# zhang-xuan1314/ABC-Net

Measured on AMD Instinct MI355X. Metric: training images/sec (384x384, b16/GPU), higher is better.
Workload: dtype bf16; 1 GPU; unet.py train step (pack+fwd+fused loss+bwd+allreduce+Adam), 384x384, batch 16/GPU, dropout 0.2; global_batch=16, parallelism=dp1, graph=True, device_meters=False, device_rasteriser=False, device_extraction=False, logits_stored=True

## Files before the change

abc-net_amd/_lib.py:

```python
from __future__ import annotations

import ctypes as C
import os

_HERE = os.path.dirname(os.path.abspath(__file__))
LIB_PATH = os.path.join(_HERE, "libabcnet_hip.so")

F32, BF16, FP8 = 0, 1, 2
MAX_TAPS = 49
OMEGA_RAW, OMEGA_PEAKS = 0, 1

vp, i32, u32, i64, f32, f64 = C.c_void_p, C.c_int32, C.c_uint32, C.c_int64, C.c_float, C.c_double


class ActSrc(C.Structure):
    _fields_ = [("x", vp), ("scale", vp), ("shift", vp), ("slope", vp), ("Hx", i32), ("Wx", i32), ("ldx", i32),
                ("pool", i32), ("drop_p", f32), ("drop_seed", u32), ("planar", i32), ("ctot", i32), ("drop_salt", vp)]


class ConvDesc(C.Structure):
    _fields_ = [("src", ActSrc), ("w", vp), ("bias", vp), ("y", vp), ("stats", vp),
                ("dtype_in", i32), ("dtype_c", i32), ("dtype_out", i32),
                ("B", i32), ("Hin", i32), ("Win", i32), ("cin_off", i32), ("Cin", i32), ("Hg", i32), ("Wg", i32),
                ("Hout", i32), ("Wout", i32), ("ldy", i32), ("cout_off", i32), ("Cout", i32), ("Cout_pad", i32),
# ... 224 lines not shown
SCAN_CONSTANT, SCAN_BAD_PARAMS = 1, 2
SCAN_NBOX = 8
SCAN_GEOM_COLUMNS = ("thr", "inverted", "status", "y0", "x0", "bh", "bw", "rows", "cols", "ddx", "ddy", "ink")
SCAN_NO_COMPONENT, SCAN_CLEAN_FAILED = 4, 8
SCAN_CLEAN_CELLS = (8, 16, 32, 64)
SCAN_CLEAN_COLUMNS = ("components", "kept", "ink_kept", "ink_dropped", "heaviest", "occupied_cells")
STROKE_UNTIL_STABLE = -1
STROKE_MAX_SIZE = 1024
STROKE_STAT_COLUMNS = ("iterations", "converged", "ink_in", "ink_out", "skipped")
MOL_EMPTY, MOL_TRUNCATED = 1, 2
MAX_CAP_ATOMS, MAX_BOND_PEAKS, MAX_SCORE_RECORD, MAX_SIM_ATOMS = 2048, 4096, 1024, 512
TEXT_BAD_ROW, TEXT_OVERFLOW = 4, 8


_STRUCTS = [ActSrc, ConvDesc, PackDesc, BnFwdDesc, ActBwdDesc, BnBwdDesc, BnApplyDesc, WgradDesc, WgradReduceDesc,
            LossDesc, LossFinDesc, AdamDesc, NmsDesc, CbamChannelDesc, CbamPixDesc, CbamConv7Desc, MetricsDesc, ExtractDesc, RasterDesc,
            HeadsFusedDesc, HeadsEpi, ConvTDesc, LossScaleDesc, AdamSeg, AdamClass, AdamMultiDesc, ImageDesc, AssembleDesc]

SELF_SIZED = [(EvalDesc, "abc_eval_desc_size"), (GraphScoreDesc, "abc_graph_score_desc_size"),
              (GraphSimilarityDesc, "abc_graph_similarity_desc_size"), (MolBlockDesc, "abc_molblock_desc_size"),
              (ScanDesc, "abc_scan_desc_size")]
SELF_SIZED_SINCE = [(StrokeDesc, "abc_stroke_desc_size"), (GraphIdentityDesc, "abc_graph_identity_desc_size"),
                    (ScanCleanDesc, "abc_scan_clean_desc_size")]

P = C.POINTER
SYMBOLS = {
    "abc_conv_stat_blocks": (C.c_int, [P(ConvDesc)]),
    "abc_convt_fused_ok": (C.c_int, [P(ConvTDesc)]),
    "abc_convt_fused_fwd": (C.c_int, [P(ConvTDesc), vp]),
    "abc_conv_actbwd_ok": (C.c_int, [P(ConvDesc)]),
    "abc_conv_fwd_batch": (C.c_int, [P(ConvDesc), C.c_int32, C.c_void_p]),
    "abc_conv_batch_ok": (C.c_int, [P(ConvDesc), C.c_int32]),
    "abc_conv_variant": (C.c_int, [vp]),
    "abc_conv_weight_layout": (C.c_int, [vp]),
    "abc_conv_fwd": (C.c_int, [P(ConvDesc), vp]),
    "abc_conv_chunk": (C.c_int, [C.c_int, C.c_int]),
    "abc_heads_batch": (C.c_int, [vp, i32, i32, vp]),
    "abc_heads_fused_pack_bytes": (i64, []),
    "abc_heads_fused_chunks": (C.c_int, [P(HeadsFusedDesc)]),
    "abc_heads_fused_loss_blocks": (C.c_int, [P(HeadsFusedDesc)]),
    "abc_heads_fused_dl_elems": (i64, [P(HeadsFusedDesc)]),
    "abc_heads_fused_wgrad_floats": (i64, [P(HeadsFusedDesc)]),
    "abc_heads_fused_rows": (C.c_int, [i32]),
    "abc_heads_fused_chan_of_row": (C.c_int, [i32, i32]),
    "abc_heads_fused_pack": (C.c_int, [P(HeadsFusedDesc), vp]),
    "abc_heads_fused_fwd_bwd": (C.c_int, [P(HeadsFusedDesc), vp]),
    "abc_heads_fused_wgrad": (C.c_int, [P(HeadsFusedDesc), vp]),
    "abc_conv_tile": (C.c_int, [P(ConvDesc), P(i32), P(i32), P(i32)]),
    "abc_conv_route_info": (C.c_int, [P(ConvDesc), P(i32)]),
    "abc_pack_conv_weights": (C.c_int, [P(PackDesc), vp]),
    "abc_pack_item_bytes": (C.c_int, []),
    "abc_pack_item_fill": (i64, [vp, P(PackDesc), i64]),
    "abc_pack_batch": (C.c_int, [vp, i32, i64, vp]),
    "abc_bn_finalize_fwd": (C.c_int, [P(BnFwdDesc), vp]),
    "abc_bn_finalize_fwd_batch": (C.c_int, [vp, i32, i32, vp]),
    "abc_bn_finalize_bwd_batch": (C.c_int, [vp, i32, i32, vp]),
    "abc_bn_eval_coeffs": (C.c_int, [vp, vp, vp, vp, vp, vp, i32, f32, vp]),
    "abc_bn_eval_fold": (C.c_int, [vp, vp, vp, vp, vp, vp, vp, i32, f32, vp]),
    "abc_act_bwd_blocks": (C.c_int, [P(ActBwdDesc)]),
    "abc_act_bwd": (C.c_int, [P(ActBwdDesc), vp]),
    "abc_bn_finalize_bwd": (C.c_int, [P(BnBwdDesc), vp]),
    "abc_bn_apply_bwd": (C.c_int, [P(BnApplyDesc), vp]),
    "abc_wgrad_fuses_apply": (C.c_int, [vp]),
    "abc_wgrad_rowsum_ok": (C.c_int, [vp]),
    "abc_wgrad_pads": (C.c_int, [P(WgradDesc), P(i32), P(i32)]),
    "abc_wgrad_blocks": (C.c_int, [P(WgradDesc)]),
    "abc_wgrad_tile": (C.c_int, [P(WgradDesc), P(i32), P(i32)]),
    "abc_wgrad_route_info": (C.c_int, [P(WgradDesc), P(i32)]),
    "abc_wgrad": (C.c_int, [P(WgradDesc), vp]),
    "abc_wgrad_reduce": (C.c_int, [P(WgradReduceDesc), vp]),
    "abc_wgrad_reduce_bn_bwd": (C.c_int, [P(WgradReduceDesc), P(BnBwdDesc), vp]),
    "abc_wgrad_heads_batch": (C.c_int, [vp, i32, vp]),
    "abc_wgrad_reduce_batch": (C.c_int, [vp, i32, vp]),
    "abc_colsum_blocks": (C.c_int, [i64]),
    "abc_colsum": (C.c_int, [vp, i32, i64, i32, i32, i32, vp, vp, vp, vp]),
    "abc_colsum_w1": (C.c_int, [vp, i32, i64, i32, i32, i32, vp, vp, vp, vp, vp]),
    "abc_loss_blocks": (C.c_int, [P(LossDesc)]),
    "abc_loss_fwd_bwd": (C.c_int, [P(LossDesc), vp]),
    "abc_loss_finalize": (C.c_int, [P(LossFinDesc), vp]),
    "abc_adam_step": (C.c_int, [P(AdamDesc), vp]),
    "abc_loss_scale_grads": (C.c_int, [P(LossScaleDesc), vp]),
    "abc_adam_multi_chunk": (C.c_int, []),
    "abc_adam_multi": (C.c_int, [P(AdamMultiDesc), vp]),
    "abc_nms_peaks": (C.c_int, [P(NmsDesc), vp]),
    "abc_extract_work_ints": (i64, [P(ExtractDesc)]),
    "abc_extract_work_masks": (i64, [P(ExtractDesc)]),
    "abc_extract_peaks": (C.c_int, [P(ExtractDesc), vp]),
    "abc_assemble_work_ints": (i64, [P(AssembleDesc)]),
    "abc_assemble_graphs": (C.c_int, [P(AssembleDesc), vp]),
    "abc_rasterize_targets": (C.c_int, [P(RasterDesc), vp]),
    "abc_build_images": (C.c_int, [P(ImageDesc), vp]),
    "abc_build_scan_images": (C.c_int, [P(ScanDesc), vp]),
    "abc_scan_desc_size": (C.c_int, []),
    "abc_build_scan_images_clean": (C.c_int, [P(ScanDesc), P(ScanCleanDesc), vp]),
    "abc_scan_clean_desc_size": (C.c_int, []),
    "abc_scan_clean_scratch_bytes": (i64, [i32, i32, i32, i32]),
    "abc_normalize_strokes": (C.c_int, [P(StrokeDesc), vp]),
    "abc_stroke_desc_size": (C.c_int, []),
    "abc_metrics_blocks": (C.c_int, [P(MetricsDesc)]),
    "abc_metrics_update": (C.c_int, [P(MetricsDesc), vp]),
    "abc_eval_tables_blocks": (C.c_int, [P(EvalDesc)]),
    "abc_eval_tables_update": (C.c_int, [P(EvalDesc), vp]),
    "abc_eval_tables_update_sparse": (C.c_int, [P(EvalDesc), vp, vp]),
    "abc_eval_desc_size": (C.c_int, []),
    "abc_graph_score_update": (C.c_int, [P(GraphScoreDesc), vp]),
    "abc_graph_score_desc_size": (C.c_int, []),
    "abc_graph_similarity_update": (C.c_int, [P(GraphSimilarityDesc), vp]),
    "abc_graph_similarity_desc_size": (C.c_int, []),
    "abc_graph_identity_update": (C.c_int, [P(GraphIdentityDesc), vp]),
    "abc_graph_identity_desc_size": (C.c_int, []),
    "abc_molblock_text_bytes": (i64, [P(MolBlockDesc)]),
    "abc_write_molblocks": (C.c_int, [P(MolBlockDesc), vp]),
    "abc_molblock_desc_size": (C.c_int, []),
    "abc_plane_sum": (C.c_int, [vp, i32, i32, i32, vp, vp, vp, vp]),
    "abc_plane_sum_work": (C.c_int, [i32]),
    "abc_cbam_channel_fwd": (C.c_int, [P(CbamChannelDesc), vp]),
    "abc_cbam_channel_bwd": (C.c_int, [P(CbamChannelDesc), vp]),
    "abc_cbam_spatial_stats": (C.c_int, [P(CbamPixDesc), vp]),
    "abc_cbam_apply_fwd": (C.c_int, [P(CbamPixDesc), vp]),
    "abc_cbam_bwd1": (C.c_int, [P(CbamPixDesc), vp]),
    "abc_cbam_bwd2_blocks": (C.c_int, [P(CbamPixDesc)]),
    "abc_cbam_bwd2": (C.c_int, [P(CbamPixDesc), vp]),
    "abc_cbam_bwd3_blocks": (C.c_int, [P(CbamPixDesc)]),
    "abc_cbam_bwd3": (C.c_int, [P(CbamPixDesc), vp]),
    "abc_cbam_conv7_fwd": (C.c_int, [P(CbamConv7Desc), vp]),
    "abc_cbam_conv7_blocks": (C.c_int, [P(CbamConv7Desc)]),
    "abc_cbam_conv7_bwd": (C.c_int, [P(CbamConv7Desc), vp]),
    "abc_cbam_conv7_bwd_partial": (C.c_int, [P(CbamConv7Desc), vp]),
    "abc_cbam_channel_bwd_c7": (C.c_int, [P(CbamChannelDesc), P(CbamConv7Desc), vp]),
    "abc_add_into": (C.c_int, [vp, i32, i32, vp, i32, i32, i32, i64, i32, vp]),
    "abc_nhwc_to_nchw_f32": (C.c_int, [vp, i32, i32, i32, i32, i32, i32, vp, vp]),
    "abc_nchw_to_nhwc_f32": (C.c_int, [vp, i32, i32, i32, i32, vp, i32, i32, vp]),
    "abc_fill_f32": (C.c_int, [vp, f32, i64, vp]),
# ... 70 lines not shown
```

abc-net_amd/csrc/bn_act.hip:

```cpp
#include "common.hpp"
#include "../../include/abcnet_hip.h"
#include "capi_util.hpp"
#include "reduce_bn.hpp"
#include <stdlib.h>

namespace {

__device__ inline void bn_finalize_fwd_body(const abc_bn_fwd_desc& d, int pstride) {
    __shared__ double sm[4];
    const int c = blockIdx.x;
    if (c >= d.C) return;
    const int rows = d.rows == 4 ? 4 : 2;
    double s1 = 0.0, s2 = 0.0;
    for (int k = threadIdx.x; k < d.nblk; k += 256) {
        s1 += (double)d.partial[((size_t)k * rows + 0) * pstride + c];
        s2 += (double)d.partial[((size_t)k * rows + 1) * pstride + c];
    }
    s1 = block_sum_f64(s1, sm);
    s2 = block_sum_f64(s2, sm);
    if (threadIdx.x == 0) {
        const double mean = s1 / d.count;
        double var = s2 / d.count - mean * mean;
        if (var < 0.0) var = 0.0;
        const float invstd = (float)(1.0 / sqrt(var + (double)d.eps));
// ... 253 lines not shown
    const int64_t nitems = d.npix * ncv;
    const int64_t stride = (int64_t)gridDim.x * 256;
    T* g = (T*)d.g;
    T* o = d.out ? (T*)d.out : g;
    const int ld_o = d.out ? d.ld_out : d.ld_g;
    const T* yr = (const T*)d.y_raw;
    for (int64_t it = (int64_t)blockIdx.x * 256 + threadIdx.x; it < nitems; it += stride) {
        const int64_t p = it / ncv;
        const int c = (int)(it % ncv) * N;
        float gv[N], x[N], out[N];
        ldv<T, N>(g + p * d.ld_g + c, gv);
        ldv<T, N>(yr + p * d.ld_y + d.cy_off + c, x);
#pragma unroll
        for (int j = 0; j < N; ++j) {
            const float xh = (x[j] - d.mean[c + j]) * d.invstd[c + j];
            out[j] = d.gscale[c + j] * (gv[j] - d.k1[c + j] - xh * d.k2[c + j]);
        }
        stv<N>(o + p * ld_o + c, out);
    }
}

template <typename T>
__global__ __launch_bounds__(256) void colsum_kernel(const T* x, int64_t npix, int ld, int c_off, int C, const float* cs,
                                                      float* work, int CW) {
    __shared__ float red[256];
    const int PL = 256 / CW;
    const int cl = threadIdx.x % CW, pl = threadIdx.x / CW;
    float acc[8];
#pragma unroll
    for (int j = 0; j < 8; ++j) acc[j] = 0.f;
    for (int64_t p = (int64_t)blockIdx.x * PL + pl; p < npix; p += (int64_t)gridDim.x * PL) {
        const T* row = x + p * ld + c_off;
#pragma unroll
        for (int j = 0; j < 8; ++j) {
            const int c = cl + j * CW;
            if (c < C) acc[j] += (float)row[c];
        }
    }
#pragma unroll
    for (int j = 0; j < 8; ++j) {
        const int c = cl + j * CW;
        __syncthreads();
        red[threadIdx.x] = acc[j];
        __syncthreads();
        if (pl == 0 && c < C) {
            float s = 0.f;
            for (int q = 0; q < PL; ++q) s += red[q * CW + cl];
            work[(size_t)blockIdx.x * C + c] = s * (cs ? cs[c_off + c] : 1.f);
        }
    }
}
template <typename T>
__global__ __launch_bounds__(256) void colsum_vec_kernel(const T* x, int64_t npix, int ld, int c_off, int C, const float* cs, float* work) {
    constexpr int N = VecOf<T>::N;
    __shared__ float red[256][N + 1];
    const int ncv = C / N;
    const int cv = threadIdx.x % ncv, pl = threadIdx.x / ncv, PL = 256 / ncv;
    float acc[N];
#pragma unroll
    for (int j = 0; j < N; ++j) acc[j] = 0.f;
    const T* base = x + c_off + cv * N;
    int64_t p = (int64_t)blockIdx.x * PL + pl;
    const int64_t step = (int64_t)gridDim.x * PL;
    for (; p + step < npix; p += 2 * step) {
        float a[N], b[N];
        ldv<T, N>(base + p * ld, a);
        ldv<T, N>(base + (p + step) * ld, b);
#pragma unroll
        for (int j = 0; j < N; ++j) acc[j] += a[j] + b[j];
    }
    if (p < npix) {
        float a[N];
        ldv<T, N>(base + p * ld, a);
#pragma unroll
        for (int j = 0; j < N; ++j) acc[j] += a[j];
    }
#pragma unroll
    for (int j = 0; j < N; ++j) red[threadIdx.x][j] = acc[j];
    __syncthreads();
    for (int c = threadIdx.x; c < C; c += 256) {
        const int v = c / N, j = c % N;
        float s = 0.f;
        for (int q = 0; q < PL; ++q) s += red[q * ncv + v][j];
        work[(size_t)blockIdx.x * C + c] = s * (cs ? cs[c_off + c] : 1.f);
    }
}

__global__ __launch_bounds__(256) void colsum_reduce_kernel(const float* work, int nblk, int C, float* out) {
    __shared__ double sm[4];
    const int c = blockIdx.x;
    double s = 0.0;
    for (int k = threadIdx.x; k < nblk; k += 256) s += (double)work[(size_t)k * C + c];
    s = block_sum_f64(s, sm);
    if (threadIdx.x == 0) out[c] = (float)s;
}
template <typename T>
__global__ __launch_bounds__(256) void colsum_w1_kernel(const T* x, int64_t npix, int ld, int c_off, int C, const float* w, float* work) {
    constexpr int N = VecOf<T>::N;
    __shared__ float red[256][2 * N + 1];
    const int ncv = C / N;
    const int cv = threadIdx.x % ncv, pl = threadIdx.x / ncv, PL = 256 / ncv;
    float acc[N], accw[N];
#pragma unroll
    for (int j = 0; j < N; ++j) { acc[j] = 0.f; accw[j] = 0.f; }
    const T* base = x + c_off + cv * N;
    int64_t p = (int64_t)blockIdx.x * PL + pl;
    const int64_t step = (int64_t)gridDim.x * PL;
    for (; p + 3 * step < npix; p += 4 * step) {
        float a[4][N], wv[4];
#pragma unroll
        for (int u = 0; u < 4; ++u) { ldv<T, N>(base + (p + u * step) * ld, a[u]); wv[u] = w[p + u * step]; }
#pragma unroll
        for (int u = 0; u < 4; ++u)
#pragma unroll
            for (int j = 0; j < N; ++j) { acc[j] += a[u][j]; accw[j] = fmaf(a[u][j], wv[u], accw[j]); }
    }
    for (; p < npix; p += step) {
        float a[N];
        ldv<T, N>(base + p * ld, a);
        const float wv = w[p];
#pragma unroll
        for (int j = 0; j < N; ++j) { acc[j] += a[j]; accw[j] = fmaf(a[j], wv, accw[j]); }
    }
#pragma unroll
    for (int j = 0; j < N; ++j) { red[threadIdx.x][j] = acc[j]; red[threadIdx.x][N + j] = accw[j]; }
    __syncthreads();
    for (int c = threadIdx.x; c < 2 * C; c += 256) {
        const int row = c / C, cc = c - row * C;
        const int v = cc / N, j = cc % N;
        float s = 0.f;
        for (int q = 0; q < PL; ++q) s += red[q * ncv + v][row * N + j];
        work[((size_t)blockIdx.x * 2 + row) * C + cc] = s;
    }
}
__global__ __launch_bounds__(256) void colsum_w1_reduce_kernel(const float* work, int nblk, int C, float* out_sum, float* out_w) {
    __shared__ double sm[4];
    const int c = blockIdx.x, row = blockIdx.y;
    double s = 0.0;
    for (int k = threadIdx.x; k < nblk; k += 256) s += (double)work[((size_t)k * 2 + row) * C + c];
    s = block_sum_f64(s, sm);
    if (threadIdx.x == 0) {
        if (row == 0) { if (out_sum != nullptr) out_sum[c] = (float)s; }
        else out_w[c] = (float)s;
    }
}

__global__ void fill_kernel(float* p, float v, int64_t n) {
// ... 90 lines not shown

static int act_bwd_check(const abc_act_bwd_desc* d) {
    const int N = d->dtype == ABC_BF16 ? 8 : 4;
    if (d->C % N) return abc_fail(ABC_EINVAL, "act_bwd: C must be a multiple of the vector width");
    const int ncv = d->C / N;
    if (ncv > 256 || (256 % ncv)) return abc_fail(ABC_EUNSUPPORTED, "act_bwd: C/vec must divide 256");
    if (d->dA_pool && (((d->H | d->W) & 1) && d->drop_p > 0.f)) return abc_fail(ABC_EUNSUPPORTED, "act_bwd: odd pooled dims with dropout");
    if (!d->dA_pool && !d->dA_same) return abc_fail(ABC_EINVAL, "act_bwd: no gradient source");
    if ((d->ld_y | d->ld_g | d->cy_off) % N) return abc_fail(ABC_EINVAL, "act_bwd: alignment");
    if ((int64_t)d->B * d->H * d->W * ncv >= (int64_t(1) << 31)) return abc_fail(ABC_EUNSUPPORTED, "act_bwd: tensor too large for 32-bit indexing");
    return ABC_OK;
}

extern "C" int abc_act_bwd_blocks(const abc_act_bwd_desc* d) {
    const int N = d->dtype == ABC_BF16 ? 8 : 4;
    const bool pooled = d->dA_pool != nullptr;
    const int64_t n = (int64_t)d->B * (pooled ? d->H / 2 : d->H) * (pooled ? d->W / 2 : d->W) * (d->C / N);
    return ew_blocks(n);
}

extern "C" int abc_act_bwd(const abc_act_bwd_desc* d, abc_stream_t stream) {
    int rc = act_bwd_check(d);
    if (rc) return rc;
    const int nb = abc_act_bwd_blocks(d);
    if (d->dA_pool == nullptr && d->drop_p <= 0.f) {
        if (d->dtype == ABC_BF16) hipLaunchKernelGGL(act_bwd_plain_kernel<bf16>, dim3(nb), dim3(256), 0, (hipStream_t)stream, *d);
        else hipLaunchKernelGGL(act_bwd_plain_kernel<float>, dim3(nb), dim3(256), 0, (hipStream_t)stream, *d);
        return abc_check_launch("act_bwd");
    }
    if (d->dtype == ABC_BF16) hipLaunchKernelGGL(act_bwd_kernel<bf16>, dim3(nb), dim3(256), 0, (hipStream_t)stream, *d);
    else hipLaunchKernelGGL(act_bwd_kernel<float>, dim3(nb), dim3(256), 0, (hipStream_t)stream, *d);
    return abc_check_launch("act_bwd");
}

extern "C" int abc_bn_apply_bwd(const abc_bn_apply_desc* d, abc_stream_t stream) {
    const int N = d->dtype == ABC_BF16 ? 8 : 4;
    if (d->C % N || (d->ld_g | d->ld_y | d->cy_off) % N || (d->out && d->ld_out % N)) return abc_fail(ABC_EINVAL, "bn_apply: alignment");
    const int nb = ew_blocks(d->npix * (d->C / N));
    if (d->dtype == ABC_BF16) hipLaunchKernelGGL(bn_apply_kernel<bf16>, dim3(nb), dim3(256), 0, (hipStream_t)stream, *d);
    else hipLaunchKernelGGL(bn_apply_kernel<float>, dim3(nb), dim3(256), 0, (hipStream_t)stream, *d);
    return abc_check_launch("bn_apply_bwd");
}

extern "C" int abc_colsum_blocks(int64_t npix) {
    int64_t b = (npix + 63) / 64;
    return (int)(b < 1 ? 1 : (b > 1024 ? 1024 : b));
}

extern "C" int abc_colsum(const void* x, int32_t dtype, int64_t npix, int32_t ld, int32_t c_off, int32_t C,
                          const float* chan_scale, float* work, float* out, abc_stream_t stream) {
    const int nb = abc_colsum_blocks(npix);
    hipStream_t st = (hipStream_t)stream;
    if (C > 512) return abc_fail(ABC_EUNSUPPORTED, "colsum: C > 512");
    {
        const int N = dtype == ABC_BF16 ? 8 : 4;
        const int ncv = C / N;
        if (C % N == 0 && ncv >= 1 && ncv <= 256 && 256 % ncv == 0 && ld % N == 0 && c_off % N == 0) {
            if (dtype == ABC_BF16)
                hipLaunchKernelGGL(colsum_vec_kernel<bf16>, dim3(nb), dim3(256), 0, st, (const bf16*)x, npix, ld, c_off, C, chan_scale, work);
            else
                hipLaunchKernelGGL(colsum_vec_kernel<float>, dim3(nb), dim3(256), 0, st, (const float*)x, npix, ld, c_off, C, chan_scale, work);
            hipLaunchKernelGGL(colsum_reduce_kernel, dim3(C), dim3(256), 0, st, (const float*)work, nb, C, out);
            return abc_check_launch("colsum");
        }
    }
    int CW = 1;
    while (CW < C && CW < 64) CW <<= 1;
    if (dtype == ABC_BF16)
        hipLaunchKernelGGL(colsum_kernel<bf16>, dim3(nb), dim3(256), 0, st, (const bf16*)x, npix, ld, c_off, C, chan_scale, work, CW);
    else
        hipLaunchKernelGGL(colsum_kernel<float>, dim3(nb), dim3(256), 0, st, (const float*)x, npix, ld, c_off, C, chan_scale, work, CW);
    hipLaunchKernelGGL(colsum_reduce_kernel, dim3(C), dim3(256), 0, st, (const float*)work, nb, C, out);
    return abc_check_launch("colsum");
}

extern "C" int abc_colsum_w1(const void* x, int32_t dtype, int64_t npix, int32_t ld, int32_t c_off, int32_t C, const float* w,
                             float* work, float* out_sum, float* out_w, abc_stream_t stream) {
    const int nb = abc_colsum_blocks(npix);
    const int N = dtype == ABC_BF16 ? 8 : 4;
    const int ncv = C / N;
    if (x == nullptr || w == nullptr || work == nullptr || out_w == nullptr) return abc_fail(ABC_EINVAL, "colsum_w1: x, w, work and out_w are required");
    if (C % N || ncv < 1 || ncv > 256 || 256 % ncv || ld % N || c_off % N)
        return abc_fail(ABC_EUNSUPPORTED, "colsum_w1: C / vector width must divide 256, ld and c_off be multiples of the vector width");
    hipStream_t st = (hipStream_t)stream;
    if (dtype == ABC_BF16) hipLaunchKernelGGL(colsum_w1_kernel<bf16>, dim3(nb), dim3(256), 0, st, (const bf16*)x, npix, ld, c_off, C, w, work);
    else hipLaunchKernelGGL(colsum_w1_kernel<float>, dim3(nb), dim3(256), 0, st, (const float*)x, npix, ld, c_off, C, w, work);
    hipLaunchKernelGGL(colsum_w1_reduce_kernel, dim3(C, 2), dim3(256), 0, st, (const float*)work, nb, C, out_sum, out_w);
    return abc_check_launch("colsum_w1");
}

template <typename InT, typename OutT>
__global__ __launch_bounds__(256) void pool_act_kernel(const InT* x, const float* sc, const float* sh, const float* sl, int Hx, int Wx,
                                                        int ldx, int c_off, int C, int64_t nseg, OutT* out, int ld_out) {
    const int64_t i = (int64_t)blockIdx.x * 256 + threadIdx.x;
    if (i >= nseg) return;
    const int segs = C / 8;
    const int sg = (int)(i % segs);
    int64_t pix = i / segs;
    const int Wo = Wx / 2, Ho = Hx / 2;
    const int xo = (int)(pix % Wo); pix /= Wo;
    const int yo = (int)(pix % Ho);
    const int b = (int)(pix / Ho);
    const int c = c_off + sg * 8;
    float a[8], s_[8], t_[8];
    const bool tr = sc != nullptr;
#pragma unroll
    for (int j = 0; j < 8; ++j) { a[j] = tr ? sc[c + j] : 1.f; s_[j] = tr ? sh[c + j] : 0.f; t_[j] = tr ? sl[c + j] : 1.f; }
    float m[8];
#pragma unroll
    for (int q = 0; q < 4; ++q) {
        float v[8];
        LoadVec<InT, 8>::ld(x + ((size_t)(b * Hx + 2 * yo + (q >> 1)) * Wx + 2 * xo + (q & 1)) * ldx + c, v);
#pragma unroll
        for (int j = 0; j < 8; ++j) {
            const float y = tr ? abc_act(v[j], a[j], s_[j], t_[j]) : v[j];
            m[j] = (q == 0) ? y : fmaxf(m[j], y);
        }
// ... 54 lines not shown
```

abc-net_amd/csrc/misc.hip:

```cpp
#include "common.hpp"
#include "../../include/abcnet_hip.h"
#include "capi_util.hpp"
#include <string.h>

static thread_local char g_err[256] = "";
int abc_fail(int code, const char* msg) {
    strncpy(g_err, msg, sizeof(g_err) - 1);
    g_err[sizeof(g_err) - 1] = 0;
    return code;
}
int abc_allow_lds(const void* fn, int bytes, unsigned long long* done) {
    int dev = 0;
    if (hipGetDevice(&dev) != hipSuccess) dev = -1;
    if (dev >= 0 && dev < 64 && ((*done >> dev) & 1ull)) return ABC_OK;
    hipError_t e = hipFuncSetAttribute(fn, hipFuncAttributeMaxDynamicSharedMemorySize, bytes);
    if (e != hipSuccess) {
        snprintf(g_err, sizeof(g_err), "hipFuncSetAttribute(MaxDynamicSharedMemorySize=%d) on device %d: %s", bytes, dev, hipGetErrorString(e));
        return ABC_ELAUNCH;
    }
    if (dev >= 0 && dev < 64) *done |= 1ull << dev;
    return ABC_OK;
}
int abc_check_launch(const char* what) {
    hipError_t e = hipGetLastError();
// ... 44 lines not shown
            const int nx = d.px ? 2 : 1;
            const int iy = t / nx, ix = t % nx;
            const int ky = d.py ? (iy == 0 ? 0 : 2) : 1;
            const int kx = d.px ? (ix == 0 ? 0 : 2) : 1;
            if (n < d.Cout && rc < d.Cin) v = d.w[(((size_t)rc * d.Cout + n) * 3 + ky) * 3 + kx];
        } else {
            if (n < d.Cin && rc < d.Cout) v = d.w[((size_t)n * d.Cout + rc) * 9 + t];
        }
        if (d.row_scale != nullptr && (d.mode == 0 || d.mode == 2) && n < d.Cout) v *= d.row_scale[n];
        const int rtot = d.rows_total > 0 ? d.rows_total : d.rows_pad;
        dst[abc_pack_offset((size_t)t * nch_total + ch_off + c, rtot, d.rows_off + n, CK, k, d.layout)] = CT(v);
    }
}

struct PackItem { abc_pack_desc d; int32_t CK, ntaps, nchunks, dtype; int64_t first; int32_t ntiles, pad_; };
__device__ inline void pack_one(const PackItem& it, unsigned r) {
    const abc_pack_desc& d = it.d;
    const unsigned CK = it.CK, ntaps = it.ntaps, nchunks = it.nchunks, rows = d.rows_pad;
    const unsigned k = r % CK; r /= CK;
    const unsigned n = r % rows; r /= rows;
    const unsigned c = r % nchunks;
    const unsigned t = r / nchunks;
    const unsigned rc = c * CK + k;
    float v = 0.f;
    if (d.mode == 0) {
        if (n < (unsigned)d.Cout && rc < (unsigned)d.Cin) v = d.w[((size_t)n * d.Cin + rc) * ntaps + t];
    } else if (d.mode == 1) {
        if (n < (unsigned)d.Cin && rc < (unsigned)d.Cout) v = d.w[((size_t)rc * d.Cin + n) * ntaps + t];
    } else if (d.mode == 2) {
        const unsigned nx = d.px ? 2 : 1;
        const unsigned iy = t / nx, ix = t % nx;
        const unsigned ky = d.py ? (iy == 0 ? 0 : 2) : 1;
        const unsigned kx = d.px ? (ix == 0 ? 0 : 2) : 1;
        if (n < (unsigned)d.Cout && rc < (unsigned)d.Cin) v = d.w[(((size_t)rc * d.Cout + n) * 3 + ky) * 3 + kx];
    } else {
        if (n < (unsigned)d.Cin && rc < (unsigned)d.Cout) v = d.w[((size_t)n * d.Cout + rc) * 9 + t];
    }
    if (d.row_scale != nullptr && (d.mode == 0 || d.mode == 2) && n < (unsigned)d.Cout) v *= d.row_scale[n];
    const unsigned nch_total = (d.red_total + CK - 1) / CK, ch_off = d.red_off / CK;
    const unsigned rtot = d.rows_total > 0 ? (unsigned)d.rows_total : rows;
    const size_t o = abc_pack_offset((size_t)t * nch_total + ch_off + c, (int)rtot, (int)((unsigned)d.rows_off + n), (int)CK, (int)k, d.layout);
    if (it.dtype == ABC_BF16) ((bf16*)d.dst)[o] = (bf16)v; else if (it.dtype == ABC_FP8) ((f8*)d.dst)[o] = f8(v); else ((float*)d.dst)[o] = v;
}

constexpr int PACK_CHUNK = 2048;
__device__ inline int pack_find(const PackItem* items, int nitems, int64_t i) {
    int lo = 0, hi = nitems - 1;
    while (lo < hi) {
        const int mid = (lo + hi + 1) >> 1;
        if (items[mid].first <= i) lo = mid; else hi = mid - 1;
    }
    return lo;
}
__global__ __launch_bounds__(256) void pack_batch_kernel(const PackItem* items, int nitems, int64_t total) {
    __shared__ int s_lo, s_hi;
    const int64_t i0 = (int64_t)blockIdx.x * PACK_CHUNK;
    const int64_t i1 = (i0 + PACK_CHUNK < total) ? i0 + PACK_CHUNK : total;
    if (threadIdx.x == 0) { s_lo = pack_find(items, nitems, i0); s_hi = pack_find(items, nitems, i1 - 1); }
    __syncthreads();
    const int lo = __builtin_amdgcn_readfirstlane(s_lo), hi = __builtin_amdgcn_readfirstlane(s_hi);
    if (lo == hi) {
        const PackItem it = items[lo];
        if (it.ntiles > 0) return;
        const unsigned base = (unsigned)(i0 - it.first);
        for (unsigned e = threadIdx.x; e < (unsigned)(i1 - i0); e += 256) pack_one(it, base + e);
    } else {
        for (int64_t i = i0 + threadIdx.x; i < i1; i += 256) {
            const int j = pack_find(items, nitems, i);
            if (items[j].ntiles > 0) continue;
            pack_one(items[j], (unsigned)(i - items[j].first));
        }
    }
}

constexpr int PT_MAXT = 9;
constexpr int PT_MAXITEMS = 1023;
__global__ __launch_bounds__(256) void pack_tiles_kernel(const PackItem* items, int nitems) {
    __shared__ float tile[32 * (32 * PT_MAXT + 1)];
    __shared__ int s_nt[PT_MAXITEMS + 1];
    __shared__ int s_item, s_tile;
    const int tid = threadIdx.x;
    for (int j = tid; j < nitems; j += 256) s_nt[j + 1] = items[j].ntiles;
    __syncthreads();
    if (tid == 0) {
        s_nt[0] = 0;
        for (int j = 0; j < nitems; ++j) s_nt[j + 1] += s_nt[j];
    }
    __syncthreads();
    const int total = s_nt[nitems];
    for (int tg = blockIdx.x; tg < total; tg += gridDim.x) {
        __syncthreads();
        if (tid == 0) {
            int lo = 0, hi = nitems - 1;
            while (lo < hi) { const int mid = (lo + hi + 1) >> 1; if (s_nt[mid] <= tg) lo = mid; else hi = mid - 1; }
            s_item = lo; s_tile = tg - s_nt[lo];
        }
        __syncthreads();
        const PackItem it = items[__builtin_amdgcn_readfirstlane(s_item)];
        const abc_pack_desc& d = it.d;
        const int tl = __builtin_amdgcn_readfirstlane(s_tile);
        const int ntaps = it.ntaps, nchunks = it.nchunks;
        const int c = tl % nchunks, rb = tl / nchunks;
        const int n0 = rb * 32, k0 = c * 32;
        const int S = 32 * ntaps + 1;
        const int rows_real = d.mode == 0 ? d.Cout : d.Cin;
        const bool real = n0 < rows_real;
        if (real) {
            if ((((uintptr_t)d.w) & 15) == 0) {
                const int j = tid >> 3, q0 = tid & 7;
                const float* src = d.mode == 0 ? d.w + ((size_t)(n0 + j) * d.Cin + k0) * ntaps : d.w + ((size_t)(k0 + j) * d.Cin + n0) * ntaps;
                f32x4 v[PT_MAXT];
#pragma unroll
                for (int m = 0; m < PT_MAXT; ++m) {
                    if (m < ntaps) v[m] = *(const f32x4*)(src + 4 * (q0 + 8 * m));
                }
#pragma unroll
                for (int m = 0; m < PT_MAXT; ++m) {
                    if (m < ntaps) {
                        float* o = tile + j * S + 4 * (q0 + 8 * m);
                        o[0] = v[m][0]; o[1] = v[m][1]; o[2] = v[m][2]; o[3] = v[m][3];
                    }
                }
            } else {
                const int wv = tid >> 6, ln = tid & 63;
                constexpr int NQ = (32 * PT_MAXT + 63) / 64;
                float v[8][NQ];
#pragma unroll
                for (int jj = 0; jj < 8; ++jj) {
                    const int j = wv * 8 + jj;
                    const float* src = d.mode == 0 ? d.w + ((size_t)(n0 + j) * d.Cin + k0) * ntaps : d.w + ((size_t)(k0 + j) * d.Cin + n0) * ntaps;
#pragma unroll
                    for (int m = 0; m < NQ; ++m) {
                        const int q = ln + 64 * m;
                        v[jj][m] = q < 32 * ntaps ? src[q] : 0.f;
                    }
                }
#pragma unroll
                for (int jj = 0; jj < 8; ++jj) {
#pragma unroll
                    for (int m = 0; m < NQ; ++m) {
                        const int q = ln + 64 * m;
                        if (q < 32 * ntaps) tile[(wv * 8 + jj) * S + q] = v[jj][m];
                    }
                }
            }
        }
        __syncthreads();
        const int nch_total = (d.red_total + 31) / 32, ch_off = d.red_off / 32;
        const int rtot = d.rows_total > 0 ? d.rows_total : d.rows_pad;
        const int r = tid & 31, g = (tid >> 5) & 3, th = tid >> 7;
        const float rs = (real && d.row_scale != nullptr && d.mode == 0) ? d.row_scale[n0 + r] : 1.f;
        for (int t = th; t < ntaps; t += 2) {
            bf16x8 o;
#pragma unroll
            for (int i = 0; i < 8; ++i) {
                float v = 0.f;
                if (real) v = d.mode == 0 ? tile[r * S + (8 * g + i) * ntaps + t] : tile[(8 * g + i) * S + r * ntaps + t];
                if (d.row_scale != nullptr && d.mode == 0) v *= rs;
                o[i] = (bf16)v;
            }
            const size_t off = abc_pack_offset((size_t)t * nch_total + ch_off + c, rtot, d.rows_off + n0 + r, 32, 8 * g, d.layout);
            *(bf16x8*)((bf16*)d.dst + off) = o;
        }
    }
}

__global__ void step_inc_kernel(int64_t* step) { *step += 1; }

__global__ __launch_bounds__(256) void adam_kernel(const abc_adam_desc d) {
    const double t = (double)*d.step;
    const float bc1 = (float)(1.0 - pow((double)d.beta1, t));
    const float bc2s = (float)sqrt(1.0 - pow((double)d.beta2, t));
    const float step_size = d.lr / bc1;
    const int64_t n4 = d.n / 4;
    const int64_t stride = (int64_t)gridDim.x * 256;
    for (int64_t i = (int64_t)blockIdx.x * 256 + threadIdx.x; i < n4; i += stride) {
        f32x4 p = ((f32x4*)d.p)[i], g = ((const f32x4*)d.g)[i], m = ((f32x4*)d.m)[i], v = ((f32x4*)d.v)[i];
#pragma unroll
        for (int j = 0; j < 4; ++j) {
            const float gg = g[j] * d.grad_scale + d.weight_decay * p[j];
            m[j] = m[j] + (gg - m[j]) * (1.f - d.beta1);
            v[j] = v[j] * d.beta2 + (1.f - d.beta2) * gg * gg;
            p[j] -= step_size * m[j] / (sqrtf(v[j]) / bc2s + d.eps);
        }
        ((f32x4*)d.p)[i] = p; ((f32x4*)d.m)[i] = m; ((f32x4*)d.v)[i] = v;
    }
    if (blockIdx.x == 0) {
        for (int64_t i = n4 * 4 + threadIdx.x; i < d.n; i += 256) {
            const float gg = d.g[i] * d.grad_scale + d.weight_decay * d.p[i];
            const float m = d.m[i] + (gg - d.m[i]) * (1.f - d.beta1);
            const float v = d.v[i] * d.beta2 + (1.f - d.beta2) * gg * gg;
            d.m[i] = m; d.v[i] = v;
            d.p[i] -= step_size * m / (sqrtf(v) / bc2s + d.eps);
        }
    }
}

__global__ __launch_bounds__(256) void nms_kernel(const abc_nms_desc d) {
    const int hw = d.h * d.w;
    const int64_t npix = (int64_t)d.B * hw;
    const int64_t p = (int64_t)blockIdx.x * 256 + threadIdx.x;
    if (p >= npix) return;
    const int b = (int)(p / hw), yx = (int)(p % hw);
    const int y = yx / d.w, x = yx % d.w;
    for (int which = 0; which < 2; ++which) {
        const float* L = (which ? d.bond : d.atom) + (size_t)b * hw;
        const float v = L[yx];
        float m = v;
        for (int dy = -1; dy <= 1; ++dy)
            for (int dx = -1; dx <= 1; ++dx) {
                const int yy = y + dy, xx = x + dx;
                if (yy >= 0 && yy < d.h && xx >= 0 && xx < d.w) m = fmaxf(m, L[yy * d.w + xx]);
            }
        float* o = which ? d.bond_mask : d.atom_mask;
        o[(size_t)b * hw + yx] = (m == v && v > -1.f) ? 1.f : 0.f;
    }
    const int n = d.n_omega;
// ... 127 lines not shown
    }
    const int CK = d->ck;
    if (CK != abc_conv_chunk(d->dtype_c, d->red_total)) return abc_fail(ABC_EINVAL, "pack: ck does not match red_total");
    if (d->layout != 0 && (d->layout != 1 || CK * abc_dsize(d->dtype_c) != 64 || (d->rows_total > 0 ? d->rows_total : d->rows_pad) % 32 || d->rows_off % 32))
        return abc_fail(ABC_EINVAL, "pack: layout 1 needs 64-byte chunks (bf16 CK = 32 / fp8 CK = 64), whole 32-row blocks");
    if (d->red_pad % CK || d->red_pad < red || d->red_off % CK || d->red_off + d->red_pad > abc_roundup(d->red_total, CK))
        return abc_fail(ABC_EINVAL, "pack: red_pad/red_off");
    const int nchunks = d->red_pad / CK;
    const int64_t total = (int64_t)ntaps * nchunks * d->rows_pad * CK;
    int nb = (int)((total + 255) / 256);
    if (nb > 4096) nb = 4096;
    if (d->dtype_c == ABC_BF16) hipLaunchKernelGGL(pack_kernel<bf16>, dim3(nb), dim3(256), 0, (hipStream_t)stream, *d, CK, ntaps, nchunks);
    else if (d->dtype_c == ABC_FP8) hipLaunchKernelGGL(pack_kernel<f8>, dim3(nb), dim3(256), 0, (hipStream_t)stream, *d, CK, ntaps, nchunks);
    else hipLaunchKernelGGL(pack_kernel<float>, dim3(nb), dim3(256), 0, (hipStream_t)stream, *d, CK, ntaps, nchunks);
    return abc_check_launch("pack_conv_weights");
}

static int pack_shape(const abc_pack_desc* d, int* ntaps, int* red) {
    switch (d->mode) {
        case 0: *ntaps = d->kh * d->kw; *red = d->Cin; return 0;
        case 1: *ntaps = d->kh * d->kw; *red = d->Cout; return 0;
        case 2: *ntaps = (d->py ? 2 : 1) * (d->px ? 2 : 1); *red = d->Cin; return 0;
        case 3: *ntaps = 9; *red = d->Cout; return 0;
        default: return -1;
    }
}

extern "C" int abc_pack_item_bytes(void) { return (int)sizeof(PackItem); }

extern "C" int64_t abc_pack_item_fill(void* item, const abc_pack_desc* d, int64_t first) {
    int ntaps, red;
    if (pack_shape(d, &ntaps, &red)) { abc_fail(ABC_EINVAL, "pack: mode"); return -1; }
    const int CK = d->ck;
    if (CK != abc_conv_chunk(d->dtype_c, d->red_total) || d->red_pad % CK || d->red_pad < red || d->red_off % CK ||
        d->red_off + d->red_pad > abc_roundup(d->red_total, CK)) { abc_fail(ABC_EINVAL, "pack: red_pad/red_off/ck"); return -1; }
    if (d->layout != 0 && (d->layout != 1 || CK * abc_dsize(d->dtype_c) != 64 || (d->rows_total > 0 ? d->rows_total : d->rows_pad) % 32 || d->rows_off % 32)) {
        abc_fail(ABC_EINVAL, "pack: layout 1 needs 64-byte chunks (bf16 CK = 32 / fp8 CK = 64), whole 32-row blocks"); return -1;
    }
    PackItem* it = (PackItem*)item;
    it->d = *d; it->CK = CK; it->ntaps = ntaps; it->nchunks = d->red_pad / CK; it->dtype = d->dtype_c; it->first = first;
    const bool tiles = (d->mode == 0 || d->mode == 1) && d->dtype_c == ABC_BF16 && CK == 32 && ntaps <= PT_MAXT && d->Cout % 32 == 0 &&
                       d->Cin % 32 == 0 && d->rows_pad % 32 == 0 && d->red_pad == red && ((uintptr_t)d->dst & 15) == 0 &&
                       d->rows_off % 32 == 0;
    it->ntiles = tiles ? (d->rows_pad / 32) * it->nchunks : 0;
    it->pad_ = 0;
    return tiles ? 0 : (int64_t)ntaps * it->nchunks * d->rows_pad * CK;
}

extern "C" int abc_pack_batch(const void* items_dev, int32_t nitems, int64_t total, abc_stream_t stream) {
    if (nitems < 1 || total < 0) return abc_fail(ABC_EINVAL, "pack_batch: empty");
    if (nitems > PT_MAXITEMS) return abc_fail(ABC_EINVAL, "pack_batch: more than 1023 items");
    const int64_t nb = (total + PACK_CHUNK - 1) / PACK_CHUNK;
    if (nb > 0) hipLaunchKernelGGL(pack_batch_kernel, dim3((int)nb), dim3(256), 0, (hipStream_t)stream, (const PackItem*)items_dev, nitems, total);
    hipLaunchKernelGGL(pack_tiles_kernel, dim3(2048), dim3(256), 0, (hipStream_t)stream, (const PackItem*)items_dev, nitems);
    return abc_check_launch("pack_batch");
}

extern "C" int abc_adam_step(const abc_adam_desc* d, abc_stream_t stream) {
    if (d->n < 1) return abc_fail(ABC_EINVAL, "adam: empty");
    if (((uintptr_t)d->p | (uintptr_t)d->g | (uintptr_t)d->m | (uintptr_t)d->v) & 15) return abc_fail(ABC_EINVAL, "adam: 16-byte alignment");
    hipStream_t st = (hipStream_t)stream;
    hipLaunchKernelGGL(step_inc_kernel, dim3(1), dim3(1), 0, st, d->step);
    int64_t nb = (d->n / 4 + 255) / 256;
    if (nb > 2048) nb = 2048;
    if (nb < 1) nb = 1;
    hipLaunchKernelGGL(adam_kernel, dim3((int)nb), dim3(256), 0, st, *d);
    return abc_check_launch("adam_step");
}

extern "C" int abc_plane_sum_work(int32_t C) { return C * PS_CHUNKS; }

extern "C" int abc_plane_sum(const float* x, int32_t B, int32_t C, int32_t HW, const float* chan_scale, float* work, float* out,
                             abc_stream_t stream) {
    if (C < 1) return abc_fail(ABC_EINVAL, "plane_sum: empty");
    hipLaunchKernelGGL(plane_sum_kernel, dim3(C, PS_CHUNKS), dim3(256), 0, (hipStream_t)stream, x, B, C, HW, work);
    hipLaunchKernelGGL(plane_sum_reduce_kernel, dim3(abc_cdiv(C, 64)), dim3(64), 0, (hipStream_t)stream, (const float*)work, C,
                       chan_scale, out);
    return abc_check_launch("plane_sum");
}

extern "C" int abc_nms_peaks(const abc_nms_desc* d, abc_stream_t stream) {
    const int64_t npix = (int64_t)d->B * d->h * d->w;
    hipLaunchKernelGGL(nms_kernel, dim3((int)((npix + 255) / 256)), dim3(256), 0, (hipStream_t)stream, *d);
    return abc_check_launch("nms_peaks");
}

__global__ void counter_add_kernel(uint32_t* p, uint32_t inc) { *p += inc; }
struct ConcatArgs { const float* src[16]; int32_t first[17]; };
__global__ __launch_bounds__(256) void concat_kernel(const ConcatArgs a, int n, float* dst) {
    const int i = blockIdx.x * 256 + threadIdx.x;
    if (i >= a.first[n]) return;
    int j = 0;
    while (j + 1 < n && a.first[j + 1] <= i) ++j;
    dst[i] = a.src[j][i - a.first[j]];
}
extern "C" int abc_concat_f32(const float* const* srcs, const int32_t* counts, int32_t n, float* dst, abc_stream_t stream) {
    if (n < 1 || n > 16) return abc_fail(ABC_EINVAL, "concat_f32: 1..16 arrays");
    ConcatArgs a;
    a.first[0] = 0;
    for (int i = 0; i < n; ++i) {
        if (counts[i] < 0 || srcs[i] == nullptr) return abc_fail(ABC_EINVAL, "concat_f32: null / negative entry");
        a.src[i] = srcs[i]; a.first[i + 1] = a.first[i] + counts[i];
    }
    for (int i = n; i < 16; ++i) { a.src[i] = srcs[0]; a.first[i + 1] = a.first[n]; }
    if (a.first[n] == 0) return ABC_OK;
    hipLaunchKernelGGL(concat_kernel, dim3(abc_cdiv(a.first[n], 256)), dim3(256), 0, (hipStream_t)stream, a, n, dst);
    return abc_check_launch("concat_f32");
}

extern "C" int abc_counter_add_u32(uint32_t* p, uint32_t inc, abc_stream_t stream) {
    if (!p) return abc_fail(ABC_EINVAL, "counter_add: null");
    hipLaunchKernelGGL(counter_add_kernel, dim3(1), dim3(1), 0, (hipStream_t)stream, p, inc);
    return abc_check_launch("counter_add");
}

extern "C" int abc_sizeof(int which) {
    switch (which) {
        case 0: return (int)sizeof(abc_act_src);
        case 1: return (int)sizeof(abc_conv_desc);
        case 2: return (int)sizeof(abc_pack_desc);
// ... 29 lines not shown
```

abc-net_amd/csrc/reduce_bn.hpp:

```cpp
#pragma once
#include "common.hpp"
#include "../../include/abcnet_hip.h"

__device__ inline double block_sum_f64(double v, double* sm) {
#pragma unroll
    for (int o = 32; o > 0; o >>= 1) v += __shfl_xor(v, o);
    const int w = threadIdx.x >> 6;
    __syncthreads();
    if ((threadIdx.x & 63) == 0) sm[w] = v;
    __syncthreads();
    return sm[0] + sm[1] + sm[2] + sm[3];
}


__device__ inline void bn_finalize_bwd_body(const abc_bn_bwd_desc& d, int pstride, int c) {
    __shared__ double sm[4];
    if (c >= d.C) return;
    double s1 = 0.0, s2 = 0.0;
    for (int k = threadIdx.x; k < d.nblk; k += 256) {
        s1 += (double)d.partial[((size_t)k * 2 + 0) * pstride + c];
        s2 += (double)d.partial[((size_t)k * 2 + 1) * pstride + c];
    }
    s1 = block_sum_f64(s1, sm);
    s2 = block_sum_f64(s2, sm);
// ... 35 lines not shown
    const float s = (s0 + s1) + (s2 + s3);
    float* o = d.dw + ((size_t)ai * d.Cb + bi) * d.ntaps + t;
    *o = d.accumulate ? (*o + s) : s;
}



__device__ inline void wgrad_reduce_vec_body(const abc_wgrad_reduce_desc& d, int blk) {
    __shared__ float4 sm[3][64];
    const int cb4 = d.Cb >> 2;
    const int64_t n4 = (int64_t)d.ntaps * d.Ca * cb4;
    const int64_t idx = (int64_t)blk * 64 + (threadIdx.x & 63);
    const int g = threadIdx.x >> 6;
    const bool live = idx < n4;
    const int bi = live ? (int)(idx % cb4) * 4 : 0;
    const int ai = live ? (int)((idx / cb4) % d.Ca) : 0;
    const int t = live ? (int)(idx / ((int64_t)cb4 * d.Ca)) : 0;
    const size_t slab = (size_t)d.Ca_pad * d.Cb_pad;
    const size_t step = (size_t)d.ntaps * slab;
    const int k0 = (int)((int64_t)d.nsplit * g / 4), k1 = (int)((int64_t)d.nsplit * (g + 1) / 4);
    const float* p = d.partial + (size_t)t * slab + (size_t)ai * d.Cb_pad + bi + (size_t)k0 * step;
    float4 s0 = {0.f, 0.f, 0.f, 0.f}, s1 = s0;
    int k = k0;
    if (live) {
        for (; k + 8 <= k1; k += 8, p += 8 * step) {
            float4 v[8];
#pragma unroll
            for (int j = 0; j < 8; ++j) v[j] = *(const float4*)(p + (size_t)j * step);
#pragma unroll
            for (int j = 0; j < 8; j += 2) {
                s0.x += v[j].x; s0.y += v[j].y; s0.z += v[j].z; s0.w += v[j].w;
                s1.x += v[j + 1].x; s1.y += v[j + 1].y; s1.z += v[j + 1].z; s1.w += v[j + 1].w;
            }
        }
        for (; k < k1; ++k, p += step) {
            const float4 v = *(const float4*)p;
            s0.x += v.x; s0.y += v.y; s0.z += v.z; s0.w += v.w;
        }
    }
    s0.x += s1.x; s0.y += s1.y; s0.z += s1.z; s0.w += s1.w;
    if (g > 0) sm[g - 1][threadIdx.x & 63] = s0;
    __syncthreads();
    if (g > 0 || !live) return;
#pragma unroll
    for (int w = 0; w < 3; ++w) {
        const float4 v = sm[w][threadIdx.x];
        s0.x += v.x; s0.y += v.y; s0.z += v.z; s0.w += v.w;
    }
    float* o = d.dw + ((size_t)ai * d.Cb + bi) * d.ntaps + t;
    const float r[4] = {s0.x, s0.y, s0.z, s0.w};
#pragma unroll
    for (int j = 0; j < 4; ++j) o[(size_t)j * d.ntaps] = d.accumulate ? (o[(size_t)j * d.ntaps] + r[j]) : r[j];
}
```

abc-net_amd/csrc/wgrad.hip:

```cpp
#include "wgrad_parts.hpp"
#include "capi_util.hpp"
#include "reduce_bn.hpp"
#include "conv_fast.hpp"
#include <stddef.h>
#include <stdlib.h>
#include <algorithm>

namespace {

constexpr int MAXT_FAST = 9;
constexpr int MAXT_SLOW = 5;
constexpr int WTHR_HOST = 512;

struct WgK {
    ActSrc p, q;
    float* partial;
    int B, Hg, Wg, Hq, Wq;
    int cp_off, Ca, cq_off, Cb, Ca_pad, Cb_pad;
    int ntaps, tgw, nsplit, npatch, tiles_x, tiles_y;
    int dy_min, dx_min, HH, HW, PSWP, PSWQ, sP_bytes, sQ_bytes, coef_off, cstrP, cstrQ, nta, ntb, fast_p, fast_q, nbuf;
    unsigned bytesP2;
    int magicQ, k3;
    unsigned mg_tx, mg_ty;
    int regP;
    int qtab_off;
    unsigned bytesP, bytesQ;
    const void* p2; void* p_out; int ld_p2, cp2_off, ld_pout;
    int8_t ty[ABC_MAX_TAPS], tx[ABC_MAX_TAPS];
};
static_assert(sizeof(WgK) == 448 && offsetof(WgK, bytesP2) == 284 && offsetof(WgK, k3) == 292 && offsetof(WgK, qtab_off) == 308 &&
              offsetof(WgK, p2) == 320 && offsetof(WgK, ty) == 348, "WgK: the argument offsets the kernels were tuned with");

template <typename T, typename CT, int CW>
__device__ inline void stage_slow(char* dst, int RS, int PS, int HH, int HW, int b, int iy0, int ix0, int Hin, int Win,
                                                     const ActSrc* s, int c0, int tid, int cvalid, int nthr) {
    stage_halo<T, CT, CW>(dst, RS, PS, HH, HW, b, iy0, ix0, Hin, Win, *s, c0, tid, nthr, cvalid);
}

template <typename PT, typename QT, typename CT, int AT, int BT, int STRIDE, bool FAST, int PM, bool K3, bool DUAL = false, bool TS = false>
__global__ __launch_bounds__(WTHR_HOST, 2) void wgrad_kernel(const WgK a) {
    constexpr int WTHR = WTHR_HOST;
    static_assert(!TS || (AT == 1 && BT == 1 && FAST && !K3 && sizeof(CT) == 2), "tap split: one bf16 tile pair on the prefetch path");
    constexpr int MAXT = TS ? 4 : (FAST ? MAXT_FAST : MAXT_SLOW);
    constexpr int RSPLIT = TS ? 1 : (WTHR / 64) / (AT * BT);
    constexpr int PROWS = 8 * PM;
    constexpr int ROWS = PROWS / RSPLIT;
    constexpr int CWP = AT * 32, CWQ = BT * 32;
    constexpr int NPF_P = (PROWS * 16 * (CWP / Frag<CT>::NV) + WTHR - 1) / WTHR;
    constexpr int NPF_Q = (PM > 1 || STRIDE == 2) ? 5 : ((sizeof(CT) == 2) ? 4 : 6);
    extern __shared__ __attribute__((aligned(16))) char smem[];
    const int buf_bytes = a.sP_bytes + a.sQ_bytes;
    float* sCoefP = (float*)(smem + a.coef_off);
    float* sCoefQ = sCoefP + 3 * a.cstrP;
    const int tid = threadIdx.x, lane = tid & 63, wave = tid >> 6;
    const int r = lane & 31, h = lane >> 5;

    int id = abc_xcd_remap(blockIdx.x, gridDim.x);
    const int bt = id % a.ntb; id /= a.ntb;
// ... 268 lines not shown
            if (a.nbuf == 1) __syncthreads();
        }
        if (has_next) commit(next, smem + ((a.nbuf == 2) ? ((it + 1) & 1) * buf_bytes : 0));
        __syncthreads();
    }

    if constexpr (RSPLIT > 1) {
        float* red = (float*)smem;
#pragma unroll
        for (int t = 0; t < MAXT; ++t) {
            if (t < tcnt) {
                __syncthreads();
                if (rs > 0) {
#pragma unroll
                    for (int k = 0; k < 16; ++k) red[(wave * 16 + k) * 64 + lane] = acc[t][k];
                }
                __syncthreads();
                if (rs == 0) {
                    for (int w = 1; w < RSPLIT; ++w)
#pragma unroll
                        for (int k = 0; k < 16; ++k) acc[t][k] += red[((wave + w) * 16 + k) * 64 + lane];
                }
            }
        }
        if (rs != 0) return;
    }

#pragma unroll
    for (int t = 0; t < MAXT; ++t) {
        if (tap_ok(t)) {
            float* out = a.partial + ((size_t)(split * a.ntaps + tap_of(t)) * a.Ca_pad + ca0 + ai * 32) * a.Cb_pad + cb0 + bi * 32 + r;
#pragma unroll
            for (int k = 0; k < 16; ++k) {
                const int arow = (k & 3) + 8 * (k >> 2) + 4 * h;
                out[(size_t)arow * a.Cb_pad] = acc[t][k];
            }
        }
    }
}

__global__ __launch_bounds__(256) void wgrad_reduce_kernel(const abc_wgrad_reduce_desc d) { wgrad_reduce_body(d, blockIdx.x); }

__global__ __launch_bounds__(256) void wgrad_reduce_vec_kernel(const abc_wgrad_reduce_desc d) { wgrad_reduce_vec_body(d, blockIdx.x); }

struct ReduceBn { abc_wgrad_reduce_desc r; abc_bn_bwd_desc f; int nr, vec; };
__global__ __launch_bounds__(256) void wgrad_reduce_bn_kernel(const ReduceBn a) {
    if ((int)blockIdx.x < a.nr) {
        if (a.vec) wgrad_reduce_vec_body(a.r, blockIdx.x); else wgrad_reduce_body(a.r, blockIdx.x);
    } else {
        bn_finalize_bwd_body(a.f, a.f.C, (int)blockIdx.x - a.nr);
    }
}

__global__ __launch_bounds__(64) void wgrad_reduce_wave_kernel(const abc_wgrad_reduce_desc d) {
    const int idx = blockIdx.x;
    const int bi = idx % d.Cb, ai = (idx / d.Cb) % d.Ca, t = idx / (d.Cb * d.Ca);
    const size_t slab = (size_t)d.Ca_pad * d.Cb_pad;
    const float* p = d.partial + (size_t)t * slab + (size_t)ai * d.Cb_pad + bi;
    const size_t step = (size_t)d.ntaps * slab;
    float s = 0.f;
    for (int k = threadIdx.x; k < d.nsplit; k += 64) s += p[(size_t)k * step];
    for (int m = 32; m >= 1; m >>= 1) s += __shfl_xor(s, m);
    if (threadIdx.x == 0) {
        float* o = d.dw + ((size_t)ai * d.Cb + bi) * d.ntaps + t;
        *o = d.accumulate ? (*o + s) : s;
    }
}

constexpr int MAX_RB = 16;
struct ReduceBatch { abc_wgrad_reduce_desc d[MAX_RB]; };
__global__ __launch_bounds__(256) void wgrad_reduce_batch_kernel(const ReduceBatch bt) {
    const abc_wgrad_reduce_desc& d = bt.d[blockIdx.y];
    const int64_t n = (int64_t)d.ntaps * d.Ca * d.Cb;
    const size_t slab = (size_t)d.Ca_pad * d.Cb_pad;
    const size_t step = (size_t)d.ntaps * slab;
    if (n <= 4096 && d.nsplit >= 128) {
        const int64_t idx = (int64_t)blockIdx.x * 4 + (threadIdx.x >> 6);
        const int lane = threadIdx.x & 63;
        if (idx >= n) return;
        const int bi = (int)(idx % d.Cb), ai = (int)((idx / d.Cb) % d.Ca), t = (int)(idx / ((int64_t)d.Cb * d.Ca));
        const float* p = d.partial + (size_t)t * slab + (size_t)ai * d.Cb_pad + bi;
        float s = 0.f;
        for (int k = lane; k < d.nsplit; k += 64) s += p[(size_t)k * step];
        for (int m = 32; m >= 1; m >>= 1) s += __shfl_xor(s, m);
        if (lane == 0) {
            float* o = d.dw + ((size_t)ai * d.Cb + bi) * d.ntaps + t;
            *o = d.accumulate ? (*o + s) : s;
        }
        return;
    }
    const int64_t idx = (int64_t)blockIdx.x * 256 + threadIdx.x;
    if (idx >= n) return;
    const int bi = (int)(idx % d.Cb);
    const int ai = (int)((idx / d.Cb) % d.Ca);
    const int t = (int)(idx / ((int64_t)d.Cb * d.Ca));
    const float* p = d.partial + (size_t)t * slab + (size_t)ai * d.Cb_pad + bi;
    float s0 = 0.f, s1 = 0.f, s2 = 0.f, s3 = 0.f;
    int k = 0;
    for (; k + 4 <= d.nsplit; k += 4) {
        s0 += p[(size_t)k * step]; s1 += p[(size_t)(k + 1) * step]; s2 += p[(size_t)(k + 2) * step]; s3 += p[(size_t)(k + 3) * step];
    }
    for (; k < d.nsplit; ++k) s0 += p[(size_t)k * step];
    const float s = (s0 + s1) + (s2 + s3);
    float* o = d.dw + ((size_t)ai * d.Cb + bi) * d.ntaps + t;
    *o = d.accumulate ? (*o + s) : s;
}

struct WGeom {
    int AT, BT, dy_min, dx_min, HH, HW, PSWP, PSWQ, sP_bytes, sQ_bytes, coef_off, cstrP, cstrQ, lds, tgw, ngroups, nta, ntb, npatch,
        tiles_x, tiles_y, fast_p, fast_q, nbuf, PM, ts;
    int64_t bytesP, bytesQ;
};

static int psw_for(int cw, int csz) {
    if (csz == 2) return cw == 32 ? 64 : (cw == 64 ? 192 : 320);
    return cw * 4;
}

static bool fast_ok(const abc_act_src& s, int csz_c, int cvalid_min, int64_t bytes) {
    const int nv = 16 / csz_c;
    return !s.pool && !s.planar && s.drop_p <= 0.f && (cvalid_min % nv) == 0 && bytes < (int64_t(1) << 31);
}

static int wgeom_pm(const abc_wgrad_desc* d, WGeom* g, int pm) {
    const int csz = d->dtype_c == ABC_BF16 ? 2 : 4;
    const int cwp = g->AT * 32, cwq = g->BT * 32;
    g->PM = pm;
    int dymin = 127, dymax = -127, dxmin = 127, dxmax = -127;
    for (int t = 0; t < d->ntaps; ++t) {
        dymin = d->tap_dy[t] < dymin ? d->tap_dy[t] : dymin; dymax = d->tap_dy[t] > dymax ? d->tap_dy[t] : dymax;
        dxmin = d->tap_dx[t] < dxmin ? d->tap_dx[t] : dxmin; dxmax = d->tap_dx[t] > dxmax ? d->tap_dx[t] : dxmax;
    }
    g->dy_min = dymin; g->dx_min = dxmin;
    g->HH = (8 * pm - 1) * d->stride + (dymax - dymin) + 1;
    g->HW = 15 * d->stride + (dxmax - dxmin) + 1;
    g->PSWP = psw_for(cwp, csz); g->PSWQ = psw_for(cwq, csz);
    g->sP_bytes = abc_roundup(128 * pm * g->PSWP, 256);
    g->sQ_bytes = abc_roundup(g->HH * g->HW * g->PSWQ, 256);
    g->cstrP = cwp; g->cstrQ = cwq;
    const int coef_bytes = 3 * (cwp + cwq) * 4 + 256;
    g->nbuf = (2 * (g->sP_bytes + g->sQ_bytes) + coef_bytes <= 160 * 1024) ? 2 : 1;
    g->coef_off = g->nbuf * (g->sP_bytes + g->sQ_bytes);
    g->lds = g->coef_off + coef_bytes;
    if (g->lds < 8 * 16 * 64 * 4) g->lds = 8 * 16 * 64 * 4;
    if (g->lds > 160 * 1024) return abc_fail(ABC_EUNSUPPORTED, "wgrad: LDS tile too large");
    g->nta = abc_cdiv(d->Ca, cwp); g->ntb = abc_cdiv(d->Cb, cwq);
    g->tiles_x = abc_cdiv(d->Wg, 16); g->tiles_y = abc_cdiv(d->Hg, 8 * pm);
    g->npatch = g->tiles_x * g->tiles_y * d->B;
    const int lastP = d->Ca - (g->nta - 1) * cwp, lastQ = d->Cb - (g->ntb - 1) * cwq;
    const int segq = cwq / (16 / csz);
    g->bytesP = (int64_t)d->B * d->p.Hx * d->p.Wx * d->p.ldx * (d->dtype_p == ABC_BF16 ? 2 : 4);
    g->bytesQ = (int64_t)d->B * d->q.Hx * d->q.Wx * d->q.ldx * (d->dtype_q == ABC_BF16 ? 2 : 4);
    g->fast_p = (fast_ok(d->p, csz, lastP, g->bytesP) && g->HH * g->HW * g->HW < 65536) ? 1 : 0;
    g->fast_q = (fast_ok(d->q, csz, lastQ, g->bytesQ) && abc_cdiv(g->HH * g->HW * segq, WTHR_HOST) <= ((pm > 1 || (d->stride == 2 && csz == 2)) ? 5 : (csz == 2 ? 4 : 6))) ? 1 : 0;
    g->ngroups = abc_cdiv(d->ntaps, (g->fast_p && g->fast_q) ? MAXT_FAST : MAXT_SLOW);
    g->tgw = abc_cdiv(d->ntaps, g->ngroups);
    return ABC_OK;
}
// ... 182 lines not shown
    return wgrad_route(d, &r) ? -1 : r.blocks;
}

extern "C" int abc_wgrad(const abc_wgrad_desc* d, abc_stream_t stream) {
    if (d->nsplit < 1) return abc_fail(ABC_EINVAL, "wgrad: nsplit");
    if (d->ntaps < 1 || d->ntaps > ABC_MAX_TAPS) return abc_fail(ABC_EINVAL, "wgrad: ntaps");
    WgRoute r;
    if (int rc = wgrad_route(d, &r)) return rc;
    if (r.family == WG_HEAD) return abc_wgrad_head_launch(d, stream);
    const int php = d->p.pool ? d->p.Hx / 2 : d->p.Hx, pwp = d->p.pool ? d->p.Wx / 2 : d->p.Wx;
    const int qhp = d->q.pool ? d->q.Hx / 2 : d->q.Hx, qwp = d->q.pool ? d->q.Wx / 2 : d->q.Wx;
    if (php != d->Hg || pwp != d->Wg || qhp != d->Hq || qwp != d->Wq) return abc_fail(ABC_EINVAL, "wgrad: dims mismatch");
    if (r.family == WG_C1) return abc_wgrad_c1_launch(d, stream);
    if (r.family == WG_NARROW16) return abc_wgrad_narrow_launch(d, stream);
    if (r.family == WG_N32R2) return abc_wgrad_n32r2_launch(d, stream);
    const WGeom& g = r.g;
    WgK k{};
    auto cp = [](ActSrc& o, const abc_act_src& i) {
        o.x = i.x; o.scale = i.scale; o.shift = i.shift; o.slope = i.slope; o.Hx = i.Hx; o.Wx = i.Wx; o.ldx = i.ldx;
        o.pool = i.pool; o.drop_p = i.drop_p; o.drop_seed = i.drop_seed; o.planar = i.planar; o.ctot = i.ctot; o.drop_salt = i.drop_salt;
    };
    cp(k.p, d->p); cp(k.q, d->q);
    k.partial = d->partial; k.B = d->B; k.Hg = d->Hg; k.Wg = d->Wg; k.Hq = d->Hq; k.Wq = d->Wq;
    k.cp_off = d->cp_off; k.Ca = d->Ca; k.cq_off = d->cq_off; k.Cb = d->Cb;
    k.Ca_pad = r.ca_pad; k.Cb_pad = r.cb_pad;
    k.ntaps = d->ntaps; k.tgw = g.tgw; k.nsplit = d->nsplit; k.npatch = g.npatch; k.tiles_x = g.tiles_x; k.tiles_y = g.tiles_y;
    k.dy_min = g.dy_min; k.dx_min = g.dx_min; k.HH = g.HH; k.HW = g.HW; k.PSWP = g.PSWP; k.PSWQ = g.PSWQ;
    k.sP_bytes = g.sP_bytes; k.sQ_bytes = g.sQ_bytes; k.coef_off = g.coef_off; k.cstrP = g.cstrP; k.cstrQ = g.cstrQ;
    k.nta = g.nta; k.ntb = g.ntb; k.fast_p = g.fast_p; k.fast_q = g.fast_q; k.nbuf = g.nbuf;
    k.magicQ = 65536 / g.HW + 1;
    if (g.npatch >= 65536 || g.tiles_x > 4096 || g.tiles_y > 4096) return abc_fail(ABC_EUNSUPPORTED, "wgrad: more than 65535 patches");
    k.mg_tx = (unsigned)((0x100000000ull + (unsigned)g.tiles_x - 1) / (unsigned)g.tiles_x);
    k.mg_ty = (unsigned)((0x100000000ull + (unsigned)g.tiles_y - 1) / (unsigned)g.tiles_y);
    k.regP = (d->Hg % (8 * g.PM) == 0 && d->Wg % 16 == 0 && d->p.Hx == d->Hg && d->p.Wx == d->Wg) ? 1 : 0;
    k.k3 = r.k3; k.qtab_off = r.qtab_off;
    if (d->p_dual) {
        if (!r.fuses_apply) return abc_fail(ABC_EUNSUPPORTED, "wgrad: p_dual is not served for this descriptor (abc_wgrad_fuses_apply)");
        k.p2 = d->p2; k.p_out = d->p_out; k.ld_p2 = d->ld_p2; k.cp2_off = d->cp2_off; k.ld_pout = d->ld_pout;
        k.bytesP2 = (unsigned)((int64_t)d->B * d->Hg * d->Wg * d->ld_p2 * 2);
    }
    k.bytesP = (unsigned)g.bytesP; k.bytesQ = (unsigned)g.bytesQ;
    for (int t = 0; t < d->ntaps; ++t) { k.ty[t] = (int8_t)(d->tap_dy[t] - g.dy_min); k.tx[t] = (int8_t)(d->tap_dx[t] - g.dx_min); }
    hipStream_t st = (hipStream_t)stream;
    if (d->dtype_c == ABC_F32) {
        if (d->dtype_p != ABC_F32 || d->dtype_q != ABC_F32) return abc_fail(ABC_EUNSUPPORTED, "wgrad: f32 compute needs f32 operands");
        return wdispatch<float, float, float>(k, g, d->stride, d->nsplit, st);
    }
    if (d->dtype_p == ABC_BF16 && d->dtype_q == ABC_BF16) return wdispatch<bf16, bf16, bf16>(k, g, d->stride, d->nsplit, st);
    if (d->dtype_p == ABC_F32 && d->dtype_q == ABC_BF16) return wdispatch<float, bf16, bf16>(k, g, d->stride, d->nsplit, st);
    if (d->dtype_p == ABC_BF16 && d->dtype_q == ABC_F32) return wdispatch<bf16, float, bf16>(k, g, d->stride, d->nsplit, st);
    return abc_fail(ABC_EUNSUPPORTED, "wgrad: dtype combination");
}

extern "C" int abc_wgrad_reduce(const abc_wgrad_reduce_desc* d, abc_stream_t stream) {
    const ReduceForm f = reduce_form(*d);
    if (f.kind == RED_WAVE) hipLaunchKernelGGL(wgrad_reduce_wave_kernel, dim3(f.grid), dim3(64), 0, (hipStream_t)stream, *d);
    else if (f.kind == RED_VEC) hipLaunchKernelGGL(wgrad_reduce_vec_kernel, dim3(f.grid), dim3(256), 0, (hipStream_t)stream, *d);
    else hipLaunchKernelGGL(wgrad_reduce_kernel, dim3(f.grid), dim3(256), 0, (hipStream_t)stream, *d);
    return abc_check_launch("wgrad_reduce");
}

extern "C" int abc_wgrad_reduce_bn_bwd(const abc_wgrad_reduce_desc* d, const abc_bn_bwd_desc* f, abc_stream_t stream) {
    if (f->C < 1 || f->nblk < 1) return abc_fail(ABC_EINVAL, "wgrad_reduce_bn_bwd: empty finaliser");
    const ReduceForm rf = reduce_form(*d);
    if (rf.kind == RED_WAVE) {
        if (int rc = abc_wgrad_reduce(d, stream)) return rc;
        return abc_bn_finalize_bwd(f, stream);
    }
    ReduceBn a;
    a.r = *d; a.f = *f;
    a.vec = rf.kind == RED_VEC ? 1 : 0;
    a.nr = rf.grid;
    hipLaunchKernelGGL(wgrad_reduce_bn_kernel, dim3(a.nr + f->C), dim3(256), 0, (hipStream_t)stream, a);
    return abc_check_launch("wgrad_reduce_bn_bwd");
}

extern "C" int abc_wgrad_reduce_batch(const abc_wgrad_reduce_desc* descs, int32_t n, abc_stream_t stream) {
    if (n < 1 || n > MAX_RB) return abc_fail(ABC_EINVAL, "wgrad_reduce_batch: 1..16 items");
    ReduceBatch bt;
    int64_t gx = 1;
    for (int i = 0; i < n; ++i) {
        bt.d[i] = descs[i];
        const int64_t cnt = (int64_t)descs[i].ntaps * descs[i].Ca * descs[i].Cb;
        const int64_t blocks = reduce_form(descs[i]).kind == RED_WAVE ? (cnt + 3) / 4 : (cnt + 255) / 256;
        gx = blocks > gx ? blocks : gx;
    }
    for (int i = n; i < MAX_RB; ++i) bt.d[i] = descs[0];
    hipLaunchKernelGGL(wgrad_reduce_batch_kernel, dim3((int)gx, n), dim3(256), 0, (hipStream_t)stream, bt);
    return abc_check_launch("wgrad_reduce_batch");
}
```

abc-net_amd/engine.py:

```python
from __future__ import annotations

import ctypes as C
import weakref
from typing import NamedTuple

import torch

from . import _lib as L
from . import arch

BN_EPS = 1e-5
BN_MOM = 0.1
DROP_STEP = 0x9E3779B9
def head_offsets(heads):
    offs, o = [], 0
    for h in heads:
        offs.append(o)
        o += h
    return offs


def taps_square(k):
    p = (k - 1) // 2
    return [(ky - p, kx - p) for ky in range(k) for kx in range(k)]
# ... 33 lines not shown

class Src:

    def __init__(self, t, dt, H, W, ld, coff, C, coef=None, pool=False, drop_p=0.0, drop_seed=0, producer=None, planar=False):
        self.t, self.dt, self.H, self.W, self.ld, self.coff, self.C = t, dt, H, W, ld, coff, C
        self.coef, self.pool, self.drop_p, self.drop_seed, self.producer = coef, pool, drop_p, drop_seed, producer
        self.drop_salt = None
        self.planar = planar
        self.q = None

    def lh(self):
        return (self.H // 2, self.W // 2) if self.pool else (self.H, self.W)

    def fill(self, a: L.ActSrc):
        a.x = self.t.data_ptr()
        a.planar, a.ctot = (1, self.C) if self.planar else (0, 0)
        if self.coef is not None:
            a.scale, a.shift, a.slope = (c.data_ptr() for c in self.coef)
        else:
            a.scale = a.shift = a.slope = None
        a.Hx, a.Wx, a.ldx, a.pool = self.H, self.W, self.ld, 1 if self.pool else 0
        a.drop_p, a.drop_seed = self.drop_p, self.drop_seed
        a.drop_salt = self.drop_salt.data_ptr() if (self.drop_salt is not None and self.drop_p > 0) else None


class Rec:

    def __init__(self, **kw):
        self.grad_same = None
        self.grad_pool = None
        self.__dict__.update(kw)


def set_reserved_cus(n):
    lib = L.load()
    n = (int(n) + 3) & ~3
    if n == lib.abc_get_reserved_cus():
        return n
    alive = [e for e in Engine._live]
    if alive:
        raise L.AbcNetHipError("cannot change the reserved-CU count from %d to %d: %d plan(s) built under the current value are alive "
                               "(it is a process-wide setting baked into their grids; build every Trainer / InferenceRunner of this "
                               "process with the same reserve_cus, or drop the old ones first)" % (lib.abc_get_reserved_cus(), n, len(alive)))
    L.check(lib.abc_set_reserved_cus(n), "set_reserved_cus")
    return n


class Engine:
    _live = weakref.WeakSet()

    def __init__(self, variant, in_channels, heads, params, grads, buffers, counters, layout, B, H, W, dtype, train,
                 dropout_p=0.2, device="cuda", drop_seed=0x1234ABCD, fold_bn=False, fused_heads=False, batched_heads=True, fp8=False,
                 guards=False, heads_epilogue=False, actbwd_epilogue=True, merge_reduce=True, nms_heads=False, decode=False,
                 dual_wgrad=True, fused_convt=True, zero_skip=True):
        if variant not in ("unet", "unet2"):
            raise NotImplementedError("variant %r" % variant)
        if H < 32 or W < 32:
            raise ValueError("H and W must be at least 32 (five 2x2 poolings; got %dx%d)" % (H, W))
        if in_channels < 1:
            raise ValueError("in_channels must be positive")
        self.in_channels = in_channels
        self.lib = L.load()
        self.reserved_cus = self.lib.abc_get_reserved_cus()
        self.dual_wgrad = bool(dual_wgrad)
        self.fused_convt = bool(fused_convt)
        self.variant, self.heads, self.B, self.H, self.W = variant, list(heads), B, H, W
        self.train = train
        self.fold = bool(fold_bn)
        if self.fold and (train or variant != "unet"):
            raise ValueError("fold_bn is the eval-mode graph of unet.py")
        self.fp8 = bool(fp8)
        if self.fp8 and not (self.fold and dtype == "bf16"):
            raise ValueError("fp8 is a form of the BatchNorm-folded bf16 inference graph (fold_bn=True, dtype='bf16')")
        self.fp8_recs = []
        self.hfeat_q = None
        self.fp8_calibrated = False
        self.guards = bool(guards)
        self._guarded = []
        self.heads_epilogue = bool(heads_epilogue)
        self.nms_heads = bool(nms_heads) and not train
        self.nms_rho = self.nms_omega = None
        self.decode = bool(decode) and self.nms_heads
        self.btype_idx = None
        self.actbwd_epilogue = bool(actbwd_epilogue)
        self.merge_reduce = bool(merge_reduce)
        self.zero_skip = bool(zero_skip)
        self._pending_reduce = None
        self.dt = L.BF16 if dtype == "bf16" else L.F32
        self.tdt = torch.bfloat16 if dtype == "bf16" else torch.float32
        self.batched_heads = bool(batched_heads)
        self.want_fused_heads = bool(fused_heads) and train and dtype == "bf16" and self.batched_heads and self.heads == arch.TRAIN_HEADS
        self.hf = None
        self.dev = device
        self.params, self.grads, self.buffers, self.counters = params, grads, buffers, counters
        self.lay_p, self.lay_b, self.lay_c = layout
        self.drop_p = dropout_p if (train and variant == "unet") else 0.0
        self.drop_seed = drop_seed & 0xFFFFFFFF
        self.drop_salt = torch.zeros(1, dtype=torch.int32, device=device)
        self.head_off = head_offsets(self.heads)
        self.keep = []
        self.pack_ops, self.fwd_ops, self.bwd_ops = [], [], []
        self._pack_descs = []
        self._w_layout = {}
        self.recs = []
        self._ws_need = 0
        self._ws_users = []
        self._colsum_need = 0
        self._colsum_users = []
        self._build()
        Engine._live.add(self)

    def dropout_seed(self, nth_forward):
        return (self.drop_seed + nth_forward * DROP_STEP) & 0xFFFFFFFF

    def P(self, name):
        off, n = self.lay_p[name]
        return self.params.data_ptr() + 4 * off

    def G(self, name):
        off, n = self.lay_p[name]
        return self.grads.data_ptr() + 4 * off

    def Bf(self, name):
        off, n = self.lay_b[name]
        return self.buffers.data_ptr() + 4 * off

    def Cn(self, name):
        return self.counters.data_ptr() + 8 * self.lay_c[name]

    GUARD_BYTES = 4096

    def new(self, shape, dtype=None, fill=0.0):
        dtype = dtype or self.tdt
        if not self.guards:
            t = torch.full(shape, fill, dtype=dtype, device=self.dev)
            self.keep.append(t)
            return t
        n = 1
        for s_ in shape:
            n *= s_
        esz = torch.empty((), dtype=dtype).element_size()
        body = -(-n * esz // 256) * 256
        raw = torch.full((body + 2 * self.GUARD_BYTES,), 0xA5, dtype=torch.uint8, device=self.dev)
        t = raw[self.GUARD_BYTES:self.GUARD_BYTES + n * esz].view(dtype).view(shape)
        t.fill_(fill)
        self.keep.append(t)
        self._guarded.append((raw, n * esz, tuple(shape), str(dtype)))
        return t

    def check_guards(self):
        if not self.guards:
            raise RuntimeError("this plan was built without guards (Engine(guards=True) / Trainer(guards=True))")
        bad = []
        for i, (raw, nbytes, shape, dt) in enumerate(self._guarded):
            G = self.GUARD_BYTES
            lo_ok = bool((raw[:G] == 0xA5).all())
            hi_ok = bool((raw[G + nbytes:] == 0xA5).all())
            if not (lo_ok and hi_ok):
                bad.append((i, shape, dt, "below" if not lo_ok else "above"))
        if bad:
            raise RuntimeError("out-of-bounds stores next to %d of %d plan buffers: %s" % (len(bad), len(self._guarded), bad[:8]))
        return len(self._guarded)

    def act_buf(self, H, W, C, dt=None):
        t = self.new((self.B, H, W, C), self._tdt(dt)) if dt is not None else self.new((self.B, H, W, C))
        coef = (self.new((C,), torch.float32, 1.0), self.new((C,), torch.float32, 0.0), self.new((C,), torch.float32, 1.0))
        return t, coef

    def _emit(self, ops, fn, args, what, writes=(), meta=None):
        args = [C.byref(a) if isinstance(a, C.Structure) else a for a in args]
        ops.append(Op(fn, args, what, tuple(writes), meta or {"kernel": what.split(" ")[0], "flops": 0, "bytes": 0}))
        return args

    def _ew_meta(self, kernel, npix, Cn, passes, dt=None):
        return {"kernel": kernel, "flops": 0, "bytes": float(npix * Cn * self._esz(self.dt if dt is None else dt) * passes)}

    def _batch(self, descs, metas, kernel):
        arr = (type(descs[0]) * len(descs))(*descs)
        return arr, {"kernel": kernel, "flops": sum(m["flops"] for m in metas), "bytes": sum(m["bytes"] for m in metas)}

    def _flush_reduce(self, ops):
        pr = getattr(self, "_pending_reduce", None)
        if pr is not None:
            self._pending_reduce = None
            pops, rd, what, writes, meta = pr
            self._emit(pops, self.lib.abc_wgrad_reduce, (rd,), what, writes=writes, meta=meta)

    def _emit_bn_bwd(self, ops, f, what, writes):
        pr = getattr(self, "_pending_reduce", None)
        if pr is None or pr[0] is not ops or not self.merge_reduce:
            self._flush_reduce(ops)
            self._emit(ops, self.lib.abc_bn_finalize_bwd, (f,), what, writes=writes)
            return
        self._pending_reduce = None
        _pops, rd, rwhat, rwrites, rmeta = pr
        meta = {"ws": rmeta.get("ws", 0), "kernel": "wgrad_reduce+bn_bwd", "flops": 0, "bytes": rmeta["bytes"]}
        self._emit(ops, self.lib.abc_wgrad_reduce_bn_bwd, (rd, f), rwhat + " + " + what, tuple(rwrites) + tuple(writes), meta)

    def _dn(self, dt):
        return {L.BF16: "bf16", L.F32: "f32", L.FP8: "fp8"}[dt]

    def _esz(self, dt):
        return {L.BF16: 2, L.F32: 4, L.FP8: 1}[dt]

    def _tdt(self, dt):
        return {L.BF16: torch.bfloat16, L.F32: torch.float32, L.FP8: torch.float8_e4m3fn}[dt]

    FP8_OUT = ("up3.conv.double_conv.0", "up3.conv.double_conv.3", "dconv1.double_conv.0", "dconv1.double_conv.3",
               "dconv2.double_conv.0", "dconv2.double_conv.3")

    def _out_dt(self, cname):
        return L.FP8 if (self.fp8 and cname in self.FP8_OUT) else self.dt

    def emit_pack(self, wname, dst, mode, Cout, Cin, k, rows_pad, red_real, red_total=None, red_off=0, py=0, px=0, rows_total=0,
                  rows_off=0, row_scale=None, cdt=None):
        cdt = self.dt if cdt is None else cdt
        d = L.PackDesc()
        d.rows_total, d.rows_off = rows_total, rows_off
        d.row_scale = row_scale
        d.w, d.dst, d.mode, d.dtype_c = self.P(wname), dst.data_ptr(), mode, cdt
        d.Cout, d.Cin, d.kh, d.kw, d.py, d.px = Cout, Cin, k, k, py, px
        total = red_real if red_total is None else red_total
        ck = self.lib.abc_conv_chunk(cdt, total)
        d.rows_pad, d.red_pad, d.red_total, d.red_off, d.ck = rows_pad, -(-red_real // ck) * ck, total, red_off, ck
        self._pack_descs.append(d)

    def packed(self, ntaps, red, rows_pad, cdt=None):
        cdt = self.dt if cdt is None else cdt
        ck = self.lib.abc_conv_chunk(cdt, red)
        if ck <= 0:
            raise ValueError("no K-chunk for %d reduction channels in %s" % (red, self._dn(cdt)))
        return self.new((ntaps * (-(-red // ck)) * rows_pad * ck,), self._tdt(cdt))

    def _pack_weights(self, wname, mode, cout, cin, k):
        rows, red = (cout, cin) if mode == 0 else (cin, cout)
        rows_pad = -(-rows // 32) * 32
        w = self.packed(k * k, red, rows_pad)
        self.emit_pack(wname, w, mode, cout, cin, k, rows_pad, red)
        return w

    def emit_conv(self, ops, src: Src, w, bias, y, y_dt, Hout, Wout, ldy, cout_off, Cout, taps, stats=None, stride=1,
                  grid=None, om=1, oy0=0, ox0=0, cin_off=None, Cin=None, what="conv", planar_out=False, stats_rows=2,
                  accumulate=False, collect=None, out_slope=None, cdt=None, out_scale=None, out_quant=None, out_quant_stride=0, heads_epi=None,
                  actbwd=None, only_variant=None):
        cdt = self.dt if cdt is None else cdt
        d = L.ConvDesc()
        if out_slope is not None:
            d.out_act, d.out_slope = 1, out_slope
        src.fill(d.src)
        d.w, d.bias, d.y = w.data_ptr(), bias, y.data_ptr()
# ... 51 lines not shown

    def emit_conv_batch(self, ops, items, what):
        n = len(items)
        arr, meta = self._batch([d for d, _w, _m in items], [m for _d, _w, m in items], items[0][2]["kernel"].replace("<", "_x%d<" % n, 1))
        if not self.lib.abc_conv_batch_ok(arr, n):
            for d, w, m in items:
                self._emit(ops, self.lib.abc_conv_fwd, (d,), w, meta=m)
            return
        self._emit(ops, self.lib.abc_conv_fwd_batch, (arr, n), what, meta=meta)

    def emit_heads_batch(self, ops, items, which, what):
        want = 3 if which == 0 else 4
        ok = 1 <= len(items) <= 8 and all(self.lib.abc_conv_variant(C.byref(d)) == want for d, _w, _m in items) and self.batched_heads
        if not ok:
            for d, w, m in items:
                self._emit(ops, self.lib.abc_conv_fwd, (d,), w, meta=m)
            return
        arr, meta = self._batch([d for d, _w, _m in items], [m for _d, _w, m in items], "heads_%s_batch" % ("fwd" if which == 0 else "dgrad"))
        self._emit(ops, self.lib.abc_heads_batch, (arr, len(items), which), what, meta=meta)

    def _wgrad_desc(self, p: Src, q: Src, Ca, Cb, taps, stride, cp_off=None, cq_off=None, dual=None):
        d = L.WgradDesc()
        p.fill(d.p)
        q.fill(d.q)
        d.dtype_p, d.dtype_q, d.dtype_c = p.dt, q.dt, self.dt
        gh, gw = p.lh()
        qh, qw = q.lh()
        d.B, d.Hg, d.Wg, d.Hq, d.Wq = self.B, gh, gw, qh, qw
        d.cp_off = p.coff if cp_off is None else cp_off
        d.cq_off = q.coff if cq_off is None else cq_off
        d.Ca, d.Cb, d.stride = Ca, Cb, stride
        L.set_taps(d, taps)
        if dual is not None:
            y2, ld2, c2, out_ptr, ld_out = dual
            d.p2, d.ld_p2, d.cp2_off, d.p_dual, d.p_out, d.ld_pout = y2.data_ptr(), ld2, c2, 1, out_ptr, ld_out
            if not self.lib.abc_wgrad_fuses_apply(C.byref(d)):
                return None
        ca_pad, cb_pad, at_, bt_ = L.i32(), L.i32(), L.i32(), L.i32()
        L.check(self.lib.abc_wgrad_pads(C.byref(d), C.byref(ca_pad), C.byref(cb_pad)), "wgrad_pads")
        L.check(self.lib.abc_wgrad_tile(C.byref(d), C.byref(at_), C.byref(bt_)), "wgrad_tile")
        per_split = self.lib.abc_wgrad_blocks(C.byref(d))
        npatch = self.B * (-(-gh // 8)) * (-(-gw // 16))
        nsplit = max(1, min(max(1, npatch // 2), 256 // per_split))
        meta = {"kernel": "wgrad<%s,%s,%s,%dx%d,S%d>" % (self._dn(p.dt), self._dn(q.dt), self._dn(self.dt), at_.value, bt_.value, stride),
                "flops": 2.0 * self.B * gh * gw * Ca * Cb * len(taps)}
        return d, (ca_pad.value, cb_pad.value), (at_.value, bt_.value), nsplit, meta

    def _reduce_desc(self, partial, nsplit, ntaps, Ca, Cb, ca_pad, cb_pad, dw):
        r = L.WgradReduceDesc()
        r.partial, r.nsplit, r.ntaps, r.Ca, r.Cb, r.Ca_pad, r.Cb_pad, r.dw, r.accumulate = partial, nsplit, ntaps, Ca, Cb, ca_pad, cb_pad, dw, 0
        return r

    def emit_wgrad(self, ops, p: Src, q: Src, Ca, Cb, taps, stride, wname, what, cp_off=None, cq_off=None, dual=None, rowsum_to=None,
                   collect=None, nsplit=None):
        got = self._wgrad_desc(p, q, Ca, Cb, taps, stride, cp_off, cq_off, dual)
        if got is None:
            return False
        d, (ca_pad, cb_pad), tile, nsplit_default, meta = got
        gh, gw = p.lh()
        qh, qw = q.lh()
        nsplit_arg, nsplit = nsplit, nsplit_default
        if tile == (0, 1):
            nsplit = min(-(-self.B * gh // 12), 512)
        elif tile == (0, 2):
            nsplit = max(1, min(512, self.B * (gh // 8) * (gw // 16) // 8))
        elif tile == (0, 3):
            nsplit = max(1, min(512, self.B * (gh // 8) * (gw // 16) // 4))
        elif nsplit_arg is not None and tile == (0, 0):
            nsplit = max(1, min(nsplit_arg, self.B * gh * gw // 128))
        d.nsplit = nsplit
        need = nsplit * len(taps) * ca_pad * cb_pad
        self._ws_need = max(self._ws_need, need)
        wsk = 0
        r = self._reduce_desc(None, nsplit, len(taps), Ca, Cb, ca_pad, cb_pad, self.G(wname))
        if collect is not None:
            own = self.new((need,), torch.float32)
            d.partial = r.partial = own.data_ptr()
        else:
            self._ws_users += [(d, wsk), (r, wsk)]
        operands = self.B * gh * gw * Ca * self._esz(p.dt) + self.B * qh * qw * (4 if q.pool else 1) * Cb * self._esz(q.dt)
        meta["ws"] = wsk
        meta["bytes"] = float(operands + need * 4 + (2 * self.B * gh * gw * Ca * self._esz(self.dt) if dual is not None else 0))
        meta["operand_bytes"] = float(operands + Ca * Cb * len(taps) * 4)
        if collect is None:
            self._flush_reduce(ops)
            self._emit(ops, self.lib.abc_wgrad, (d,), what, meta=meta)
        post = [(r, what + " reduce", (wname,) if wname else (),
                 {"ws": wsk, "kernel": "wgrad_reduce", "flops": 0, "bytes": float(need * 4 + Ca * Cb * len(taps) * 4)})]
        fused_rowsum = rowsum_to is not None and bool(self.lib.abc_wgrad_rowsum_ok(C.byref(d)))
        if fused_rowsum:
            rs = self.new((nsplit, ca_pad), torch.float32)
            d.rowsum_partial = rs.data_ptr()
            post.append((self._reduce_desc(rs.data_ptr(), nsplit, 1, Ca, 1, ca_pad, 1, self.G(rowsum_to)), "dbias " + what[6:] + " reduce",
                         (rowsum_to,), {"kernel": "wgrad_reduce", "flops": 0, "bytes": float(nsplit * ca_pad * 4)}))
        if collect is not None:
            collect.append((d, what, meta, post))
        else:
            for k, (rd, w, wr, m) in enumerate(post):
                if k == 0 and self.merge_reduce and self.train:
                    self._pending_reduce = (ops, rd, w, wr, m)
                else:
                    self._emit(ops, self.lib.abc_wgrad_reduce, (rd,), w, writes=wr, meta=m)
        return "rowsum" if fused_rowsum else True

    def emit_wgrad_heads_batch(self, ops, items, what):
        def tile(d):
            at_, bt_ = L.i32(), L.i32()
            L.check(self.lib.abc_wgrad_tile(C.byref(d), C.byref(at_), C.byref(bt_)), "wgrad_tile")
            return at_.value, bt_.value
        ok = 1 <= len(items) <= 8 and all(tile(d) == (0, 0) for d, _w, _m, _p in items) and self.batched_heads
        if ok:
            arr, meta = self._batch([d for d, _w, _m, _p in items], [m for _d, _w, m, _p in items], "heads_wgrad_batch")
            self._emit(ops, self.lib.abc_wgrad_heads_batch, (arr, len(items)), what, meta=meta)
        else:
            for d, w, m, _p in items:
                self._emit(ops, self.lib.abc_wgrad, (d,), w, meta=m)
        posts = [p for _d, _w, _m, post in items for p in post]
        if ok and len(posts) <= 16:
            rarr, meta = self._batch([rd for rd, _w, _wr, _m in posts], [m for _rd, _w, _wr, m in posts], "wgrad_reduce_batch")
            self._emit(ops, self.lib.abc_wgrad_reduce_batch, (rarr, len(posts)), what + " reduce",
                       tuple(w for _rd, _w, wr, _m in posts for w in wr), meta)
        else:
            for rd, w, wr, m in posts:
                self._emit(ops, self.lib.abc_wgrad_reduce, (rd,), w, writes=wr, meta=m)

    def emit_colsum(self, ops, t, dt, npix, ld, c_off, Cn, chan_scale, bname, what):
        nb = self.lib.abc_colsum_blocks(npix)
        self._colsum_need = max(self._colsum_need, nb * Cn)
        self._colsum_users.append(self._emit(
            ops, self.lib.abc_colsum, (t.data_ptr(), dt, npix, ld, c_off, Cn, None if chan_scale is None else chan_scale.data_ptr(), None, self.G(bname)),
            what, (bname,), self._ew_meta("colsum", npix, Cn, 1, dt)))

    def emit_colsum_w1(self, ops, t, dt, npix, ld, c_off, Cn, img, bname, wname, what):
        nb = self.lib.abc_colsum_blocks(npix)
        self._colsum_need = max(self._colsum_need, 2 * nb * Cn)
        self._colsum_users.append(self._emit(
            ops, self.lib.abc_colsum_w1, (t.data_ptr(), dt, npix, ld, c_off, Cn, img.data_ptr(), None, self.G(bname), self.G(wname)),
            what, (bname, wname), {"kernel": "colsum_w1", "flops": 0, "bytes": float(npix * (Cn * self._esz(dt) + 4))}))

    def conv_bn(self, cname, bname, src: Src, cout, k, dst, slope, recname=None, stats_rows=2, force_stats=False, stat_out=None,
                collect_fin=None, shared=None):
        yt, coef, H, W, ld, coff = dst
        cin = src.C
        taps = taps_square(k)
        if self.fold:
            return self._conv_bn_folded(cname, bname, src, cout, k, dst, slope, shared)
        if shared is not None:
            stats, nblk = shared
        else:
            wf = self._pack_weights(cname + ".weight", 0, cout, cin, k)
            stats, nblk = self.emit_conv(self.fwd_ops, src, wf, self.P(cname + ".bias"), yt, self.dt, H, W, ld, coff, cout, taps,
                                         stats=self.train or force_stats, what="fwd " + cname, stats_rows=stats_rows)
        rec = Rec(kind="conv", cname=cname, bname=bname, src=src, cin=cin, cout=cout, k=k, taps=taps, y=yt, H=H, W=W, ld=ld,
                  coff=coff, coef=coef, slope=slope)
        sc, sh, sl = coef
        sl[coff:coff + cout] = slope
        rec.scale, rec.shift, rec.slopes = sc[coff:coff + cout], sh[coff:coff + cout], sl[coff:coff + cout]
        if stat_out is not None:
            rec.mean, rec.invstd = stat_out
        else:
            rec.mean, rec.invstd = self.new((cout,), torch.float32), self.new((cout,), torch.float32, 1.0)
        if self.train:
            d = L.BnFwdDesc()
            d.partial, d.nblk, d.C, d.count, d.rows = stats.data_ptr() + (4 * coff if shared is not None else 0), nblk, cout, float(self.B * H * W), stats_rows
            d.gamma, d.beta = self.P(bname + ".weight"), self.P(bname + ".bias")
            d.scale, d.shift, d.mean, d.invstd = rec.scale.data_ptr(), rec.shift.data_ptr(), rec.mean.data_ptr(), rec.invstd.data_ptr()
            d.running_mean, d.running_var = self.Bf(bname + ".running_mean"), self.Bf(bname + ".running_var")
            d.num_batches_tracked = self.Cn(bname + ".num_batches_tracked")
            d.eps, d.momentum = BN_EPS, BN_MOM
            if collect_fin is not None:
                collect_fin.append(d)
            else:
                self._emit(self.fwd_ops, self.lib.abc_bn_finalize_fwd, (d,), "bn " + bname)
        else:
            a = (self.P(bname + ".weight"), self.P(bname + ".bias"), self.Bf(bname + ".running_mean"),
                 self.Bf(bname + ".running_var"), rec.scale.data_ptr(), rec.shift.data_ptr(), cout, BN_EPS)
            self._emit(self.pack_ops, self.lib.abc_bn_eval_coeffs, a, "bn-eval " + bname, meta={"kernel": "bn_eval", "flops": 0, "bytes": 0})
        rec.stats, rec.nblk = stats, nblk
        self.recs.append(rec)
        out = Src(yt, self.dt, H, W, ld, coff, cout, coef=coef, producer=rec)
        return rec, out

    def _fold_coeffs(self, cname, bname, cout, scale_t, bias_t):
        a = (self.P(bname + ".weight"), self.P(bname + ".bias"), self.Bf(bname + ".running_mean"), self.Bf(bname + ".running_var"),
             self.P(cname + ".bias"), scale_t.data_ptr(), bias_t.data_ptr(), cout, BN_EPS)
        self._emit(self.pack_ops, self.lib.abc_bn_eval_fold, a, "bn-fold " + bname, meta={"kernel": "bn_fold", "flops": 0, "bytes": 0})

    def _conv_bn_folded(self, cname, bname, src, cout, k, dst, slope, shared):
        yt, coef, H, W, ld, coff = dst
        cin = src.C
        taps = taps_square(k)
# ... 125 lines not shown
                fused = dT
                wall = self.packed(9, cin, rows_pad)
                dT.w = wall.data_ptr()
                slice_elems = wall.numel() // 9
                first_slice = {(0, 0): 0, (0, 1): 1, (1, 0): 3, (1, 1): 5}
        for py in (0, 1):
            for px in (0, 1):
                taps = convT_phase_taps(py, px, crop_y, crop_x)
                if fused is not None:
                    wp = wall[first_slice[(py, px)] * slice_elems:(first_slice[(py, px)] + len(taps)) * slice_elems]
                    self._w_layout[wp.data_ptr()] = 1
                    self.emit_pack(name + ".up.weight", wp, 2, half, cin, 3, rows_pad, cin, py=convT_pack_parity(py, crop_y),
                                   px=convT_pack_parity(px, crop_x))
                    phases.append(wp)
                    continue
                wp = self.packed(len(taps), cin, rows_pad)
                self.emit_pack(name + ".up.weight", wp, 2, half, cin, 3, rows_pad, cin, py=convT_pack_parity(py, crop_y),
                               px=convT_pack_parity(px, crop_x))
                gh, gw = (Hs - py + 1) // 2, (Ws - px + 1) // 2
                self.emit_conv(self.fwd_ops, low, wp, self.P(name + ".up.bias"), cat, self.dt, Hs, Ws, Ctot, half, half, taps,
                               grid=(gh, gw), om=2, oy0=py, ox0=px, what="fwd %s.up phase %d%d" % (name, py, px), collect=items)
                phases.append(wp)
        if fused is not None:
            meta = {"kernel": "convt_fused<bf16>", "flops": 2.0 * self.B * lh * lw * cin * half * 9,
                    "bytes": float(self.B * lh * lw * cin * 2 + self.B * Hs * Ws * half * 2)}
            self._emit(self.fwd_ops, self.lib.abc_convt_fused_fwd, (fused,), "fwd %s.up (4 phases, one pass)" % name, meta=meta)
        else:
            self.emit_conv_batch(self.fwd_ops, items, "fwd %s.up (4 phases)" % name)
        rec = Rec(kind="convT", cname=name + ".up", src=low, cin=cin, cout=half, H=Hs, W=Ws, ld=Ctot, coff=half, y=cat,
                  taps_bwd=convT_dgrad_taps(crop_y, crop_x))
        self.recs.append(rec)
        cat_src = Src(cat, self.dt, Hs, Ws, Ctot, 0, Ctot, coef=None if self.fold else cat_coef, producer=("cat", None))
        if skip_producer is None:
            skip_producer = [r for r in self.recs if r.kind == "conv" and r.y is cat and r.coff == 0][0]
        cat_src.cat = (skip_producer, rec)
        if self.variant == "unet2":
            self.units2.append(("convT", rec))
            return self.block2(name + ".conv", cat_src, cout, 3), rec
        return self.double_conv(name + ".conv", cat_src, cout, 3), rec

    def _image_src(self):
        cin = self.in_channels
        self.img = self.new((self.B, cin, self.H, self.W), torch.float32)
        if cin == 1:
            return Src(self.img, L.F32, self.H, self.W, 1, 0, 1)
        return Src(self.img, L.F32, self.H, self.W, 0, 0, cin, planar=True)

    def _build(self):
        if self.variant == "unet2":
            return self._build2()
        B, H, W = self.B, self.H, self.W
        S = [(H >> i, W >> i) for i in range(6)]
        img_src = self._image_src()
        if self.drop_p > 0:
            self._emit(self.fwd_ops, self.lib.abc_counter_add_u32, (self.drop_salt.data_ptr(), DROP_STEP), "dropout step",
                       meta={"kernel": "counter_add", "flops": 0, "bytes": 0})
        x = None
        if self.fold and self.dt == L.BF16 and self.in_channels == 1:
            x = self._stem_fused_double_conv("inc1", img_src, 16)
        if x is None:
            x = self.double_conv("inc1", img_src, 16, 3)
        x1 = self.double_conv("inc2", x, 16, 3)
        x2 = self.double_conv("down1.maxpool_conv.1", self.pooled(x1), 32, 3)
        x = self.double_conv("down2.maxpool_conv.1", self.pooled(x2), 64, 3)
        cat3, cc3 = self.act_buf(S[2][0], S[2][1], 128)
        cat2, cc2 = self.act_buf(S[3][0], S[3][1], 256)
        cat1, cc1 = self.act_buf(S[4][0], S[4][1], 512)
        x3 = self.double_conv("inc3", x, 64, 3, dst_b=(cat3, cc3, S[2][0], S[2][1], 128, 0))
        x4 = self.double_conv("down3.maxpool_conv.1", self.pooled(x3), 128, 3, dst_b=(cat2, cc2, S[3][0], S[3][1], 256, 0))
        x5 = self.double_conv("down4.maxpool_conv.1", self.pooled(x4), 256, 3, dst_b=(cat1, cc1, S[4][0], S[4][1], 512, 0))
        x6 = self.double_conv("down5.maxpool_conv.1", self.pooled(x5), 512, 3)
        u, _ = self.up("up1", x6, cat1, cc1, S[4][0], S[4][1], 512, 256)
        u, _ = self.up("up2", u, cat2, cc2, S[3][0], S[3][1], 256, 128)
        u, _ = self.up("up3", u, cat3, cc3, S[2][0], S[2][1], 128, 128)
        u = self.double_conv("dconv1", u, 128, 3)
        trunk = self.double_conv("dconv2", u, 128, 3)
        self.trunk = trunk
        self._build_heads(trunk)
        if self.train:
            self._build_backward()
            self._flush_reduce(self.bwd_ops)
        self._finish_build()

    def _finish_build(self):
        lib = self.lib
        isz = lib.abc_pack_item_bytes()
        host = (C.c_char * (isz * len(self._pack_descs)))()
        first, elems = 0, 0
        for i, pd in enumerate(self._pack_descs):
            pd.layout = self._w_layout.get(pd.dst, 0)
            n = lib.abc_pack_item_fill(C.addressof(host) + i * isz, C.byref(pd), first)
            if n < 0:
                L.check(-1, "pack_item_fill")
            first += n
            ntaps = {0: pd.kh * pd.kw, 1: pd.kh * pd.kw, 2: (2 if pd.py else 1) * (2 if pd.px else 1), 3: 9}[pd.mode]
            elems += ntaps * pd.red_pad * pd.rows_pad
        table = torch.frombuffer(bytearray(bytes(host)), dtype=torch.uint8).to(self.dev)
        self.keep.append(table)
        self._emit(self.pack_ops, lib.abc_pack_batch, (table.data_ptr(), len(self._pack_descs), first), "pack weights",
                   meta={"kernel": "pack_batch", "flops": 0, "bytes": float(elems * (2 if self.dt == L.BF16 else 4) + elems * 4)})
        self.ws = [self.new((max(self._ws_need, 4),), torch.float32)]
        for d, k in self._ws_users:
            d.partial = self.ws[k].data_ptr()
        self.cs_ws = self.new((max(self._colsum_need, 4),), torch.float32)
        for a in self._colsum_users:
            a[7] = self.cs_ws.data_ptr()

    def _build_heads(self, trunk: Src):
        h, w = trunk.H, trunk.W
        nh = len(self.heads)
        self.h, self.w = h, w
        f8_feat = self.fp8 and trunk.dt == L.FP8 and trunk.C == 128 and nh <= 8 and self.batched_heads and (h * w) % 64 == 0
        self.hepi = None
        if self.fold and self.heads_epilogue and self.batched_heads and self.dt == L.BF16 and trunk.C == 128 and nh <= 8 and \
                (trunk.dt == L.BF16 or f8_feat):
            self.hepi = torch.zeros(nh * C.sizeof(L.HeadsEpi), dtype=torch.uint8, device=self.dev)
            self.keep.append(self.hepi)
        if self.hepi is not None:
            self.hfeat = self.new((1, 1, 1, 128 * nh), self._tdt(L.FP8) if f8_feat else None)
            self.hcoef = None
        else:
            self.hfeat, self.hcoef = self.act_buf(h, w, 128 * nh, L.FP8 if f8_feat else None)
        if f8_feat:
            self.hfeat_q = (self.new((nh,), torch.float32, 0.0), self.new((nh,), torch.float32, 1.0), self.new((nh,), torch.float32, 1.0))
        epi_items = []
        self.logits = [self.new((self.B, hc, h, w), torch.float32) for hc in self.heads]
        self.head_recs, self.head2 = [], []
        head_convs, head_fins = [], []
        self.hmean, self.hinvstd = self.new((128 * nh,), torch.float32), self.new((128 * nh,), torch.float32, 1.0)
        batch_fin = nh <= 8 and self.batched_heads
        shared = None
        if batch_fin and self.dt == L.BF16 and trunk.C == 128:
            shared = self._heads_conv1_merged(trunk, h, w)
        fused = self.want_fused_heads and shared is not None and (h * w) % 128 == 0 \
            and self.B * h * w * 128 * nh < (1 << 30)
        for i, hc in enumerate(self.heads):
            p = "out_modules.%d" % i
            rec, f = self.conv_bn(p + ".conv1", p + ".bn", trunk, 128, 3, (self.hfeat, self.hcoef, h, w, 128 * nh, 128 * i), 0.01,
                                  stat_out=(self.hmean[128 * i:128 * (i + 1)], self.hinvstd[128 * i:128 * (i + 1)]),
                                  collect_fin=head_fins if batch_fin else None, shared=shared)
            rec.is_head = True
            self.head_recs.append(rec)
            f.drop_p, f.drop_seed, f.drop_salt = self.drop_p, self.drop_seed, self.drop_salt
            if not fused:
                rows_pad = -(-hc // 32) * 32
                if self.hfeat_q is not None:
                    f.dt, f.q = L.FP8, tuple(t[i:i + 1] for t in self.hfeat_q)
                    qmul, deq = self._fp8_weight_scales(p + ".conv2.weight", hc, 128, None, f.q[1], self.new((hc,), torch.float32, 1.0),
                                                        self.new((hc,), torch.float32, 1.0))
                    w2 = self.packed(1, 128, rows_pad, cdt=L.FP8)
                    self.emit_pack(p + ".conv2.weight", w2, 0, hc, 128, 1, rows_pad, 128, row_scale=qmul.data_ptr(), cdt=L.FP8)
                    if self.hepi is not None:
                        epi_items.append((w2, self.P(p + ".conv2.bias"), deq, self.logits[i], hc, rows_pad))
                    else:
                        self.emit_conv(self.fwd_ops, f, w2, self.P(p + ".conv2.bias"), self.logits[i], L.F32, h, w, hc, 0, hc,
                                       [(0, 0)], what="fwd %s.conv2" % p, planar_out=True, collect=head_convs, cdt=L.FP8, out_scale=deq)
                    self.head2.append(Rec(kind="head2", cname=p + ".conv2", src=f, cout=hc, idx=i))
                    continue
                w2 = self._pack_weights(p + ".conv2.weight", 0, hc, 128, 1)
# ... 357 lines not shown
        self.emit_conv(ops, dy_all, wd_all, None, dtrunk, self.dt, h, w, 128, 0, 128, taps_mirror(taps), what=what)

    def _heads_bn_bwd_batch(self, ops, g, part, nblk, in_scale=None):
        nh = len(self.heads)
        Ct = 128 * nh
        ca_all, cb_all, cc_all = (self.new((Ct,), torch.float32) for _ in range(3))
        descs, writes, out = [], (), []
        for i, rec in enumerate(self.head_recs):
            sl = slice(128 * i, 128 * (i + 1))
            f, _k, wr = self._bn_bwd_desc(rec, part.data_ptr() + 4 * 128 * i, nblk, (ca_all[sl], cb_all[sl], cc_all[sl]),
                                          None if in_scale is None else in_scale.data_ptr() + 4 * self.head_off[i])
            descs.append(f)
            writes += wr
            out.append(Src(g, self.dt, rec.H, rec.W, Ct, 128 * i, 128, coef=(ca_all, cc_all, cb_all)))
        self._emit(ops, self.lib.abc_bn_finalize_bwd_batch, ((L.BnBwdDesc * nh)(*descs), nh, Ct), "bn_bwd out_modules.*.bn", writes,
                   {"kernel": "bn_bwd", "flops": 0, "bytes": 0})
        return out

    def _heads_backward_fused(self, ops):
        B, h, w = self.B, self.h, self.w
        nh = len(self.heads)
        Ct = 128 * nh
        npx = B * h * w
        writes = tuple(n for i in range(nh) for n in ("out_modules.%d.conv2.weight" % i, "out_modules.%d.conv2.bias" % i))
        self._emit(ops, self.lib.abc_heads_fused_wgrad, (self.hf,), "wgrad out_modules.*.conv2", writes,
                   {"kernel": "heads_fused_wgrad", "flops": 2.0 * npx * sum(self.heads) * 128,
                    "bytes": float(npx * Ct * 2 + self.hf_dl.numel() * 2 + self.hf_work.numel() * 4)})
        merged = self._heads_bn_bwd_batch(ops, self.hf_g, self.hf_bnpart, self.hf_chunks, in_scale=self.chan_scale)
        taps = taps_square(3)
        dyh = self.new((B, h, w, Ct))
        if not self._heads_conv1_wgrad_merged(ops, merged, dyh, taps):
            raise RuntimeError("fused heads: the merged conv1 weight gradient was refused")
        self._heads_conv1_dgrad(ops, dyh, taps)

    def _heads_conv1_wgrad_merged(self, ops, merged, dyh, taps):
        nh = len(self.heads)
        Ct = 128 * nh
        q = self.head_recs[0].src
        g0 = merged[0]
        p = Src(g0.t, self.dt, g0.H, g0.W, Ct, 0, Ct, coef=g0.coef)
        got = self._wgrad_desc(p, q, Ct, 128, taps, 1, dual=(self.hfeat, Ct, 0, dyh.data_ptr(), Ct))
        if got is None:
            return False
        d, (ca_pad, cb_pad), _tile, nsplit, meta = got
        d.nsplit = nsplit
        need = nsplit * len(taps) * ca_pad * cb_pad
        slabs = self.new((need,), torch.float32)
        d.partial = slabs.data_ptr()
        npx = self.B * g0.H * g0.W
        meta["bytes"] = float(3 * npx * Ct * self._esz(self.dt) + npx * 128 * self._esz(q.dt) + need * 4)
        self._emit(ops, self.lib.abc_wgrad, (d,), "wgrad out_modules.*.conv1", meta=meta)
        reduces = [self._reduce_desc(slabs.data_ptr() + 4 * 128 * i * cb_pad, nsplit, len(taps), 128, 128, ca_pad, cb_pad, self.G(rec.cname + ".weight"))
                   for i, rec in enumerate(self.head_recs)]
        self._emit(ops, self.lib.abc_wgrad_reduce_batch, ((L.WgradReduceDesc * nh)(*reduces), nh), "wgrad out_modules.*.conv1 reduce",
                   tuple(rec.cname + ".weight" for rec in self.head_recs),
                   {"kernel": "wgrad_reduce_batch", "flops": 0, "bytes": float(need * 4 + Ct * 128 * len(taps) * 4)})
        return True

    def _convT_backward(self, ops, rec):
        B = self.B
        dcat, ld, coff = rec.grad_out
        hs, ws = rec.H, rec.W
        dOut = Src(dcat, self.dt, hs, ws, ld, coff, rec.cout)
        self.emit_colsum(ops, dcat, self.dt, B * hs * ws, ld, coff, rec.cout, None, rec.cname + ".bias", "dbias " + rec.cname)
        self.emit_wgrad(ops, rec.src, dOut, rec.cin, rec.cout, rec.taps_bwd, 2, rec.cname + ".weight", "wgrad " + rec.cname)
        lh, lw = rec.src.lh()
        wd = self._pack_weights(rec.cname + ".weight", 3, rec.cout, rec.cin, 3)
        dsrc = self.new((B, lh, lw, rec.cin))
        rec.dsrc = dsrc
        self.emit_conv(ops, dOut, wd, None, dsrc, self.dt, lh, lw, rec.cin, 0, rec.cin, rec.taps_bwd, stride=2,
                       what="dgrad " + rec.cname)
        rec.src.producer.grad_same = (dsrc, rec.cin, 0)

    def f32buf(self, *shape, fill=0.0):
        return self.new(tuple(shape), torch.float32, fill)

    def block2(self, prefix, xin: Src, cout, k, dst=None):
        lib = self.lib
        H, W = xin.lh()
        B, cin = self.B, xin.C
        p = prefix + ".double_conv"
        t1, c1 = self.act_buf(H, W, cout)
        rec1, a1 = self.conv_bn(p + ".0", p + ".1", xin, cout, k, (t1, c1, H, W, cout, 0), 0.0)
        t2, c2 = self.act_buf(H, W, cout)
        rec2, _ = self.conv_bn(p + ".3", p + ".4", a1, cout, k, (t2, c2, H, W, cout, 0), 1.0, stats_rows=4, force_stats=True)
        mid = cout // 16
        m = p + ".5.channel_attention.shared_MLP"
        blk = Rec(kind="blk2", prefix=prefix, rec1=rec1, rec2=rec2, xin=xin, cin=cin, cout=cout, k=k, H=H, W=W, mid=mid)
        blk.ca, blk.avgz, blk.maxz = self.f32buf(B, cout), self.f32buf(B, cout), self.f32buf(B, cout)
        blk.ext, blk.first = self.f32buf(B, cout), self.new((B, cout), torch.int32, 0x7FFFFFFF)
        blk.hid_a, blk.hid_m = self.f32buf(B, mid), self.f32buf(B, mid)
        ch = L.CbamChannelDesc()
        ch.partial, ch.tiles_per_img, ch.B, ch.C, ch.mid, ch.HW = rec2.stats.data_ptr(), rec2.nblk // B, B, cout, mid, float(H * W)
        ch.scale, ch.shift = rec2.scale.data_ptr(), rec2.shift.data_ptr()
        ch.w1, ch.b1, ch.w2, ch.b2 = self.P(m + ".0.weight"), self.P(m + ".0.bias"), self.P(m + ".2.weight"), self.P(m + ".2.bias")
        ch.ca, ch.avgz, ch.maxz = blk.ca.data_ptr(), blk.avgz.data_ptr(), blk.maxz.data_ptr()
        ch.hid_avg, ch.hid_max = blk.hid_a.data_ptr(), blk.hid_m.data_ptr()
        ch.ext, ch.first = blk.ext.data_ptr(), blk.first.data_ptr()
        self._emit(self.fwd_ops, lib.abc_cbam_channel_fwd, (ch,), "cbam_channel " + prefix)
        blk.st, blk.amax, blk.sa = self.f32buf(B, H, W, 2), self.new((B, H, W), torch.int32), self.f32buf(B, H, W)
        if cin != cout:
            tr = self.new((B, H, W, cout))
            wr = self._pack_weights(prefix + ".res_conv.weight", 0, cout, cin, 1)
            self.emit_conv(self.fwd_ops, xin, wr, self.P(prefix + ".res_conv.bias"), tr, self.dt, H, W, cout, 0, cout, [(0, 0)],
                           what="fwd %s.res_conv" % prefix)
            res = (tr, cout, 0, 0)
        else:
            res = (xin.t, xin.ld, xin.coff, 1 if xin.pool else 0)
        if dst is None:
            to = self.new((B, H, W, cout))
            dst = (to, H, W, cout, 0)
        to, _, _, ld_o, coff_o = dst
        blk.out, blk.ld_out, blk.coff_out, blk.res = to, ld_o, coff_o, res

        def pix():
            d = L.CbamPixDesc()
            d.y, d.ld_y, d.cy_off = t2.data_ptr(), cout, 0
            d.scale, d.shift, d.mean, d.invstd = rec2.scale.data_ptr(), rec2.shift.data_ptr(), rec2.mean.data_ptr(), rec2.invstd.data_ptr()
            d.ca, d.maxz, d.sa, d.st, d.amax = blk.ca.data_ptr(), blk.maxz.data_ptr(), blk.sa.data_ptr(), blk.st.data_ptr(), blk.amax.data_ptr()
            d.ext, d.first = blk.ext.data_ptr(), blk.first.data_ptr()
            d.res, d.ld_res, d.cres_off, d.res_pool = res[0].data_ptr(), res[1], res[2], res[3]
            d.out, d.ld_out, d.cout_off = to.data_ptr(), ld_o, coff_o
            d.dtype, d.B, d.H, d.W, d.C = self.dt, B, H, W, cout
            return d

        blk.pix = pix
        npx = B * H * W
        self._emit(self.fwd_ops, lib.abc_cbam_spatial_stats, (pix(),), "cbam_spatial_stats " + prefix, meta=self._ew_meta("cbam_spatial_stats", npx, cout, 1))
        c7 = L.CbamConv7Desc()
        sp = p + ".5.spatial_attention.conv2d"
        c7.st, c7.w7, c7.b7, c7.sa = blk.st.data_ptr(), self.P(sp + ".weight"), self.P(sp + ".bias"), blk.sa.data_ptr()
        c7.B, c7.H, c7.W = B, H, W
        self._emit(self.fwd_ops, lib.abc_cbam_conv7_fwd, (c7,), "cbam_conv7 " + prefix)
        self._emit(self.fwd_ops, lib.abc_cbam_apply_fwd, (pix(),), "cbam_apply " + prefix, meta=self._ew_meta("cbam_apply", npx, cout, 3))
        self.units2.append(("blk", blk))
        return Src(to, self.dt, H, W, ld_o, coff_o, cout, coef=None, producer=blk)

    def _build2(self):
        B, H, W = self.B, self.H, self.W
        S = [(H >> i, W >> i) for i in range(6)]
        self.units2 = []
        img_src = self._image_src()
        x = self.block2("inc1", img_src, 32, 5)
        x1 = self.block2("inc2", x, 32, 5)
        x2 = self.block2("down1.maxpool_conv.1", self.pooled(x1), 32, 3)
        x = self.block2("down2.maxpool_conv.1", self.pooled(x2), 64, 3)
        cat3, cc3 = self.act_buf(S[2][0], S[2][1], 128)
        cat2, cc2 = self.act_buf(S[3][0], S[3][1], 256)
        cat1, cc1 = self.act_buf(S[4][0], S[4][1], 512)
        x3 = self.block2("inc3", x, 64, 3, dst=(cat3, S[2][0], S[2][1], 128, 0))
        x4 = self.block2("down3.maxpool_conv.1", self.pooled(x3), 128, 3, dst=(cat2, S[3][0], S[3][1], 256, 0))
        x5 = self.block2("down4.maxpool_conv.1", self.pooled(x4), 256, 3, dst=(cat1, S[4][0], S[4][1], 512, 0))
        x6 = self.block2("down5.maxpool_conv.1", self.pooled(x5), 512, 3)
        u, _ = self.up("up1", x6, cat1, None, S[4][0], S[4][1], 512, 256, skip_producer=x5.producer)
        u, _ = self.up("up2", u, cat2, None, S[3][0], S[3][1], 256, 128, skip_producer=x4.producer)
        u, _ = self.up("up3", u, cat3, None, S[2][0], S[2][1], 128, 128, skip_producer=x3.producer)
        u = self.block2("dconv1", u, 128, 3)
        trunk = self.block2("dconv2", u, 128, 3)
        self.trunk = trunk
        self._build_heads(trunk)
        if self.train:
            self._build_backward2()
            self._flush_reduce(self.bwd_ops)
        self._finish_build()

    def _build_backward2(self):
        ops = self.bwd_ops
        lib = self.lib
        B = self.B
        self._heads_backward(ops)
        for kind, u in reversed(self.units2):
            if kind == "convT":
                self._convT_backward(ops, u)
                continue
            blk = u
            H, W, Cc = blk.H, blk.W, blk.cout
            npx = B * H * W
            g = self.new((B, H, W, Cc))
            dz = self.new((B, H, W, Cc))
            du, dst = self.f32buf(B, H, W), self.f32buf(B, H, W, 2)
            d_avgz, d_maxz = self.f32buf(B, Cc), self.f32buf(B, Cc)
            blk.bw = {"g": g, "dz": dz, "du": du, "dst": dst, "d_avgz": d_avgz, "d_maxz": d_maxz}

            def pix(blk=blk, g=g, dz=dz, du=du, dst=dst, d_avgz=d_avgz, d_maxz=d_maxz):
                d = blk.pix()
                d.g, d.ld_g, d.dz, d.ld_dz = g.data_ptr(), Cc, dz.data_ptr(), Cc
                d.du, d.dst, d.d_avgz, d.d_maxz = du.data_ptr(), dst.data_ptr(), d_avgz.data_ptr(), d_maxz.data_ptr()
                return d

            d1 = pix()
            if blk.grad_same is not None:
                d1.d_same, d1.ld_same, d1.csame_off = blk.grad_same[0].data_ptr(), blk.grad_same[1], blk.grad_same[2]
            if blk.grad_pool is not None:
                d1.d_pool, d1.ld_pool, d1.cpool_off = blk.grad_pool[0].data_ptr(), blk.grad_pool[1], blk.grad_pool[2]
            self._emit(ops, lib.abc_cbam_bwd1, (d1,), "cbam_bwd1 " + blk.prefix, meta=self._ew_meta("cbam_bwd1", npx, Cc, 4))
            p = blk.prefix + ".double_conv"
            sp = p + ".5.spatial_attention.conv2d"
            c7 = L.CbamConv7Desc()
            c7.st, c7.w7, c7.b7, c7.du, c7.dst = blk.st.data_ptr(), self.P(sp + ".weight"), self.P(sp + ".bias"), du.data_ptr(), dst.data_ptr()
            c7.B, c7.H, c7.W = B, H, W
            nb7 = lib.abc_cbam_conv7_blocks(C.byref(c7))
            part7 = self.f32buf(nb7, 99)
            c7.dw_partial, c7.dw7, c7.db7 = part7.data_ptr(), self.G(sp + ".weight"), self.G(sp + ".bias")
            self._emit(ops, lib.abc_cbam_conv7_bwd_partial, (c7,), "cbam_conv7_bwd " + blk.prefix)
            d2 = pix()
            nb2 = lib.abc_cbam_bwd2_blocks(C.byref(d2))
            part2 = self.f32buf(B, nb2, Cc)
            d2.partial = part2.data_ptr()
            self._emit(ops, lib.abc_cbam_bwd2, (d2,), "cbam_bwd2 " + blk.prefix, meta=self._ew_meta("cbam_bwd2", npx, Cc, 3))
            m = p + ".5.channel_attention.shared_MLP"
            ch = L.CbamChannelDesc()
            ch.partial, ch.tiles_per_img, ch.B, ch.C, ch.mid, ch.HW = part2.data_ptr(), nb2, B, Cc, blk.mid, float(H * W)
            ch.w1, ch.b1, ch.w2, ch.b2 = self.P(m + ".0.weight"), self.P(m + ".0.bias"), self.P(m + ".2.weight"), self.P(m + ".2.bias")
            ch.ca, ch.avgz, ch.maxz = blk.ca.data_ptr(), blk.avgz.data_ptr(), blk.maxz.data_ptr()
            ch.hid_avg, ch.hid_max = blk.hid_a.data_ptr(), blk.hid_m.data_ptr()
            ch.dw1, ch.db1, ch.dw2, ch.db2 = self.G(m + ".0.weight"), self.G(m + ".0.bias"), self.G(m + ".2.weight"), self.G(m + ".2.bias")
# ... 58 lines not shown
```

abc-net_amd/model.py:

```python
from __future__ import annotations

import ctypes as C
import threading
import weakref
from collections import OrderedDict

import torch
import torch.nn as nn

from . import _lib as L
from . import arch
from .engine import Engine


GRAD_STORE_ALIGN = 840 * 128


def _kaiming_uniform_(t, fan_in, gen=None):
    b = 1.0 / (fan_in ** 0.5)
    with torch.no_grad():
        t.uniform_(-b, b, generator=gen)


class _UNetFn(torch.autograd.Function):
# ... 150 lines not shown

    def reset_parameters(self, seed=None):
        gen = None
        if seed is not None:
            gen = torch.Generator().manual_seed(seed)
        fan = {}
        for name, shape, role in self._table:
            if role == "param" and name.endswith(".weight") and len(shape) >= 2:
                f = shape[1]
                for d in shape[2:]:
                    f *= d
                fan[name[:-7]] = f
        with torch.no_grad():
            for name, shape, role in self._table:
                v = self._view(name)
                if v.device.type != "cpu":
                    raise L.AbcNetHipError("reset_parameters(): initialise on the host, then .to(device)")
                if role == "param":
                    if name == "s":
                        v.copy_(torch.randn(10, generator=gen) / 100)
                    elif len(shape) >= 2:
                        _kaiming_uniform_(v, fan[name[:-7]], gen)
                    elif name.endswith(".bias") and name[:-5] in fan:
                        _kaiming_uniform_(v, fan[name[:-5]], gen)
                    elif name.endswith(".weight"):
                        v.fill_(1.0)
                    else:
                        v.zero_()
                elif role == "buffer":
                    v.fill_(1.0 if name.endswith("running_var") else 0.0)
                else:
                    v.zero_()

    def named_reference_parameters(self):
        for name, shape, role in self._table:
            if role == "param":
                yield name, self._view(name)

    def grad_of(self, name):
        off, cnt = self._lay_p[name]
        return self._flat_grad[off:off + cnt].view(self._shape_role(name)[0])

    def flat_param_grads(self):
        return torch.cat([(p.grad if p.grad is not None else torch.zeros_like(p)).reshape(-1) for p in self.parameters()])

    def load_state_dict(self, state_dict, strict=True, assign=False):
        if assign:
            raise L.AbcNetHipError("load_state_dict(assign=True) would detach the parameters from the arena")
        if state_dict and all(k.startswith("module.") for k in state_dict.keys()):
            state_dict = OrderedDict((k[7:], v) for k, v in state_dict.items())
        return super().load_state_dict(state_dict, strict=strict)

    def _engine_for(self, x, train, fold_bn=False, fused_heads=False, batched_heads=True, fp8=False, guards=False, heads_epilogue=False,
                    actbwd_epilogue=True, merge_reduce=True, nms_heads=False, decode=False, dual_wgrad=True, fused_convt=True, zero_skip=True):
        if not x.is_cuda:
            raise L.AbcNetHipError("abcnet_amd runs on an MI355X only (got a %s tensor); there is no CPU fallback" % x.device)
        if x.device != self._flat.device:
            raise L.AbcNetHipError("input on %s but the model lives on %s (move one of them; several GPUs: nn.DataParallel(model, "
                                   "device_ids=...) or, better, one process per GPU -- abcnet_amd.distributed.launch_ranks / torchrun)"
                                   % (x.device, self._flat.device))
        B, Cc, H, W = x.shape
        if Cc != self.n_channels:
            raise ValueError("expected %d input channels, got %d" % (self.n_channels, Cc))
        key = (B, H, W, bool(train), self.compute_dtype, self.dropout_seed, bool(fold_bn), bool(fused_heads), bool(batched_heads), bool(fp8), bool(guards), bool(heads_epilogue), bool(actbwd_epilogue), bool(merge_reduce),
               bool(nms_heads), bool(decode), bool(dual_wgrad), bool(fused_convt), bool(zero_skip), L.load().abc_get_reserved_cus())
        eng = self._engines.get(key)
        if eng is None or eng.params.data_ptr() != self._flat.data_ptr():
            if self._flat_grad is None or self._flat_grad.device != x.device:
                pad = -(-self._np // GRAD_STORE_ALIGN) * GRAD_STORE_ALIGN
                self._grad_store = torch.zeros(pad, dtype=torch.float32, device=x.device)
                self._flat_grad = self._grad_store[:self._np]
            with torch.cuda.device(x.device):
                eng = Engine(self.VARIANT, self.n_channels, self.heads, self._flat, self._flat_grad, self._flat_buf,
                             self._counters, (self._lay_p, self._lay_b, self._lay_c), B, H, W, self.compute_dtype, train,
                             dropout_p=self.dropout_p, device=x.device, drop_seed=self.dropout_seed, fold_bn=fold_bn,
                             fused_heads=fused_heads, batched_heads=batched_heads, fp8=fp8, guards=guards, heads_epilogue=heads_epilogue, nms_heads=nms_heads,
                             actbwd_epilogue=actbwd_epilogue, merge_reduce=merge_reduce, decode=decode, dual_wgrad=dual_wgrad, fused_convt=fused_convt, zero_skip=zero_skip)
            self._engines[key] = eng
        return eng

    def _load_image(self, eng, x):
        eng.img.copy_(x.reshape(eng.img.shape))

    def _export_logits(self, eng, st):
        return [t.clone() for t in eng.logits]

    def _replica_tensors(self):
        params, bufs, cnts = [], [], []
        for name, shape, role in self._table:
            *path, attr = name.split(".")
            mod = self
            for seg in path:
                mod = mod._modules[seg]
            if role == "param":
                params.append(mod._former_parameters[attr])
            elif role == "buffer":
                bufs.append(mod._buffers[attr])
            else:
                cnts.append(mod._buffers[attr])
        return params, bufs, cnts

    def _dp_release(self, token=None):
        lock = getattr(self, "_dp_lock", None)
        if lock is None:
            self._dp_busy = False
            return
        with lock:
            if token is None or getattr(self, "_dp_token", None) is token:
                self._dp_busy = False
                self._dp_token = None

    def _dp_checkout(self, master, dev):
        with master._dp_lock:
            if dev == master._flat.device and not master._dp_busy:
                master._dp_busy = True
                return master
            pool = master._dp_shadows.setdefault(dev, [])
            for sh in pool:
                if not sh._dp_busy:
                    sh._dp_busy = True
                    return sh
            if len(pool) >= 4:
                raise L.AbcNetHipError("nn.DataParallel: more than 4 unfinished forward passes on %s (a training forward holds its "
                                       "engine until its backward has run)" % dev)
            fn, args = master.__reduce__()
            args = list(args)
            args[8] = str(dev)
            sh = fn(*args)
            sh._dp_busy = True
            pool.append(sh)
# ... 70 lines not shown
```

abc-net_amd/ops.py:

```python
from __future__ import annotations

import ctypes as C

import numpy as np
import torch

from . import _lib as L
from .contract import (HEAD_NAMES, HEADS, CandidateLists, GraphRecords, MoleculeRows, check_head_maps, check_targets, current_stream,
                       require_device_tensor, set_target_ptrs, stream_or_current)

EXTRACT_HEADS = HEADS


def _fin_desc(partial, s_ptr, ds_ptr, out, chan_scale, chan_off, head_c, grad_scale):
    f = L.LossFinDesc()
    f.partial, f.nblk, f.s, f.ds, f.out = partial.data_ptr(), partial.shape[0], s_ptr, ds_ptr, out.data_ptr()
    f.chan_scale, f.nchan = chan_scale.data_ptr(), chan_scale.numel()
    for i in range(8):
        f.chan_off[i], f.head_c[i] = chan_off[i], head_c[i]
    f.grad_scale = grad_scale
    return f


def terms_dict(out):
# ... 572 lines not shown
    UPDATE, COLUMNS = "graph_identity_update", L.GRAPH_IDENT_COLUMNS
    MAX_CAP_ATOMS, MAX_RECORD = L.MAX_SIM_ATOMS, (L.MAX_SIM_ATOMS, None)

    def __init__(self, mol_counts, mol_atoms=None, mol_bonds=None, max_atoms=256, max_bonds=256, n_valid=None, records=None,
                 max_tries=None, max_rounds=None, witness=False):
        budgets = []
        for name, v, default in (("max_tries", max_tries, L.IDENT_DEFAULT_TRIES), ("max_rounds", max_rounds, L.IDENT_DEFAULT_ROUNDS)):
            v = default if v is None else int(v)
            if not (1 <= v < 1 << 31):
                raise ValueError("GraphIdentity: %s must be 1..2^31-1, got %d" % (name, v))
            budgets.append(v)
        self.max_tries, self.max_rounds = budgets
        d = L.GraphIdentityDesc()
        d.max_tries, d.max_rounds = budgets
        records = records.records if isinstance(records, _RecordScorer) else records
        self._bind(d, (mol_counts, mol_atoms, mol_bonds), n_valid, records, max_atoms, max_bonds)
        self.map = torch.full((self.B, self.cap_atoms), -1, dtype=torch.int32, device=self.rows.device) if witness else None
        d.map_out = L.ptr(self.map)

    def result(self):
        out = self._totals()
        for share, num in (("share_same", "same"), ("share_undecided", "undecided")):
            out[share] = out[num] / out["counted"] if out["counted"] else float("nan")
        return out


def timed(stream, marks, label, flops, nbytes, fn, operand_bytes=None):
    e0, e1 = torch.cuda.Event(enable_timing=True), torch.cuda.Event(enable_timing=True)
    e0.record(stream)
    rc = fn()
    e1.record(stream)
    marks.append((label, e0, e1, {"flops": flops, "bytes": nbytes, "operand_bytes": nbytes if operand_bytes is None else operand_bytes}))
    return rc


def fold_marks(acc, marks, fields):
    for label, e0, e1, cost in marks:
        r = acc.setdefault(label, dict({"calls": 0, "ms": 0.0}, **{f: 0.0 for f in fields}))
        r["calls"] += 1
        r["ms"] += e0.elapsed_time(e1)
        for f in fields:
            r[f] += cost[f]


def per_iteration(acc, iters):
    for r in acc.values():
        for f in r:
            r[f] /= iters
    return acc


class FusedAdam:

    def __init__(self, params, grads, lr=2.5e-4, betas=(0.9, 0.999), eps=1e-8, weight_decay=1e-8, grad_scale=1.0):
        self.lib = L.load()
        self.p, self.g = params, grads
        self.m = torch.zeros_like(params)
        self.v = torch.zeros_like(params)
        self.step_t = torch.zeros(1, dtype=torch.int64, device=params.device)
        d = L.AdamDesc()
        d.p, d.g, d.m, d.v, d.n = params.data_ptr(), grads.data_ptr(), self.m.data_ptr(), self.v.data_ptr(), params.numel()
        d.step = self.step_t.data_ptr()
        d.lr, d.beta1, d.beta2, d.eps, d.weight_decay, d.grad_scale = lr, betas[0], betas[1], eps, weight_decay, grad_scale
        self.d = d

    def step(self, stream=None):
        L.check(self.lib.abc_adam_step(C.byref(self.d), stream_or_current(stream)), "adam_step")
```

abc-net_amd/train.py:

```python
from __future__ import annotations

import os

import torch

from . import _lib as L
from . import distributed as D
from .contract import HEADS, alloc_targets, check_sparse_rasterizer, current_stream, refuse_dense_targets, resolve_device
from .ops import FusedAdam, FusedHeadsLoss, FusedLoss, FusedMetrics, fold_marks, meters_dict, per_iteration, timed


class Trainer:
    def __init__(self, model, batch, height, width, lr=2.5e-4, weight_decay=1e-8, use_graph=True, bucket_mb=8.0,
                 process_group=None, device=None, metrics=False, broadcast_buffers="lazy", fused_heads=True, keep_logits=True,
                 batched_heads=True, exchange="all_reduce", force_exchange=False, guards=False, actbwd_epilogue=True, merge_reduce=True,
                 reserve_cus=None, dual_wgrad=True, fused_convt=True, exchange_dtype="f32", zero_skip=True):
        if exchange_dtype not in D.GradReducer.WIRE_DTYPES:
            raise ValueError("Trainer: exchange_dtype must be one of %s, got %r" % (D.GradReducer.WIRE_DTYPES, exchange_dtype))
        if exchange_dtype == "bf16" and exchange != "direct":
            raise ValueError("Trainer: exchange_dtype='bf16' needs exchange='direct' (the local f32 sum between all-to-all and "
                             "all-gather), got exchange=%r" % (exchange,))
        if tuple(model.heads) != HEADS:
            raise ValueError("Trainer: the fused training step is defined for heads %s (train.py:47), got heads %s"
                             % (list(HEADS), list(model.heads)))
        self.dev = dev = resolve_device(model, device, "Trainer")
        self.model = model
        dist_on = torch.distributed.is_initialized()
        self.world = torch.distributed.get_world_size(process_group) if dist_on else 1
        self.rank = torch.distributed.get_rank(process_group) if dist_on else 0
        self.group = process_group
        if broadcast_buffers not in ("step", "lazy", False):
            raise ValueError("broadcast_buffers must be 'step', 'lazy' or False")
        self.broadcast_buffers = broadcast_buffers if self.world > 1 else False
        model.dropout_seed = D.rank_dropout_seed(model.dropout_seed_base, self.rank)
        model.train()
        from .engine import set_reserved_cus
        self.reserve_cus = L.load().abc_get_reserved_cus() if reserve_cus is None else set_reserved_cus(reserve_cus)
        with torch.cuda.device(dev):
            x0 = torch.zeros((batch, model.n_channels, height, width), device=dev)
            self.eng = model._engine_for(x0, True, fused_heads=fused_heads, batched_heads=batched_heads, guards=guards,
                                         actbwd_epilogue=actbwd_epilogue, merge_reduce=merge_reduce, dual_wgrad=dual_wgrad, fused_convt=fused_convt, zero_skip=zero_skip)
        eng = self.eng
        self.targets = alloc_targets(batch, eng.h, eng.w, dev)
        off_s, _ = model._lay_p["s"]
        extra = {"keep_logits": bool(keep_logits or metrics)} if eng.hf is not None else {}
        self.loss = (FusedHeadsLoss if eng.hf is not None else FusedLoss)(
            eng, self.targets, model._flat.data.data_ptr() + 4 * off_s, model._flat_grad.data_ptr() + 4 * off_s, grad_scale=1.0 / self.world, **extra)
        self.metrics = FusedMetrics(eng.logits, self.targets) if metrics else None
        self.lr, self.wd = lr, weight_decay
        self.opt = FusedAdam(model._flat.data, model._flat_grad, lr=lr, weight_decay=weight_decay)
        names = list(model._lay_p.keys())
        sizes = [model._lay_p[n][1] for n in names]
        ready = {n: -1 for n in names}
        for j, (_fn, _args, _what, writes, _meta) in enumerate(eng.bwd_ops):
            for n in writes:
                ready[n] = max(ready[n], j)
        rd = [ready[n] for n in names]
        self.buckets = D.plan_buckets(rd, sizes, int(bucket_mb * (1 << 20) / 4))
        store = getattr(model, "_grad_store", None)
        align = 128 * self.world
        self.exchange_on = self.world > 1 or (bool(force_exchange) and dist_on)
        if self.exchange_on and exchange != "all_reduce" and store is not None and store.numel() % align == 0 \
                and store.data_ptr() == model._flat_grad.data_ptr():
            self.buckets = D.align_buckets(self.buckets, sizes, rd, align, store.numel())
            self.reducer = D.GradReducer(store, self.buckets, process_group, mode=exchange, force=force_exchange, wire_dtype=exchange_dtype)
        else:
            self.reducer = D.GradReducer(model._flat_grad, self.buckets, process_group, mode="all_reduce", force=force_exchange)
            if self.exchange_on and exchange_dtype == "bf16":
                self.reducer.fallback_reason = "the gradient store does not split into buckets of 128 x world elements: f32 all_reduce instead of the bf16 exchange"
        self.use_graph = use_graph
        self._graphs = None
        self._segments = self._plan_segments()
        self.steps = 0
        self._buffers_synced_at = 0
        self._loss_acc = torch.zeros(2, dtype=torch.float64, device=dev)

    def load_batch(self, imgs, targets=None):
        self.eng.img.copy_(imgs.reshape(self.eng.img.shape), non_blocking=True)
        if targets is None:
            return
        refuse_dense_targets(getattr(self, "_rasterizer", None))
        for dst, src in zip(self.targets, targets):
            dst.copy_(src, non_blocking=True)

    @property
    def input_images(self):
        return self.eng.img

    def use_sparse_targets(self, rasterizer):
        if not hasattr(self.loss, "use_target_flags"):
            raise L.AbcNetHipError("sparse targets need the fused heads pass (bf16, fused_heads=True)")
        if rasterizer is None:
            self.loss.use_target_flags(None)
            self._rasterizer = None
        else:
            check_sparse_rasterizer(rasterizer, self.targets, "Trainer")
            self.loss.use_target_flags(rasterizer.group_flags)
            self._rasterizer = rasterizer
        self._graphs = None

    def reset_optimizer(self, lr):
        self.lr = lr
        self.opt = FusedAdam(self.model._flat.data, self.model._flat_grad, lr=lr, weight_decay=self.wd)
        self._graphs = None

    def _plan_segments(self):
        eng = self.eng
        pre = [eng.run_pack, eng.run_forward, self.loss.run]
        if self.metrics is not None:
            pre.append(self.metrics.run)
        cut = sorted(set(b[2] for b in self.buckets)) if self.exchange_on else []
        segs, seg_b = [], []
        cur = list(pre)
        start = 0
        ops = eng.bwd_ops
        early = [b for b in self.buckets if b[2] < 0]
        for c in [c for c in cut if c >= 0]:
            chunk = ops[start:c + 1]
            cur.append(lambda st, chunk=chunk: eng._run(chunk, st))
            segs.append(cur)
            seg_b.append([b for b in self.buckets if b[2] == c])
            cur = []
            start = c + 1
        tail = ops[start:]
        if tail:
            cur.append(lambda st, chunk=tail: eng._run(chunk, st))
        segs.append(cur)
        seg_b.append([])
        self._early = early
        self._seg_buckets = seg_b
        return segs

    def _run_segment(self, k):
        st = current_stream(self.dev)
        for fn in self._segments[k]:
            fn(st)

    def _capture(self):
        graphs = []
        for k in range(len(self._segments)):
            if not self._segments[k]:
                graphs.append(None)
                continue
            g = torch.cuda.CUDAGraph()
            with torch.cuda.graph(g, capture_error_mode="thread_local"):
                self._run_segment(k)
            graphs.append(g)
        gopt = torch.cuda.CUDAGraph()
        with torch.cuda.graph(gopt, capture_error_mode="thread_local"):
            self.opt.step()
        self._graphs = (graphs, gopt)

    def sync_buffers(self):
        if self.world > 1:
            with torch.cuda.device(self.dev):
                D.broadcast_buffers(self.model._flat_buf, self.model._counters, group=self.group)
# ... 130 lines not shown
```

include/abcnet_hip.h:

```cpp
#ifndef ABCNET_HIP_H
#define ABCNET_HIP_H
#include <stdint.h>

#ifdef __cplusplus
extern "C" {
#endif

typedef void* abc_stream_t;

enum abc_status { ABC_OK = 0, ABC_EINVAL = -1, ABC_EUNSUPPORTED = -2, ABC_ELAUNCH = -3 };
enum abc_dtype { ABC_F32 = 0, ABC_BF16 = 1, ABC_FP8 = 2  };
#define ABC_MAX_TAPS_C 49

typedef struct abc_act_src {
    const void* x;
    const float* scale;
    const float* shift;
    const float* slope;
    int32_t Hx, Wx, ldx;
    int32_t pool;
    float drop_p;
    uint32_t drop_seed;
    int32_t planar;
    int32_t ctot;
// ... 29 lines not shown
    void* pool_y;
    int32_t ld_pool;
    const float* stem_x; const float* stem_w; const float* stem_scale; const float* stem_bias; float stem_slope;
    const float* out_scale;
    const float* out_quant;
    int32_t out_quant_stride;
    const abc_heads_epi* heads_epi;
    const void* actbwd_y;
    int32_t actbwd_ld, actbwd_coff;
    const float *actbwd_scale, *actbwd_shift, *actbwd_slope, *actbwd_mean, *actbwd_invstd;
    float* head_aux;
    int32_t head_aux_mode;
} abc_conv_desc;

int abc_conv_stat_blocks(const abc_conv_desc* d);
int abc_conv_fwd_batch(const abc_conv_desc* d, int32_t n, abc_stream_t stream);

typedef struct abc_convt_desc {
    abc_act_src src;
    const void* w; const float* bias; void* y;
    int32_t dtype;
    int32_t B, Hin, Win, cin_off, Cin;
    int32_t Hout, Wout, ldy, cout_off, Cout, Cout_pad;
} abc_convt_desc;
int abc_convt_fused_ok(const abc_convt_desc* d);
int abc_convt_fused_fwd(const abc_convt_desc* d, abc_stream_t stream);
int abc_conv_batch_ok(const abc_conv_desc* d, int32_t n);
int abc_conv_actbwd_ok(const abc_conv_desc* d);
int abc_conv_variant(const abc_conv_desc* d);
int abc_conv_fwd(const abc_conv_desc* d, abc_stream_t stream);
int abc_conv_tile(const abc_conv_desc* d, int32_t* bn, int32_t* mt, int32_t* ck);
int abc_conv_route_info(const abc_conv_desc* d, int32_t* info);

int abc_conv_chunk(int dtype_c, int Cin);

typedef struct abc_pack_desc {
    const float* w; void* dst;
    int32_t mode, dtype_c, Cout, Cin, kh, kw, py, px;
    int32_t rows_pad;
    int32_t red_pad;
    int32_t red_total;
    int32_t red_off;
    int32_t ck;
    int32_t rows_total;
    int32_t rows_off;
    int32_t layout;
    const float* row_scale;
} abc_pack_desc;
int abc_pack_conv_weights(const abc_pack_desc* d, abc_stream_t stream);
int abc_conv_weight_layout(const abc_conv_desc* d);
int abc_pack_item_bytes(void);
int64_t abc_pack_item_fill(void* item, const abc_pack_desc* d, int64_t first);
int abc_pack_batch(const void* items_dev, int32_t nitems, int64_t total, abc_stream_t stream);

int abc_absmax(const void* x, int32_t dtype, int64_t n, float* out, abc_stream_t stream);
int abc_absmax_cols(const void* x, int32_t dtype, int64_t npix, int32_t ld, int32_t c_off, int32_t C, float* out, abc_stream_t stream);
int abc_fp8_act_scale(const float* amax, float margin, float* s_out, float* inv_s_out, abc_stream_t stream);
int abc_fp8_weight_scales(const float* w, int32_t rows, int32_t K, const float* fold, const float* s_in, float* qmul, float* deq,
                          abc_stream_t stream);

typedef struct abc_bn_fwd_desc {
    const float* partial; int32_t nblk; int32_t C; double count;
    int32_t rows;
    const float* gamma; const float* beta;
    float* scale; float* shift; float* mean; float* invstd;
    float* running_mean; float* running_var; int64_t* num_batches_tracked;
    float eps, momentum;
} abc_bn_fwd_desc;
int abc_bn_finalize_fwd(const abc_bn_fwd_desc* d, abc_stream_t stream);
int abc_bn_finalize_fwd_batch(const abc_bn_fwd_desc* descs, int32_t n, int32_t pstride, abc_stream_t stream);
int abc_bn_eval_coeffs(const float* gamma, const float* beta, const float* running_mean, const float* running_var,
                       float* scale, float* shift, int32_t C, float eps, abc_stream_t stream);

int abc_bn_eval_fold(const float* gamma, const float* beta, const float* running_mean, const float* running_var,
                     const float* conv_bias, float* scale, float* bias_out, int32_t C, float eps, abc_stream_t stream);

typedef struct abc_act_bwd_desc {
    const void* y_raw; int32_t ld_y;
    const void* dA_same; int32_t ld_same;
    const void* dA_pool; int32_t ld_pool;
    void* g; int32_t ld_g;
    float* partial;
    const float* scale; const float* shift; const float* slope; const float* mean; const float* invstd;
    int32_t dtype, B, H, W, C, cy_off, csame_off, cpool_off;
    float drop_p; uint32_t drop_seed; int32_t drop_ld;
    const uint32_t* drop_salt;
} abc_act_bwd_desc;
int abc_act_bwd_blocks(const abc_act_bwd_desc* d);
int abc_act_bwd(const abc_act_bwd_desc* d, abc_stream_t stream);
typedef struct abc_bn_bwd_desc {
    const float* partial; int32_t nblk; int32_t C; double count;
    const float* gamma; const float* invstd;
    float* dgamma; float* dbeta; float* k1; float* k2; float* gscale;
    const float* mean; float* ca; float* cb; float* cc;
    const float* in_scale;
} abc_bn_bwd_desc;
int abc_bn_finalize_bwd(const abc_bn_bwd_desc* d, abc_stream_t stream);
int abc_bn_finalize_bwd_batch(const abc_bn_bwd_desc* descs, int32_t n, int32_t pstride, abc_stream_t stream);
typedef struct abc_bn_apply_desc {
    void* g; int32_t ld_g; const void* y_raw; int32_t ld_y; int32_t cy_off;
    const float* mean; const float* invstd; const float* k1; const float* k2; const float* gscale;
    int32_t dtype, C; int64_t npix;
    void* out; int32_t ld_out;
} abc_bn_apply_desc;
int abc_bn_apply_bwd(const abc_bn_apply_desc* d, abc_stream_t stream);

typedef struct abc_wgrad_desc {
    abc_act_src p;
    abc_act_src q;
    float* partial;
    int32_t dtype_p, dtype_q, dtype_c;
    int32_t B, Hg, Wg;
    int32_t Hq, Wq;
    int32_t cp_off, Ca, cq_off, Cb;
    int32_t stride, ntaps, nsplit;
    int8_t tap_dy[ABC_MAX_TAPS_C];
    int8_t tap_dx[ABC_MAX_TAPS_C];
    const void* p2; int32_t ld_p2, cp2_off, p_dual; void* p_out; int32_t ld_pout;
    float* rowsum_partial;
} abc_wgrad_desc;
int abc_wgrad_rowsum_ok(const abc_wgrad_desc* d);
int abc_wgrad_fuses_apply(const abc_wgrad_desc* d);
int abc_wgrad_pads(const abc_wgrad_desc* d, int32_t* ca_pad, int32_t* cb_pad);
int abc_wgrad_tile(const abc_wgrad_desc* d, int32_t* at, int32_t* bt);
int abc_wgrad_route_info(const abc_wgrad_desc* d, int32_t* info);
int abc_wgrad_blocks(const abc_wgrad_desc* d);
int abc_wgrad(const abc_wgrad_desc* d, abc_stream_t stream);
typedef struct abc_wgrad_reduce_desc {
    const float* partial; int32_t nsplit, ntaps, Ca, Cb, Ca_pad, Cb_pad;
    float* dw;
    int32_t accumulate;
} abc_wgrad_reduce_desc;
int abc_wgrad_heads_batch(const abc_wgrad_desc* descs, int32_t n, abc_stream_t stream);
int abc_wgrad_reduce(const abc_wgrad_reduce_desc* d, abc_stream_t stream);
int abc_wgrad_reduce_bn_bwd(const abc_wgrad_reduce_desc* r, const abc_bn_bwd_desc* f, abc_stream_t stream);
int abc_wgrad_reduce_batch(const abc_wgrad_reduce_desc* descs, int32_t n, abc_stream_t stream);

int abc_colsum_blocks(int64_t npix);
int abc_colsum(const void* x, int32_t dtype, int64_t npix, int32_t ld, int32_t c_off, int32_t C,
               const float* chan_scale, float* work , float* out, abc_stream_t stream);
int abc_colsum_w1(const void* x, int32_t dtype, int64_t npix, int32_t ld, int32_t c_off, int32_t C, const float* w,
                  float* work, float* out_sum, float* out_w, abc_stream_t stream);

typedef struct abc_loss_desc {
    const float* logits[8]; float* dlogits[8];
    const float* t_atom; const float* t_types; const float* t_charges; const float* t_hs; const float* t_bond;
    const float* t_btypes; const double* t_rho; const double* t_omega;
    int32_t B, h, w;
    double* partial;
} abc_loss_desc;
int abc_loss_blocks(const abc_loss_desc* d);
int abc_loss_fwd_bwd(const abc_loss_desc* d, abc_stream_t stream);
typedef struct abc_loss_fin_desc {
    const double* partial; int32_t nblk;
    const float* s; float* ds;
    double* out;
    float* chan_scale; int32_t nchan;
    int32_t chan_off[8]; int32_t head_c[8];
    float grad_scale;
} abc_loss_fin_desc;
int abc_loss_finalize(const abc_loss_fin_desc* d, abc_stream_t stream);
typedef struct abc_loss_scale_desc {
    float* dlogits[8]; int64_t n[8];
    const float* head_scale;
    float* ds;
    const double* grad_out;
} abc_loss_scale_desc;
int abc_loss_scale_grads(const abc_loss_scale_desc* d, abc_stream_t stream);

int abc_plane_sum_work(int32_t C);
int abc_plane_sum(const float* x, int32_t B, int32_t C, int32_t HW, const float* chan_scale, float* work, float* out,
                  abc_stream_t stream);

typedef struct abc_adam_desc {
    float* p; const float* g; float* m; float* v; int64_t n;
    int64_t* step;
    float lr, beta1, beta2, eps, weight_decay, grad_scale;
} abc_adam_desc;
int abc_adam_step(const abc_adam_desc* d, abc_stream_t stream);

#define ABC_ADAM_MAX_CLASSES 32
typedef struct abc_adam_seg {
    float* p; const float* g; float* m; float* v;
    int64_t n;
    int64_t first_chunk;
    int32_t cls;
    int32_t pad_;
} abc_adam_seg;
typedef struct abc_adam_class {
    float step_size;
    float bc2_sqrt;
    float beta1, beta2, eps, weight_decay;
    float pad_[2];
} abc_adam_class;
typedef struct abc_adam_multi_desc {
    const abc_adam_seg* segs;
    int32_t nseg;
    int32_t nclass;
    int64_t chunk_total;
    abc_adam_class cls[ABC_ADAM_MAX_CLASSES];
} abc_adam_multi_desc;
int abc_adam_multi_chunk(void);
int abc_adam_multi(const abc_adam_multi_desc* d, abc_stream_t stream);

int abc_heads_batch(const abc_conv_desc* descs, int32_t n, int32_t which, abc_stream_t stream);

typedef struct abc_heads_fused_desc {
    const void* feat; int32_t ld;
    const float* scale; const float* shift; const float* slope;
    const float* mean; const float* invstd;
    float drop_p; uint32_t drop_seed; const uint32_t* drop_salt;
    const float* w2[8]; const float* b2[8];
    void* w2_pack;
    float* logits[8];
    const float* t_atom; const float* t_types; const float* t_charges; const float* t_hs; const float* t_bond;
    const float* t_btypes; const double* t_rho; const double* t_omega;
    void* dl;
    void* g;
    float* bn_partial;
    double* loss_partial;
    int32_t B, h, w;
    const float* chan_scale; int32_t chan_off[8];
    float* dw2[8]; float* db2[8];
    float* wgrad_work;
    void* keep_mask;
    const uint32_t* target_flags; const void* zero_bytes;
    uint64_t* dl_tiles; int32_t no_zero_skip; int32_t pad_;
} abc_heads_fused_desc;
int64_t abc_heads_fused_pack_bytes(void);
int abc_heads_fused_chunks(const abc_heads_fused_desc* d);
int abc_heads_fused_loss_blocks(const abc_heads_fused_desc* d);
int64_t abc_heads_fused_dl_elems(const abc_heads_fused_desc* d);
// ... 322 lines not shown
```

Measured before the change: 2815 images/sec.

## Merge small independent kernels into shared launches to cut launch count

Adds combined kernels that dispatch by block index: the pack-tiles and pack-batch kernels share one grid (with an optional counter bump), the wgrad reduce batch is fused with the BN backward finalize, and a 'shared small' kernel runs a wgrad reduce, BN bwd finalize, colsum and colsum-reduce together. The Adam step counter increment is folded into an existing launch, so Adam uses an update-only entry point. The intent is to remove per-launch overhead and serialization gaps for many tiny kernels in the graph. The risk is heterogeneous blocks sharing one launch, with larger shared memory or register use per block and possible ordering issues between the merged pieces.

```diff
diff --git a/abc-net_amd/_lib.py b/abc-net_amd/_lib.py
--- a/abc-net_amd/_lib.py
+++ b/abc-net_amd/_lib.py
@@ -300,6 +300,7 @@
     "abc_pack_item_bytes": (C.c_int, []),
     "abc_pack_item_fill": (i64, [vp, P(PackDesc), i64]),
     "abc_pack_batch": (C.c_int, [vp, i32, i64, vp]),
+    "abc_pack_batch_shared": (C.c_int, [vp, i32, i64, vp, u32, vp]),
     "abc_bn_finalize_fwd": (C.c_int, [P(BnFwdDesc), vp]),
     "abc_bn_finalize_fwd_batch": (C.c_int, [vp, i32, i32, vp]),
     "abc_bn_finalize_bwd_batch": (C.c_int, [vp, i32, i32, vp]),
@@ -317,9 +318,13 @@
     "abc_wgrad_route_info": (C.c_int, [P(WgradDesc), P(i32)]),
     "abc_wgrad": (C.c_int, [P(WgradDesc), vp]),
     "abc_wgrad_reduce": (C.c_int, [P(WgradReduceDesc), vp]),
+    "abc_wgrad_reduce_is_wave": (C.c_int, [P(WgradReduceDesc)]),
     "abc_wgrad_reduce_bn_bwd": (C.c_int, [P(WgradReduceDesc), P(BnBwdDesc), vp]),
     "abc_wgrad_heads_batch": (C.c_int, [vp, i32, vp]),
     "abc_wgrad_reduce_batch": (C.c_int, [vp, i32, vp]),
+    "abc_wgrad_reduce_batch_bn_bwd": (C.c_int, [vp, i32, P(BnBwdDesc), vp]),
+    "abc_shared_small_colsum_ok": (C.c_int, [i32, i32, i32, i32]),
+    "abc_shared_small": (C.c_int, [P(WgradReduceDesc), P(BnBwdDesc), vp, i32, i64, i32, i32, i32, vp, vp, vp, i32, i32, vp, vp, vp]),
     "abc_colsum_blocks": (C.c_int, [i64]),
     "abc_colsum": (C.c_int, [vp, i32, i64, i32, i32, i32, vp, vp, vp, vp]),
     "abc_colsum_w1": (C.c_int, [vp, i32, i64, i32, i32, i32, vp, vp, vp, vp, vp]),
@@ -327,6 +332,7 @@
     "abc_loss_fwd_bwd": (C.c_int, [P(LossDesc), vp]),
     "abc_loss_finalize": (C.c_int, [P(LossFinDesc), vp]),
     "abc_adam_step": (C.c_int, [P(AdamDesc), vp]),
+    "abc_adam_update": (C.c_int, [P(AdamDesc), vp]),
     "abc_loss_scale_grads": (C.c_int, [P(LossScaleDesc), vp]),
     "abc_adam_multi_chunk": (C.c_int, []),
     "abc_adam_multi": (C.c_int, [P(AdamMultiDesc), vp]),
diff --git a/abc-net_amd/csrc/bn_act.hip b/abc-net_amd/csrc/bn_act.hip
--- a/abc-net_amd/csrc/bn_act.hip
+++ b/abc-net_amd/csrc/bn_act.hip
@@ -329,47 +329,11 @@
 }
 template <typename T>
 __global__ __launch_bounds__(256) void colsum_vec_kernel(const T* x, int64_t npix, int ld, int c_off, int C, const float* cs, float* work) {
-    constexpr int N = VecOf<T>::N;
-    __shared__ float red[256][N + 1];
-    const int ncv = C / N;
-    const int cv = threadIdx.x % ncv, pl = threadIdx.x / ncv, PL = 256 / ncv;
-    float acc[N];
-#pragma unroll
-    for (int j = 0; j < N; ++j) acc[j] = 0.f;
-    const T* base = x + c_off + cv * N;
-    int64_t p = (int64_t)blockIdx.x * PL + pl;
-    const int64_t step = (int64_t)gridDim.x * PL;
-    for (; p + step < npix; p += 2 * step) {
-        float a[N], b[N];
-        ldv<T, N>(base + p * ld, a);
-        ldv<T, N>(base + (p + step) * ld, b);
-#pragma unroll
-        for (int j = 0; j < N; ++j) acc[j] += a[j] + b[j];
-    }
-    if (p < npix) {
-        float a[N];
-        ldv<T, N>(base + p * ld, a);
-#pragma unroll
-        for (int j = 0; j < N; ++j) acc[j] += a[j];
-    }
-#pragma unroll
-    for (int j = 0; j < N; ++j) red[threadIdx.x][j] = acc[j];
-    __syncthreads();
-    for (int c = threadIdx.x; c < C; c += 256) {
-        const int v = c / N, j = c % N;
-        float s = 0.f;
-        for (int q = 0; q < PL; ++q) s += red[q * ncv + v][j];
-        work[(size_t)blockIdx.x * C + c] = s * (cs ? cs[c_off + c] : 1.f);
-    }
+    colsum_vec_body<T, VecOf<T>::N>(x, npix, ld, c_off, C, cs, work, blockIdx.x, gridDim.x);
 }
 
 __global__ __launch_bounds__(256) void colsum_reduce_kernel(const float* work, int nblk, int C, float* out) {
-    __shared__ double sm[4];
-    const int c = blockIdx.x;
-    double s = 0.0;
-    for (int k = threadIdx.x; k < nblk; k += 256) s += (double)work[(size_t)k * C + c];
-    s = block_sum_f64(s, sm);
-    if (threadIdx.x == 0) out[c] = (float)s;
+    colsum_reduce_body(work, nblk, C, out, blockIdx.x);
 }
 template <typename T>
 __global__ __launch_bounds__(256) void colsum_w1_kernel(const T* x, int64_t npix, int ld, int c_off, int C, const float* w, float* work) {
@@ -566,17 +530,13 @@
     const int nb = abc_colsum_blocks(npix);
     hipStream_t st = (hipStream_t)stream;
     if (C > 512) return abc_fail(ABC_EUNSUPPORTED, "colsum: C > 512");
-    {
-        const int N = dtype == ABC_BF16 ? 8 : 4;
-        const int ncv = C / N;
-        if (C % N == 0 && ncv >= 1 && ncv <= 256 && 256 % ncv == 0 && ld % N == 0 && c_off % N == 0) {
-            if (dtype == ABC_BF16)
-                hipLaunchKernelGGL(colsum_vec_kernel<bf16>, dim3(nb), dim3(256), 0, st, (const bf16*)x, npix, ld, c_off, C, chan_scale, work);
-            else
-                hipLaunchKernelGGL(colsum_vec_kernel<float>, dim3(nb), dim3(256), 0, st, (const float*)x, npix, ld, c_off, C, chan_scale, work);
-            hipLaunchKernelGGL(colsum_reduce_kernel, dim3(C), dim3(256), 0, st, (const float*)work, nb, C, out);
-            return abc_check_launch("colsum");
-        }
+    if (colsum_vec_ok(dtype, ld, c_off, C)) {
+        if (dtype == ABC_BF16)
+            hipLaunchKernelGGL(colsum_vec_kernel<bf16>, dim3(nb), dim3(256), 0, st, (const bf16*)x, npix, ld, c_off, C, chan_scale, work);
+        else
+            hipLaunchKernelGGL(colsum_vec_kernel<float>, dim3(nb), dim3(256), 0, st, (const float*)x, npix, ld, c_off, C, chan_scale, work);
+        hipLaunchKernelGGL(colsum_reduce_kernel, dim3(C), dim3(256), 0, st, (const float*)work, nb, C, out);
+        return abc_check_launch("colsum");
     }
     int CW = 1;
     while (CW < C && CW < 64) CW <<= 1;
diff --git a/abc-net_amd/csrc/misc.hip b/abc-net_amd/csrc/misc.hip
--- a/abc-net_amd/csrc/misc.hip
+++ b/abc-net_amd/csrc/misc.hip
@@ -120,9 +120,9 @@
     }
     return lo;
 }
-__global__ __launch_bounds__(256) void pack_batch_kernel(const PackItem* items, int nitems, int64_t total) {
+__device__ inline void pack_batch_body(const PackItem* items, int nitems, int64_t total, int blk) {
     __shared__ int s_lo, s_hi;
-    const int64_t i0 = (int64_t)blockIdx.x * PACK_CHUNK;
+    const int64_t i0 = (int64_t)blk * PACK_CHUNK;
     const int64_t i1 = (i0 + PACK_CHUNK < total) ? i0 + PACK_CHUNK : total;
     if (threadIdx.x == 0) { s_lo = pack_find(items, nitems, i0); s_hi = pack_find(items, nitems, i1 - 1); }
     __syncthreads();
@@ -140,10 +140,13 @@
         }
     }
 }
+__global__ __launch_bounds__(256) void pack_batch_kernel(const PackItem* items, int nitems, int64_t total) {
+    pack_batch_body(items, nitems, total, blockIdx.x);
+}
 
 constexpr int PT_MAXT = 9;
 constexpr int PT_MAXITEMS = 1023;
-__global__ __launch_bounds__(256) void pack_tiles_kernel(const PackItem* items, int nitems) {
+__device__ inline void pack_tiles_body(const PackItem* items, int nitems, int blk, int nblk) {
     __shared__ float tile[32 * (32 * PT_MAXT + 1)];
     __shared__ int s_nt[PT_MAXITEMS + 1];
     __shared__ int s_item, s_tile;
@@ -156,7 +159,7 @@
     }
     __syncthreads();
     const int total = s_nt[nitems];
-    for (int tg = blockIdx.x; tg < total; tg += gridDim.x) {
+    for (int tg = blk; tg < total; tg += nblk) {
         __syncthreads();
         if (tid == 0) {
             int lo = 0, hi = nitems - 1;
@@ -231,6 +234,15 @@
             *(bf16x8*)((bf16*)d.dst + off) = o;
         }
     }
+}
+constexpr int PT_BLOCKS = 2048;
+__global__ __launch_bounds__(256) void pack_tiles_kernel(const PackItem* items, int nitems) { pack_tiles_body(items, nitems, blockIdx.x, gridDim.x); }
+
+__global__ __launch_bounds__(256) void pack_shared_kernel(const PackItem* items, int nitems, int64_t total, int nbatch, uint32_t* counter, uint32_t inc) {
+    const int blk = blockIdx.x;
+    if (blk < PT_BLOCKS) pack_tiles_body(items, nitems, blk, PT_BLOCKS);
+    else if (blk < PT_BLOCKS + nbatch) pack_batch_body(items, nitems, total, blk - PT_BLOCKS);
+    else if (counter != nullptr && threadIdx.x == 0) *counter += inc;
 }
 
 __global__ void step_inc_kernel(int64_t* step) { *step += 1; }
@@ -464,8 +476,18 @@
     if (nitems > PT_MAXITEMS) return abc_fail(ABC_EINVAL, "pack_batch: more than 1023 items");
     const int64_t nb = (total + PACK_CHUNK - 1) / PACK_CHUNK;
     if (nb > 0) hipLaunchKernelGGL(pack_batch_kernel, dim3((int)nb), dim3(256), 0, (hipStream_t)stream, (const PackItem*)items_dev, nitems, total);
-    hipLaunchKernelGGL(pack_tiles_kernel, dim3(2048), dim3(256), 0, (hipStream_t)stream, (const PackItem*)items_dev, nitems);
+    hipLaunchKernelGGL(pack_tiles_kernel, dim3(PT_BLOCKS), dim3(256), 0, (hipStream_t)stream, (const PackItem*)items_dev, nitems);
     return abc_check_launch("pack_batch");
+}
+
+extern "C" int abc_pack_batch_shared(const void* items_dev, int32_t nitems, int64_t total, uint32_t* counter, uint32_t inc, abc_stream_t stream) {
+    if (nitems < 1 || total < 0) return abc_fail(ABC_EINVAL, "pack_batch_shared: empty");
+    if (nitems > PT_MAXITEMS) return abc_fail(ABC_EINVAL, "pack_batch_shared: more than 1023 items");
+    const int64_t nb = (total + PACK_CHUNK - 1) / PACK_CHUNK;
+    if (nb > 0x7fffffff - PT_BLOCKS - 1) return abc_fail(ABC_EUNSUPPORTED, "pack_batch_shared: grid");
+    hipLaunchKernelGGL(pack_shared_kernel, dim3(PT_BLOCKS + (int)nb + (counter != nullptr ? 1 : 0)), dim3(256), 0, (hipStream_t)stream,
+                       (const PackItem*)items_dev, nitems, total, (int)nb, counter, inc);
+    return abc_check_launch("pack_batch_shared");
 }
 
 extern "C" int abc_adam_step(const abc_adam_desc* d, abc_stream_t stream) {
@@ -478,6 +500,16 @@
     if (nb < 1) nb = 1;
     hipLaunchKernelGGL(adam_kernel, dim3((int)nb), dim3(256), 0, st, *d);
     return abc_check_launch("adam_step");
+}
+
+extern "C" int abc_adam_update(const abc_adam_desc* d, abc_stream_t stream) {
+    if (d->n < 1) return abc_fail(ABC_EINVAL, "adam: empty");
+    if (((uintptr_t)d->p | (uintptr_t)d->g | (uintptr_t)d->m | (uintptr_t)d->v) & 15) return abc_fail(ABC_EINVAL, "adam: 16-byte alignment");
+    int64_t nb = (d->n / 4 + 255) / 256;
+    if (nb > 2048) nb = 2048;
+    if (nb < 1) nb = 1;
+    hipLaunchKernelGGL(adam_kernel, dim3((int)nb), dim3(256), 0, (hipStream_t)stream, *d);
+    return abc_check_launch("adam_update");
 }
 
 extern "C" int abc_plane_sum_work(int32_t C) { return C * PS_CHUNKS; }
diff --git a/abc-net_amd/csrc/reduce_bn.hpp b/abc-net_amd/csrc/reduce_bn.hpp
--- a/abc-net_amd/csrc/reduce_bn.hpp
+++ b/abc-net_amd/csrc/reduce_bn.hpp
@@ -111,3 +111,75 @@
 #pragma unroll
     for (int j = 0; j < 4; ++j) o[(size_t)j * d.ntaps] = d.accumulate ? (o[(size_t)j * d.ntaps] + r[j]) : r[j];
 }
+
+
+__device__ inline void wgrad_reduce_wave_body(const abc_wgrad_reduce_desc& d, int64_t idx, int lane) {
+    if (idx >= (int64_t)d.ntaps * d.Ca * d.Cb) return;
+    const int bi = (int)(idx % d.Cb), ai = (int)((idx / d.Cb) % d.Ca), t = (int)(idx / ((int64_t)d.Cb * d.Ca));
+    const size_t slab = (size_t)d.Ca_pad * d.Cb_pad;
+    const float* p = d.partial + (size_t)t * slab + (size_t)ai * d.Cb_pad + bi;
+    const size_t step = (size_t)d.ntaps * slab;
+    float s = 0.f;
+    for (int k = lane; k < d.nsplit; k += 64) s += p[(size_t)k * step];
+    for (int m = 32; m >= 1; m >>= 1) s += __shfl_xor(s, m);
+    if (lane == 0) {
+        float* o = d.dw + ((size_t)ai * d.Cb + bi) * d.ntaps + t;
+        *o = d.accumulate ? (*o + s) : s;
+    }
+}
+
+__device__ inline bool wgrad_reduce_batch_wave(const abc_wgrad_reduce_desc& d) { return (int64_t)d.ntaps * d.Ca * d.Cb <= 4096 && d.nsplit >= 128; }
+__device__ inline void wgrad_reduce_batch_body(const abc_wgrad_reduce_desc& d, int blk) {
+    if (wgrad_reduce_batch_wave(d)) wgrad_reduce_wave_body(d, (int64_t)blk * 4 + (threadIdx.x >> 6), threadIdx.x & 63);
+    else wgrad_reduce_body(d, blk);
+}
+
+
+template <typename T, int N>
+__device__ inline void colsum_vec_body(const T* x, int64_t npix, int ld, int c_off, int C, const float* cs, float* work, int blk, int nblk) {
+    __shared__ float red[256][N + 1];
+    const int ncv = C / N;
+    const int cv = threadIdx.x % ncv, pl = threadIdx.x / ncv, PL = 256 / ncv;
+    float acc[N];
+#pragma unroll
+    for (int j = 0; j < N; ++j) acc[j] = 0.f;
+    const T* base = x + c_off + cv * N;
+    int64_t p = (int64_t)blk * PL + pl;
+    const int64_t step = (int64_t)nblk * PL;
+    for (; p + step < npix; p += 2 * step) {
+        float a[N], b[N];
+        LoadVec<T, N>::ld(base + p * ld, a);
+        LoadVec<T, N>::ld(base + (p + step) * ld, b);
+#pragma unroll
+        for (int j = 0; j < N; ++j) acc[j] += a[j] + b[j];
+    }
+    if (p < npix) {
+        float a[N];
+        LoadVec<T, N>::ld(base + p * ld, a);
+#pragma unroll
+        for (int j = 0; j < N; ++j) acc[j] += a[j];
+    }
+#pragma unroll
+    for (int j = 0; j < N; ++j) red[threadIdx.x][j] = acc[j];
+    __syncthreads();
+    for (int c = threadIdx.x; c < C; c += 256) {
+        const int v = c / N, j = c % N;
+        float s = 0.f;
+        for (int q = 0; q < PL; ++q) s += red[q * ncv + v][j];
+        work[(size_t)blk * C + c] = s * (cs ? cs[c_off + c] : 1.f);
+    }
+}
+
+inline bool colsum_vec_ok(int dtype, int ld, int c_off, int C) {
+    const int N = dtype == ABC_BF16 ? 8 : 4;
+    const int ncv = C / N;
+    return C <= 512 && C % N == 0 && ncv >= 1 && ncv <= 256 && 256 % ncv == 0 && ld % N == 0 && c_off % N == 0;
+}
+
+__device__ inline void colsum_reduce_body(const float* work, int nblk, int C, float* out, int c) {
+    __shared__ double sm[4];
+    double s = 0.0;
+    for (int k = threadIdx.x; k < nblk; k += 256) s += (double)work[(size_t)k * C + c];
+    s = block_sum_f64(s, sm);
+    if (threadIdx.x == 0) out[c] = (float)s;
+}
diff --git a/abc-net_amd/csrc/wgrad.hip b/abc-net_amd/csrc/wgrad.hip
--- a/abc-net_amd/csrc/wgrad.hip
+++ b/abc-net_amd/csrc/wgrad.hip
@@ -4,6 +4,7 @@
 #include "conv_fast.hpp"
 #include <stddef.h>
 #include <stdlib.h>
+#include <string.h>
 #include <algorithm>
 
 namespace {
@@ -378,58 +379,45 @@
     }
 }
 
-__global__ __launch_bounds__(64) void wgrad_reduce_wave_kernel(const abc_wgrad_reduce_desc d) {
-    const int idx = blockIdx.x;
-    const int bi = idx % d.Cb, ai = (idx / d.Cb) % d.Ca, t = idx / (d.Cb * d.Ca);
-    const size_t slab = (size_t)d.Ca_pad * d.Cb_pad;
-    const float* p = d.partial + (size_t)t * slab + (size_t)ai * d.Cb_pad + bi;
-    const size_t step = (size_t)d.ntaps * slab;
-    float s = 0.f;
-    for (int k = threadIdx.x; k < d.nsplit; k += 64) s += p[(size_t)k * step];
-    for (int m = 32; m >= 1; m >>= 1) s += __shfl_xor(s, m);
-    if (threadIdx.x == 0) {
-        float* o = d.dw + ((size_t)ai * d.Cb + bi) * d.ntaps + t;
-        *o = d.accumulate ? (*o + s) : s;
-    }
-}
+__global__ __launch_bounds__(64) void wgrad_reduce_wave_kernel(const abc_wgrad_reduce_desc d) { wgrad_reduce_wave_body(d, blockIdx.x, threadIdx.x); }
 
 constexpr int MAX_RB = 16;
 struct ReduceBatch { abc_wgrad_reduce_desc d[MAX_RB]; };
-__global__ __launch_bounds__(256) void wgrad_reduce_batch_kernel(const ReduceBatch bt) {
-    const abc_wgrad_reduce_desc& d = bt.d[blockIdx.y];
-    const int64_t n = (int64_t)d.ntaps * d.Ca * d.Cb;
-    const size_t slab = (size_t)d.Ca_pad * d.Cb_pad;
-    const size_t step = (size_t)d.ntaps * slab;
-    if (n <= 4096 && d.nsplit >= 128) {
-        const int64_t idx = (int64_t)blockIdx.x * 4 + (threadIdx.x >> 6);
-        const int lane = threadIdx.x & 63;
-        if (idx >= n) return;
-        const int bi = (int)(idx % d.Cb), ai = (int)((idx / d.Cb) % d.Ca), t = (int)(idx / ((int64_t)d.Cb * d.Ca));
-        const float* p = d.partial + (size_t)t * slab + (size_t)ai * d.Cb_pad + bi;
-        float s = 0.f;
-        for (int k = lane; k < d.nsplit; k += 64) s += p[(size_t)k * step];
-        for (int m = 32; m >= 1; m >>= 1) s += __shfl_xor(s, m);
-        if (lane == 0) {
-            float* o = d.dw + ((size_t)ai * d.Cb + bi) * d.ntaps + t;
-            *o = d.accumulate ? (*o + s) : s;
-        }
+__global__ __launch_bounds__(256) void wgrad_reduce_batch_kernel(const ReduceBatch bt) { wgrad_reduce_batch_body(bt.d[blockIdx.y], blockIdx.x); }
+
+struct ReduceBatchBn { ReduceBatch bt; abc_bn_bwd_desc f; int gx, n; };
+__global__ __launch_bounds__(256) void wgrad_reduce_batch_bn_kernel(const ReduceBatchBn a) {
+    const int blk = blockIdx.x, nb = a.gx * a.n;
+    if (blk < nb) wgrad_reduce_batch_body(a.bt.d[blk / a.gx], blk % a.gx);
+    else bn_finalize_bwd_body(a.f, a.f.C, blk - nb);
+}
+
+struct SharedSmall {
+    abc_wgrad_reduce_desc r; int r_kind, nr;
+    abc_bn_bwd_desc f; int nf;
+    const void* cs_x; int64_t cs_npix; int cs_f32, cs_ld, cs_coff, cs_C; const float* cs_scale; float* cs_work; int ncs;
+    const float* cr_work; int cr_nblk, cr_C; float* cr_out;
+    int64_t* step;
+};
+__global__ __launch_bounds__(256) void shared_small_kernel(const SharedSmall a) {
+    int blk = blockIdx.x;
+    if (blk < a.nr) {
+        if (a.r_kind == 0) wgrad_reduce_wave_body(a.r, (int64_t)blk * 4 + (threadIdx.x >> 6), threadIdx.x & 63);
+        else if (a.r_kind == 1) wgrad_reduce_vec_body(a.r, blk);
+        else wgrad_reduce_body(a.r, blk);
         return;
     }
-    const int64_t idx = (int64_t)blockIdx.x * 256 + threadIdx.x;
-    if (idx >= n) return;
-    const int bi = (int)(idx % d.Cb);
-    const int ai = (int)((idx / d.Cb) % d.Ca);
-    const int t = (int)(idx / ((int64_t)d.Cb * d.Ca));
-    const float* p = d.partial + (size_t)t * slab + (size_t)ai * d.Cb_pad + bi;
-    float s0 = 0.f, s1 = 0.f, s2 = 0.f, s3 = 0.f;
-    int k = 0;
-    for (; k + 4 <= d.nsplit; k += 4) {
-        s0 += p[(size_t)k * step]; s1 += p[(size_t)(k + 1) * step]; s2 += p[(size_t)(k + 2) * step]; s3 += p[(size_t)(k + 3) * step];
-    }
-    for (; k < d.nsplit; ++k) s0 += p[(size_t)k * step];
-    const float s = (s0 + s1) + (s2 + s3);
-    float* o = d.dw + ((size_t)ai * d.Cb + bi) * d.ntaps + t;
-    *o = d.accumulate ? (*o + s) : s;
+    blk -= a.nr;
+    if (blk < a.nf) { bn_finalize_bwd_body(a.f, a.f.C, blk); return; }
+    blk -= a.nf;
+    if (blk < a.ncs) {
+        if (a.cs_f32) colsum_vec_body<float, 4>((const float*)a.cs_x, a.cs_npix, a.cs_ld, a.cs_coff, a.cs_C, a.cs_scale, a.cs_work, blk, a.ncs);
+        else colsum_vec_body<bf16, 8>((const bf16*)a.cs_x, a.cs_npix, a.cs_ld, a.cs_coff, a.cs_C, a.cs_scale, a.cs_work, blk, a.ncs);
+        return;
+    }
+    blk -= a.ncs;
+    if (blk < a.cr_C) { colsum_reduce_body(a.cr_work, a.cr_nblk, a.cr_C, a.cr_out, blk); return; }
+    if (a.step != nullptr && threadIdx.x == 0) *a.step += 1;
 }
 
 struct WGeom {
@@ -718,6 +706,8 @@
     return abc_fail(ABC_EUNSUPPORTED, "wgrad: dtype combination");
 }
 
+extern "C" int abc_wgrad_reduce_is_wave(const abc_wgrad_reduce_desc* d) { return reduce_form(*d).kind == RED_WAVE ? 1 : 0; }
+
 extern "C" int abc_wgrad_reduce(const abc_wgrad_reduce_desc* d, abc_stream_t stream) {
     const ReduceForm f = reduce_form(*d);
     if (f.kind == RED_WAVE) hipLaunchKernelGGL(wgrad_reduce_wave_kernel, dim3(f.grid), dim3(64), 0, (hipStream_t)stream, *d);
@@ -755,3 +745,59 @@
     hipLaunchKernelGGL(wgrad_reduce_batch_kernel, dim3((int)gx, n), dim3(256), 0, (hipStream_t)stream, bt);
     return abc_check_launch("wgrad_reduce_batch");
 }
+
+extern "C" int abc_wgrad_reduce_batch_bn_bwd(const abc_wgrad_reduce_desc* descs, int32_t n, const abc_bn_bwd_desc* f, abc_stream_t stream) {
+    if (n < 1 || n > MAX_RB) return abc_fail(ABC_EINVAL, "wgrad_reduce_batch_bn_bwd: 1..16 items");
+    if (f->C < 1 || f->nblk < 1) return abc_fail(ABC_EINVAL, "wgrad_reduce_batch_bn_bwd: empty finaliser");
+    ReduceBatchBn a;
+    int64_t gx = 1;
+    for (int i = 0; i < n; ++i) {
+        a.bt.d[i] = descs[i];
+        const int64_t cnt = (int64_t)descs[i].ntaps * descs[i].Ca * descs[i].Cb;
+        const int64_t blocks = reduce_form(descs[i]).kind == RED_WAVE ? (cnt + 3) / 4 : (cnt + 255) / 256;
+        gx = blocks > gx ? blocks : gx;
+    }
+    for (int i = n; i < MAX_RB; ++i) a.bt.d[i] = descs[0];
+    if (gx * n + f->C > 0x7fffffff) return abc_fail(ABC_EUNSUPPORTED, "wgrad_reduce_batch_bn_bwd: grid");
+    a.f = *f; a.gx = (int)gx; a.n = n;
+    hipLaunchKernelGGL(wgrad_reduce_batch_bn_kernel, dim3((int)gx * n + f->C), dim3(256), 0, (hipStream_t)stream, a);
+    return abc_check_launch("wgrad_reduce_batch_bn_bwd");
+}
+
+extern "C" int abc_shared_small_colsum_ok(int32_t dtype, int32_t ld, int32_t c_off, int32_t C) {
+    return (dtype == ABC_BF16 || dtype == ABC_F32) && colsum_vec_ok(dtype, ld, c_off, C) ? 1 : 0;
+}
+
+extern "C" int abc_shared_small(const abc_wgrad_reduce_desc* r, const abc_bn_bwd_desc* f,
+                                const void* cs_x, int32_t cs_dtype, int64_t cs_npix, int32_t cs_ld, int32_t cs_c_off, int32_t cs_C,
+                                const float* cs_scale, float* cs_work,
+                                const float* cr_work, int32_t cr_nblk, int32_t cr_C, float* cr_out, int64_t* step, abc_stream_t stream) {
+    SharedSmall a;
+    memset(&a, 0, sizeof(a));
+    if (r != nullptr) {
+        const ReduceForm rf = reduce_form(*r);
+        a.r = *r; a.r_kind = (int)rf.kind;
+        a.nr = rf.kind == RED_WAVE ? (rf.grid + 3) / 4 : rf.grid;
+    }
+    if (f != nullptr) {
+        if (f->C < 1 || f->nblk < 1) return abc_fail(ABC_EINVAL, "shared_small: empty finaliser");
+        a.f = *f; a.nf = f->C;
+    }
+    if (cs_x != nullptr) {
+        if (cs_work == nullptr || cs_npix < 1 || !abc_shared_small_colsum_ok(cs_dtype, cs_ld, cs_c_off, cs_C))
+            return abc_fail(ABC_EUNSUPPORTED, "shared_small: column sums in the vector form only (abc_shared_small_colsum_ok)");
+        a.cs_x = cs_x; a.cs_npix = cs_npix; a.cs_f32 = cs_dtype == ABC_F32 ? 1 : 0; a.cs_ld = cs_ld; a.cs_coff = cs_c_off; a.cs_C = cs_C;
+        a.cs_scale = cs_scale; a.cs_work = cs_work; a.ncs = abc_colsum_blocks(cs_npix);
+    }
+    if (cr_out != nullptr) {
+        if (cr_work == nullptr || cr_nblk < 1 || cr_C < 1) return abc_fail(ABC_EINVAL, "shared_small: empty column-sum second stage");
+        if (cs_x != nullptr && cs_work == cr_work) return abc_fail(ABC_EINVAL, "shared_small: both column-sum stages over one workspace");
+        a.cr_work = cr_work; a.cr_nblk = cr_nblk; a.cr_C = cr_C; a.cr_out = cr_out;
+    }
+    a.step = step;
+    const int64_t grid = (int64_t)a.nr + a.nf + a.ncs + a.cr_C + (step != nullptr ? 1 : 0);
+    if (grid < 1) return abc_fail(ABC_EINVAL, "shared_small: no part");
+    if (grid > 0x7fffffff) return abc_fail(ABC_EUNSUPPORTED, "shared_small: grid");
+    hipLaunchKernelGGL(shared_small_kernel, dim3((int)grid), dim3(256), 0, (hipStream_t)stream, a);
+    return abc_check_launch("shared_small");
+}
diff --git a/abc-net_amd/engine.py b/abc-net_amd/engine.py
--- a/abc-net_amd/engine.py
+++ b/abc-net_amd/engine.py
@@ -109,7 +109,7 @@
     def __init__(self, variant, in_channels, heads, params, grads, buffers, counters, layout, B, H, W, dtype, train,
                  dropout_p=0.2, device="cuda", drop_seed=0x1234ABCD, fold_bn=False, fused_heads=False, batched_heads=True, fp8=False,
                  guards=False, heads_epilogue=False, actbwd_epilogue=True, merge_reduce=True, nms_heads=False, decode=False,
-                 dual_wgrad=True, fused_convt=True, zero_skip=True):
+                 dual_wgrad=True, fused_convt=True, zero_skip=True, share_launches=True, step_plan=False):
         if variant not in ("unet", "unet2"):
             raise NotImplementedError("variant %r" % variant)
         if H < 32 or W < 32:
@@ -142,7 +142,12 @@
         self.actbwd_epilogue = bool(actbwd_epilogue)
         self.merge_reduce = bool(merge_reduce)
         self.zero_skip = bool(zero_skip)
+        self.share_launches = bool(share_launches)
+        self.step_plan = bool(step_plan) and train
+        self.opt_step = None
         self._pending_reduce = None
+        self._pending_batch = None
+        self._pending_colsum2 = None
         self.dt = L.BF16 if dtype == "bf16" else L.F32
         self.tdt = torch.bfloat16 if dtype == "bf16" else torch.float32
         self.batched_heads = bool(batched_heads)
@@ -236,23 +241,90 @@
         arr = (type(descs[0]) * len(descs))(*descs)
         return arr, {"kernel": kernel, "flops": sum(m["flops"] for m in metas), "bytes": sum(m["bytes"] for m in metas)}
 
-    def _flush_reduce(self, ops):
+    CS_NONE = (None, 0, 0, 0, 0, 0, None, None)
+    CR_NONE = (None, 0, 0, None)
+
+    def _emit_shared(self, ops, rd, f, cs, cr, what, writes, parts):
+        meta = {"kernel": "shared<%s>" % "+".join(k for k, _m in parts), "flops": 0, "bytes": sum(m.get("bytes", 0) for _k, m in parts),
+                "launches": 1, "riders": len(parts) - 1}
+        for _k, m in parts:
+            if "ws" in m:
+                meta["ws"] = m["ws"]
+        args = self._emit(ops, self.lib.abc_shared_small, (rd, f) + (cs or self.CS_NONE) + (cr or self.CR_NONE) + (None,), what, writes, meta)
+        if cs is not None:
+            self._colsum_users.append((args, 9))
+        if cr is not None:
+            self._colsum_users.append((args, 10))
+        return args
+
+    def _reduce_is_wave(self, rd):
+        return bool(self.lib.abc_wgrad_reduce_is_wave(C.byref(rd)))
+
+    def _flush_reduce(self, ops, cs=None):
         pr = getattr(self, "_pending_reduce", None)
         if pr is not None:
             self._pending_reduce = None
             pops, rd, what, writes, meta = pr
+            if cs is not None and pops is ops:
+                cs_args, cs_what, cs_writes, cs_meta = cs
+                self._emit_shared(ops, rd, None, cs_args, None, what + " + " + cs_what, tuple(writes) + tuple(cs_writes),
+                                  [("wgrad_reduce", meta), ("colsum1", cs_meta)])
+                return True
             self._emit(pops, self.lib.abc_wgrad_reduce, (rd,), what, writes=writes, meta=meta)
+        return False
+
+    def _flush_batch(self):
+        pb, self._pending_batch = self._pending_batch, None
+        if pb is not None:
+            pops, arr, n, what, writes, meta = pb
+            self._emit(pops, self.lib.abc_wgrad_reduce_batch, (arr, n), what, writes, meta)
+
+    def _flush_colsum2(self):
+        pc, self._pending_colsum2 = self._pending_colsum2, None
+        if pc is not None:
+            pops, cr, what, writes, meta = pc
+            self._emit_shared(pops, None, None, None, cr, what, writes, [("colsum2", meta)])
 
     def _emit_bn_bwd(self, ops, f, what, writes):
         pr = getattr(self, "_pending_reduce", None)
         if pr is None or pr[0] is not ops or not self.merge_reduce:
             self._flush_reduce(ops)
+            pr = None
+        pb, pc = self._pending_batch, self._pending_colsum2
+        if pb is not None and (pb[0] is not ops or pr is not None or pc is not None):
+            self._flush_batch()
+            pb = None
+        if pc is not None and pc[0] is not ops:
+            self._flush_colsum2()
+            pc = None
+        fmeta = {"kernel": "bn_bwd", "flops": 0, "bytes": 0}
+        if pb is not None:
+            self._pending_batch = None
+            _pops, arr, n, bwhat, bwrites, bmeta = pb
+            meta = {"kernel": "shared<bn_bwd+%s>" % bmeta["kernel"], "flops": 0, "bytes": bmeta["bytes"], "launches": 1, "riders": 1}
+            self._emit(ops, self.lib.abc_wgrad_reduce_batch_bn_bwd, (arr, n, f), what + " + " + bwhat, tuple(writes) + tuple(bwrites), meta)
+            return
+        if pr is None and pc is None:
             self._emit(ops, self.lib.abc_bn_finalize_bwd, (f,), what, writes=writes)
             return
         self._pending_reduce = None
-        _pops, rd, rwhat, rwrites, rmeta = pr
-        meta = {"ws": rmeta.get("ws", 0), "kernel": "wgrad_reduce+bn_bwd", "flops": 0, "bytes": rmeta["bytes"]}
-        self._emit(ops, self.lib.abc_wgrad_reduce_bn_bwd, (rd, f), rwhat + " + " + what, tuple(rwrites) + tuple(writes), meta)
+        rd, rwhat, rwrites, rmeta = pr[1:] if pr is not None else (None, None, (), None)
+        wave = pr is not None and self._reduce_is_wave(rd)
+        if pc is None and not (wave and self.share_launches):
+            meta = {"ws": rmeta.get("ws", 0), "kernel": "wgrad_reduce+bn_bwd", "flops": 0, "bytes": rmeta["bytes"], "launches": 2 if wave else 1}
+            self._emit(ops, self.lib.abc_wgrad_reduce_bn_bwd, (rd, f), rwhat + " + " + what, tuple(rwrites) + tuple(writes), meta)
+            return
+        parts, name, wr = [("bn_bwd", fmeta)], what, tuple(writes)
+        if pr is not None:
+            parts, name, wr = [("wgrad_reduce", rmeta)] + parts, rwhat + " + " + what, tuple(rwrites) + wr
+        cr = None
+        if pc is not None:
+            self._pending_colsum2 = None
+            _pops, cr, cwhat, cwrites, cmeta = pc
+            parts, name, wr = parts + [("colsum2", cmeta)], name + " + " + cwhat, wr + tuple(cwrites)
+        self._emit_shared(ops, rd, f, None, cr, name, wr, parts)
+        if pr is not None and not wave:
+            ops[-1].meta["riders"] -= 1
 
     def _dn(self, dt):
         return {L.BF16: "bf16", L.F32: "f32", L.FP8: "fp8"}[dt]
@@ -410,7 +482,7 @@
         return r
 
     def emit_wgrad(self, ops, p: Src, q: Src, Ca, Cb, taps, stride, wname, what, cp_off=None, cq_off=None, dual=None, rowsum_to=None,
-                   collect=None, nsplit=None):
+                   collect=None, nsplit=None, cs_rider=None):
         got = self._wgrad_desc(p, q, Ca, Cb, taps, stride, cp_off, cq_off, dual)
         if got is None:
             return False
@@ -457,6 +529,10 @@
             for k, (rd, w, wr, m) in enumerate(post):
                 if k == 0 and self.merge_reduce and self.train:
                     self._pending_reduce = (ops, rd, w, wr, m)
+                elif k == 0 and cs_rider is not None:
+                    cs_args, cs_what, cs_writes, cs_meta = cs_rider
+                    self._emit_shared(ops, rd, None, cs_args, None, w + " + " + cs_what, tuple(wr) + tuple(cs_writes),
+                                      [("wgrad_reduce", m), ("colsum1", cs_meta)])
                 else:
                     self._emit(ops, self.lib.abc_wgrad_reduce, (rd,), w, writes=wr, meta=m)
         return "rowsum" if fused_rowsum else True
@@ -483,18 +559,31 @@
                 self._emit(ops, self.lib.abc_wgrad_reduce, (rd,), w, writes=wr, meta=m)
 
     def emit_colsum(self, ops, t, dt, npix, ld, c_off, Cn, chan_scale, bname, what):
+        self._flush_colsum2()
         nb = self.lib.abc_colsum_blocks(npix)
         self._colsum_need = max(self._colsum_need, nb * Cn)
-        self._colsum_users.append(self._emit(
+        meta = self._ew_meta("colsum", npix, Cn, 1, dt)
+        meta["launches"] = 2
+        self._colsum_users.append((self._emit(
             ops, self.lib.abc_colsum, (t.data_ptr(), dt, npix, ld, c_off, Cn, None if chan_scale is None else chan_scale.data_ptr(), None, self.G(bname)),
-            what, (bname,), self._ew_meta("colsum", npix, Cn, 1, dt)))
+            what, (bname,), meta), 7))
+
+    def colsum_stages(self, t, dt, npix, ld, c_off, Cn, bname, what):
+        if not self.lib.abc_shared_small_colsum_ok(dt, ld, c_off, Cn):
+            return None
+        nb = self.lib.abc_colsum_blocks(npix)
+        self._colsum_need = max(self._colsum_need, nb * Cn)
+        first = ((t.data_ptr(), dt, npix, ld, c_off, Cn, None, None), what + " (first stage)", (), self._ew_meta("colsum", npix, Cn, 1, dt))
+        second = ((None, nb, Cn, self.G(bname)), what + " (second stage)", (bname,), {"kernel": "colsum2", "flops": 0, "bytes": float(nb * Cn * 4)})
+        return first, second
 
     def emit_colsum_w1(self, ops, t, dt, npix, ld, c_off, Cn, img, bname, wname, what):
+        self._flush_colsum2()
         nb = self.lib.abc_colsum_blocks(npix)
         self._colsum_need = max(self._colsum_need, 2 * nb * Cn)
-        self._colsum_users.append(self._emit(
+        self._colsum_users.append((self._emit(
             ops, self.lib.abc_colsum_w1, (t.data_ptr(), dt, npix, ld, c_off, Cn, img.data_ptr(), None, self.G(bname), self.G(wname)),
-            what, (bname, wname), {"kernel": "colsum_w1", "flops": 0, "bytes": float(npix * (Cn * self._esz(dt) + 4))}))
+            what, (bname, wname), {"kernel": "colsum_w1", "flops": 0, "bytes": float(npix * (Cn * self._esz(dt) + 4)), "launches": 2}), 7))
 
     def conv_bn(self, cname, bname, src: Src, cout, k, dst, slope, recname=None, stats_rows=2, force_stats=False, stat_out=None,
                 collect_fin=None, shared=None):
@@ -726,7 +815,8 @@
         B, H, W = self.B, self.H, self.W
         S = [(H >> i, W >> i) for i in range(6)]
         img_src = self._image_src()
-        if self.drop_p > 0:
+        self._drop_in_pack = self.drop_p > 0 and self.share_launches and self.step_plan
+        if self.drop_p > 0 and not self._drop_in_pack:
             self._emit(self.fwd_ops, self.lib.abc_counter_add_u32, (self.drop_salt.data_ptr(), DROP_STEP), "dropout step",
                        meta={"kernel": "counter_add", "flops": 0, "bytes": 0})
         x = None
@@ -753,8 +843,29 @@
         self._build_heads(trunk)
         if self.train:
             self._build_backward()
-            self._flush_reduce(self.bwd_ops)
+            self._finish_backward()
         self._finish_build()
+
+    def _finish_backward(self):
+        ops = self.bwd_ops
+        self._flush_reduce(ops)
+        self._flush_batch()
+        self._flush_colsum2()
+        if not (self.share_launches and self.step_plan and ops):
+            return
+        last = ops[-1]
+        if last.fn is self.lib.abc_wgrad_reduce:
+            rd = last.args[0]
+            ops.pop()
+            self._emit_shared(ops, rd, None, None, None, last.what, last.writes, [("wgrad_reduce", last.meta)])
+            last = ops[-1]
+        if last.fn is not self.lib.abc_shared_small:
+            return
+        self.opt_step = torch.zeros(1, dtype=torch.int64, device=self.dev)
+        last.args[14] = self.opt_step.data_ptr()
+        last.meta["riders"] += 1
+        last.meta["kernel"] = last.meta["kernel"][:-1] + "+step>"
+        ops[-1] = last._replace(what=last.what + " + optimiser step counter")
 
     def _finish_build(self):
         lib = self.lib
@@ -771,14 +882,23 @@
             elems += ntaps * pd.red_pad * pd.rows_pad
         table = torch.frombuffer(bytearray(bytes(host)), dtype=torch.uint8).to(self.dev)
         self.keep.append(table)
-        self._emit(self.pack_ops, lib.abc_pack_batch, (table.data_ptr(), len(self._pack_descs), first), "pack weights",
-                   meta={"kernel": "pack_batch", "flops": 0, "bytes": float(elems * (2 if self.dt == L.BF16 else 4) + elems * 4)})
+        meta = {"kernel": "pack_batch", "flops": 0, "bytes": float(elems * (2 if self.dt == L.BF16 else 4) + elems * 4),
+                "launches": 2 if first > 0 else 1}
+        if self.share_launches and self.train:
+            drop = getattr(self, "_drop_in_pack", False)
+            meta.update(kernel="shared<pack_batch+pack_tiles%s>" % ("+counter_add" if drop else ""), launches=1,
+                        riders=meta["launches"] - 1 + (1 if drop else 0))
+            self._emit(self.pack_ops, lib.abc_pack_batch_shared,
+                       (table.data_ptr(), len(self._pack_descs), first, self.drop_salt.data_ptr() if drop else None, DROP_STEP),
+                       "pack weights + dropout step" if drop else "pack weights", meta=meta)
+        else:
+            self._emit(self.pack_ops, lib.abc_pack_batch, (table.data_ptr(), len(self._pack_descs), first), "pack weights", meta=meta)
         self.ws = [self.new((max(self._ws_need, 4),), torch.float32)]
         for d, k in self._ws_users:
             d.partial = self.ws[k].data_ptr()
         self.cs_ws = self.new((max(self._colsum_need, 4),), torch.float32)
-        for a in self._colsum_users:
-            a[7] = self.cs_ws.data_ptr()
+        for a, k in self._colsum_users:
+            a[k] = self.cs_ws.data_ptr()
 
     def _build_heads(self, trunk: Src):
         h, w = trunk.H, trunk.W
@@ -1242,9 +1362,13 @@
         self._emit(ops, self.lib.abc_wgrad, (d,), "wgrad out_modules.*.conv1", meta=meta)
         reduces = [self._reduce_desc(slabs.data_ptr() + 4 * 128 * i * cb_pad, nsplit, len(taps), 128, 128, ca_pad, cb_pad, self.G(rec.cname + ".weight"))
                    for i, rec in enumerate(self.head_recs)]
-        self._emit(ops, self.lib.abc_wgrad_reduce_batch, ((L.WgradReduceDesc * nh)(*reduces), nh), "wgrad out_modules.*.conv1 reduce",
-                   tuple(rec.cname + ".weight" for rec in self.head_recs),
-                   {"kernel": "wgrad_reduce_batch", "flops": 0, "bytes": float(need * 4 + Ct * 128 * len(taps) * 4)})
+        rarr, rwrites = (L.WgradReduceDesc * nh)(*reduces), tuple(rec.cname + ".weight" for rec in self.head_recs)
+        rmeta = {"kernel": "wgrad_reduce_batch", "flops": 0, "bytes": float(need * 4 + Ct * 128 * len(taps) * 4)}
+        if self.share_launches:
+            self._flush_batch()
+            self._pending_batch = (ops, rarr, nh, "wgrad out_modules.*.conv1 reduce", rwrites, rmeta)
+        else:
+            self._emit(ops, self.lib.abc_wgrad_reduce_batch, (rarr, nh), "wgrad out_modules.*.conv1 reduce", rwrites, rmeta)
         return True
 
     def _convT_backward(self, ops, rec):
@@ -1252,8 +1376,21 @@
         dcat, ld, coff = rec.grad_out
         hs, ws = rec.H, rec.W
         dOut = Src(dcat, self.dt, hs, ws, ld, coff, rec.cout)
-        self.emit_colsum(ops, dcat, self.dt, B * hs * ws, ld, coff, rec.cout, None, rec.cname + ".bias", "dbias " + rec.cname)
-        self.emit_wgrad(ops, rec.src, dOut, rec.cin, rec.cout, rec.taps_bwd, 2, rec.cname + ".weight", "wgrad " + rec.cname)
+        stages = self.colsum_stages(dcat, self.dt, B * hs * ws, ld, coff, rec.cout, rec.cname + ".bias", "dbias " + rec.cname) \
+            if self.share_launches else None
+        pr = self._pending_reduce
+        if stages is not None and self.merge_reduce and (pr is None or pr[0] is not ops):
+            stages = None
+        if stages is None:
+            self.emit_colsum(ops, dcat, self.dt, B * hs * ws, ld, coff, rec.cout, None, rec.cname + ".bias", "dbias " + rec.cname)
+            self.emit_wgrad(ops, rec.src, dOut, rec.cin, rec.cout, rec.taps_bwd, 2, rec.cname + ".weight", "wgrad " + rec.cname)
+        else:
+            self._flush_colsum2()
+            first, second = stages
+            shared = self._flush_reduce(ops, cs=first)
+            self.emit_wgrad(ops, rec.src, dOut, rec.cin, rec.cout, rec.taps_bwd, 2, rec.cname + ".weight", "wgrad " + rec.cname,
+                            cs_rider=None if shared else first)
+            self._pending_colsum2 = (ops,) + second
         lh, lw = rec.src.lh()
         wd = self._pack_weights(rec.cname + ".weight", 3, rec.cout, rec.cin, 3)
         dsrc = self.new((B, lh, lw, rec.cin))
@@ -1351,7 +1488,7 @@
         self._build_heads(trunk)
         if self.train:
             self._build_backward2()
-            self._flush_reduce(self.bwd_ops)
+            self._finish_backward()
         self._finish_build()
 
     def _build_backward2(self):
diff --git a/abc-net_amd/model.py b/abc-net_amd/model.py
--- a/abc-net_amd/model.py
+++ b/abc-net_amd/model.py
@@ -226,7 +226,8 @@
         return super().load_state_dict(state_dict, strict=strict)
 
     def _engine_for(self, x, train, fold_bn=False, fused_heads=False, batched_heads=True, fp8=False, guards=False, heads_epilogue=False,
-                    actbwd_epilogue=True, merge_reduce=True, nms_heads=False, decode=False, dual_wgrad=True, fused_convt=True, zero_skip=True):
+                    actbwd_epilogue=True, merge_reduce=True, nms_heads=False, decode=False, dual_wgrad=True, fused_convt=True, zero_skip=True,
+                    share_launches=True, step_plan=False):
         if not x.is_cuda:
             raise L.AbcNetHipError("abcnet_amd runs on an MI355X only (got a %s tensor); there is no CPU fallback" % x.device)
         if x.device != self._flat.device:
@@ -237,7 +238,7 @@
         if Cc != self.n_channels:
             raise ValueError("expected %d input channels, got %d" % (self.n_channels, Cc))
         key = (B, H, W, bool(train), self.compute_dtype, self.dropout_seed, bool(fold_bn), bool(fused_heads), bool(batched_heads), bool(fp8), bool(guards), bool(heads_epilogue), bool(actbwd_epilogue), bool(merge_reduce),
-               bool(nms_heads), bool(decode), bool(dual_wgrad), bool(fused_convt), bool(zero_skip), L.load().abc_get_reserved_cus())
+               bool(nms_heads), bool(decode), bool(dual_wgrad), bool(fused_convt), bool(zero_skip), bool(share_launches), bool(step_plan), L.load().abc_get_reserved_cus())
         eng = self._engines.get(key)
         if eng is None or eng.params.data_ptr() != self._flat.data_ptr():
             if self._flat_grad is None or self._flat_grad.device != x.device:
@@ -249,7 +250,8 @@
                              self._counters, (self._lay_p, self._lay_b, self._lay_c), B, H, W, self.compute_dtype, train,
                              dropout_p=self.dropout_p, device=x.device, drop_seed=self.dropout_seed, fold_bn=fold_bn,
                              fused_heads=fused_heads, batched_heads=batched_heads, fp8=fp8, guards=guards, heads_epilogue=heads_epilogue, nms_heads=nms_heads,
-                             actbwd_epilogue=actbwd_epilogue, merge_reduce=merge_reduce, decode=decode, dual_wgrad=dual_wgrad, fused_convt=fused_convt, zero_skip=zero_skip)
+                             actbwd_epilogue=actbwd_epilogue, merge_reduce=merge_reduce, decode=decode, dual_wgrad=dual_wgrad, fused_convt=fused_convt, zero_skip=zero_skip,
+                             share_launches=share_launches, step_plan=step_plan)
             self._engines[key] = eng
         return eng
 
diff --git a/abc-net_amd/ops.py b/abc-net_amd/ops.py
--- a/abc-net_amd/ops.py
+++ b/abc-net_amd/ops.py
@@ -648,12 +648,14 @@
 
 class FusedAdam:
 
-    def __init__(self, params, grads, lr=2.5e-4, betas=(0.9, 0.999), eps=1e-8, weight_decay=1e-8, grad_scale=1.0):
+    def __init__(self, params, grads, lr=2.5e-4, betas=(0.9, 0.999), eps=1e-8, weight_decay=1e-8, grad_scale=1.0, step_t=None):
         self.lib = L.load()
         self.p, self.g = params, grads
         self.m = torch.zeros_like(params)
         self.v = torch.zeros_like(params)
-        self.step_t = torch.zeros(1, dtype=torch.int64, device=params.device)
+        self.counts_itself = step_t is None
+        self.launches = 2 if self.counts_itself else 1
+        self.step_t = torch.zeros(1, dtype=torch.int64, device=params.device) if step_t is None else step_t.zero_()
         d = L.AdamDesc()
         d.p, d.g, d.m, d.v, d.n = params.data_ptr(), grads.data_ptr(), self.m.data_ptr(), self.v.data_ptr(), params.numel()
         d.step = self.step_t.data_ptr()
@@ -661,4 +663,5 @@
         self.d = d
 
     def step(self, stream=None):
-        L.check(self.lib.abc_adam_step(C.byref(self.d), stream_or_current(stream)), "adam_step")
+        fn = self.lib.abc_adam_step if self.counts_itself else self.lib.abc_adam_update
+        L.check(fn(C.byref(self.d), stream_or_current(stream)), "adam_step")
diff --git a/abc-net_amd/train.py b/abc-net_amd/train.py
--- a/abc-net_amd/train.py
+++ b/abc-net_amd/train.py
@@ -14,7 +14,7 @@
     def __init__(self, model, batch, height, width, lr=2.5e-4, weight_decay=1e-8, use_graph=True, bucket_mb=8.0,
                  process_group=None, device=None, metrics=False, broadcast_buffers="lazy", fused_heads=True, keep_logits=True,
                  batched_heads=True, exchange="all_reduce", force_exchange=False, guards=False, actbwd_epilogue=True, merge_reduce=True,
-                 reserve_cus=None, dual_wgrad=True, fused_convt=True, exchange_dtype="f32", zero_skip=True):
+                 reserve_cus=None, dual_wgrad=True, fused_convt=True, exchange_dtype="f32", zero_skip=True, share_launches=True):
         if exchange_dtype not in D.GradReducer.WIRE_DTYPES:
             raise ValueError("Trainer: exchange_dtype must be one of %s, got %r" % (D.GradReducer.WIRE_DTYPES, exchange_dtype))
         if exchange_dtype == "bf16" and exchange != "direct":
@@ -39,7 +39,8 @@
         with torch.cuda.device(dev):
             x0 = torch.zeros((batch, model.n_channels, height, width), device=dev)
             self.eng = model._engine_for(x0, True, fused_heads=fused_heads, batched_heads=batched_heads, guards=guards,
-                                         actbwd_epilogue=actbwd_epilogue, merge_reduce=merge_reduce, dual_wgrad=dual_wgrad, fused_convt=fused_convt, zero_skip=zero_skip)
+                                         actbwd_epilogue=actbwd_epilogue, merge_reduce=merge_reduce, dual_wgrad=dual_wgrad, fused_convt=fused_convt, zero_skip=zero_skip,
+                                         share_launches=share_launches, step_plan=True)
         eng = self.eng
         self.targets = alloc_targets(batch, eng.h, eng.w, dev)
         off_s, _ = model._lay_p["s"]
@@ -48,7 +49,7 @@
             eng, self.targets, model._flat.data.data_ptr() + 4 * off_s, model._flat_grad.data_ptr() + 4 * off_s, grad_scale=1.0 / self.world, **extra)
         self.metrics = FusedMetrics(eng.logits, self.targets) if metrics else None
         self.lr, self.wd = lr, weight_decay
-        self.opt = FusedAdam(model._flat.data, model._flat_grad, lr=lr, weight_decay=weight_decay)
+        self.opt = FusedAdam(model._flat.data, model._flat_grad, lr=lr, weight_decay=weight_decay, step_t=eng.opt_step)
         names = list(model._lay_p.keys())
         sizes = [model._lay_p[n][1] for n in names]
         ready = {n: -1 for n in names}
@@ -101,7 +102,7 @@
 
     def reset_optimizer(self, lr):
         self.lr = lr
-        self.opt = FusedAdam(self.model._flat.data, self.model._flat_grad, lr=lr, weight_decay=self.wd)
+        self.opt = FusedAdam(self.model._flat.data, self.model._flat_grad, lr=lr, weight_decay=self.wd, step_t=self.eng.opt_step)
         self._graphs = None
 
     def _plan_segments(self):
diff --git a/include/abcnet_hip.h b/include/abcnet_hip.h
--- a/include/abcnet_hip.h
+++ b/include/abcnet_hip.h
@@ -105,6 +105,7 @@
 int abc_pack_item_bytes(void);
 int64_t abc_pack_item_fill(void* item, const abc_pack_desc* d, int64_t first);
 int abc_pack_batch(const void* items_dev, int32_t nitems, int64_t total, abc_stream_t stream);
+int abc_pack_batch_shared(const void* items_dev, int32_t nitems, int64_t total, uint32_t* counter, uint32_t inc, abc_stream_t stream);
 
 int abc_absmax(const void* x, int32_t dtype, int64_t n, float* out, abc_stream_t stream);
 int abc_absmax_cols(const void* x, int32_t dtype, int64_t npix, int32_t ld, int32_t c_off, int32_t C, float* out, abc_stream_t stream);
@@ -186,8 +187,15 @@
 } abc_wgrad_reduce_desc;
 int abc_wgrad_heads_batch(const abc_wgrad_desc* descs, int32_t n, abc_stream_t stream);
 int abc_wgrad_reduce(const abc_wgrad_reduce_desc* d, abc_stream_t stream);
+int abc_wgrad_reduce_is_wave(const abc_wgrad_reduce_desc* d);
 int abc_wgrad_reduce_bn_bwd(const abc_wgrad_reduce_desc* r, const abc_bn_bwd_desc* f, abc_stream_t stream);
 int abc_wgrad_reduce_batch(const abc_wgrad_reduce_desc* descs, int32_t n, abc_stream_t stream);
+int abc_wgrad_reduce_batch_bn_bwd(const abc_wgrad_reduce_desc* descs, int32_t n, const abc_bn_bwd_desc* f, abc_stream_t stream);
+int abc_shared_small_colsum_ok(int32_t dtype, int32_t ld, int32_t c_off, int32_t C);
+int abc_shared_small(const abc_wgrad_reduce_desc* r, const abc_bn_bwd_desc* f,
+                     const void* cs_x, int32_t cs_dtype, int64_t cs_npix, int32_t cs_ld, int32_t cs_c_off, int32_t cs_C,
+                     const float* cs_scale, float* cs_work,
+                     const float* cr_work, int32_t cr_nblk, int32_t cr_C, float* cr_out, int64_t* step, abc_stream_t stream);
 
 int abc_colsum_blocks(int64_t npix);
 int abc_colsum(const void* x, int32_t dtype, int64_t npix, int32_t ld, int32_t c_off, int32_t C,
@@ -231,6 +239,7 @@
     float lr, beta1, beta2, eps, weight_decay, grad_scale;
 } abc_adam_desc;
 int abc_adam_step(const abc_adam_desc* d, abc_stream_t stream);
+int abc_adam_update(const abc_adam_desc* d, abc_stream_t stream);
 
 #define ABC_ADAM_MAX_CLASSES 32
 typedef struct abc_adam_seg {
```

Result: no change. 2835 images/sec, median of 6 (+0.7%).
